# joejep/FOCNeRF

Measured on AMD Instinct MI355X. Metric: train_samples_per_sec, higher is better.
Workload: dtype f16

## Files before the change

### focnerf_amd/backend.py

```python
import math

import torch

from . import _lib
from ._lib import lib, ptr, stream_of, check, require_cuda, dtype_code, raw_stream


def _f32(*ts):
    for t in ts:
        if t is not None and t.dtype != torch.float32:
            raise RuntimeError(f"focnerf_amd: expected float32 tensor, got {t.dtype}")


def _contig(*ts):
    for t in ts:
        if t is not None and not t.is_contiguous():
            raise RuntimeError("focnerf_amd: tensor must be contiguous")


class _Scratch:

    def __init__(self):
        self._bufs = {}
        self._pinned = []
# ... 278 lines not shown
    def ffmlp_inference(inputs, weights, B, input_dim, output_dim, hidden_dim, num_layers, activation, output_activation, inference_buffer, outputs):
        require_cuda(inputs, weights, outputs); _half(inputs, weights, outputs); _contig(inputs, weights, outputs)
        check(lib.foc_ffmlp_inference(ptr(inputs), ptr(weights), B, input_dim, output_dim, hidden_dim, num_layers, activation, output_activation,
                                      ptr(inference_buffer), ptr(outputs), stream_of(inputs)), "ffmlp_inference")

    @staticmethod
    def ffmlp_backward(grad, inputs, weights, forward_buffer, B, input_dim, output_dim, hidden_dim, num_layers, activation, output_activation,
                       calc_grad_inputs, backward_buffer, grad_inputs, grad_weights):
        ts = (grad, inputs, weights, forward_buffer, backward_buffer, grad_inputs, grad_weights)
        require_cuda(*ts); _half(*ts); _contig(*ts)
        ws_bytes = lib.foc_ffmlp_backward_workspace_bytes(input_dim, hidden_dim, num_layers)
        ws = _scratch.get("ffmlp_ws", ws_bytes, grad.device)
        check(lib.foc_ffmlp_backward(ptr(grad), ptr(inputs), ptr(weights), ptr(forward_buffer), B, input_dim, output_dim, hidden_dim, num_layers,
                                     activation, output_activation, int(bool(calc_grad_inputs)), ptr(backward_buffer), ptr(grad_inputs),
                                     ptr(grad_weights), ptr(ws), ws.numel(), stream_of(grad)), "ffmlp_backward")

    @staticmethod
    def ffmlp_forward_planar(inputs_planar, weights, B, input_dim, output_dim, hidden_dim, num_layers, activation, output_activation, outputs):
        require_cuda(inputs_planar, weights, outputs); _half(inputs_planar, weights, outputs); _contig(inputs_planar, weights, outputs)
        check(lib.foc_ffmlp_forward_planar(ptr(inputs_planar), ptr(weights), B, input_dim, output_dim, hidden_dim, num_layers, activation,
                                           output_activation, ptr(outputs), stream_of(inputs_planar)), "ffmlp_forward_planar")

    @staticmethod
    def ffmlp_backward_planar(grad, inputs_planar, weights, B, input_dim, output_dim, hidden_dim, num_layers, activation, output_activation,
                              calc_grad_inputs, grad_inputs_planar, grad_weights):
        ts = (grad, inputs_planar, weights, grad_inputs_planar, grad_weights)
        require_cuda(*ts); _half(*ts); _contig(*ts)
        ws = _scratch.get("ffmlp_ws", lib.foc_ffmlp_backward_workspace_bytes(input_dim, hidden_dim, num_layers), grad.device)
        check(lib.foc_ffmlp_backward_planar(ptr(grad), ptr(inputs_planar), ptr(weights), B, input_dim, output_dim, hidden_dim, num_layers,
                                            activation, output_activation, int(bool(calc_grad_inputs)), ptr(grad_inputs_planar),
                                            ptr(grad_weights), ptr(ws), ws.numel(), stream_of(grad)), "ffmlp_backward_planar")

    @staticmethod
    def allocate_splitk(size):
        check(lib.foc_allocate_splitk(int(size)), "allocate_splitk")

    @staticmethod
    def free_splitk():
        check(lib.foc_free_splitk(), "free_splitk")
```

### focnerf_amd/csrc/combine.hip

```cpp
#include "common.h"
#include "fs_common.h"
#include <string.h>
#include <cmath>

static thread_local char g_err[512] = "";

void foc_set_error(const char *fmt, ...) {
    va_list ap;
    va_start(ap, fmt);
    vsnprintf(g_err, sizeof(g_err), fmt, ap);
    va_end(ap);
}

__global__ void __launch_bounds__(256) k_combine_select(const float *__restrict__ dens, const float *__restrict__ rgb,
                                                        float *__restrict__ max_dens, float *__restrict__ best_rgb, uint64_t n) {
    for (uint64_t i = (uint64_t)blockIdx.x * 256 + threadIdx.x; i < n; i += (uint64_t)gridDim.x * 256) {
        const float d = dens[i], m = max_dens[i];
        if (d > m) { best_rgb[i * 3] = rgb[i * 3]; best_rgb[i * 3 + 1] = rgb[i * 3 + 1]; best_rgb[i * 3 + 2] = rgb[i * 3 + 2]; }
        max_dens[i] = (d != d || m != m) ? __builtin_nanf("") : (d > m ? d : m);
    }
}

__global__ void __launch_bounds__(256) k_combine_pack(const float *__restrict__ dens, uint32_t rank, uint64_t *__restrict__ keys, uint64_t n) {
    for (uint64_t i = (uint64_t)blockIdx.x * 256 + threadIdx.x; i < n; i += (uint64_t)gridDim.x * 256) {
// ... 328 lines not shown
        acc4[i] = best;
    }
}

template <typename T>
__global__ void __launch_bounds__(256) k_mo_select(const T *__restrict__ sig_new, const T *__restrict__ feat_new, T *__restrict__ sig_best,
                                                   T *__restrict__ feat_best, uint64_t n, uint32_t width) {
    const uint64_t s0 = ((uint64_t)blockIdx.x * 4u + (threadIdx.x >> 6)) * 64u;
    if (s0 >= n) return;
    const uint32_t lane = threadIdx.x & 63u;
    bool take = false;
    if (s0 + lane < n) {
        const T a_raw = sig_new[s0 + lane];
        const float a = (float)a_raw, b = (float)sig_best[s0 + lane];
        take = (a != a) || (b == b && a >= b);
        if (take) sig_best[s0 + lane] = a_raw;
    }
    const uint64_t rows = __ballot(take);
    const uint32_t live = (uint32_t)(n - s0 < 64u ? n - s0 : 64u);
    const uint64_t base = s0 * width;
    for (uint32_t e = lane; e < live * width; e += 64u)
        if ((rows >> (e / width)) & 1ull) feat_best[base + e] = feat_new[base + e];
}

#include <stdlib.h>
#include <string.h>
#include <atomic>
#include <mutex>
struct FocOptionRow { const char *name; std::atomic<int> value; };
static FocOptionRow foc_option_table[FOC_OPT_COUNT] = {
    {"FOC_MLP_BWD_FUSED", 1}, {"FOC_FIELD_FWD_FUSED", 1}, {"FOC_GB_MERGE_MAX_RES", 480}, {"FOC_GB_FACTORED", 1}, {"FOC_GB_TAIL_SPLIT", 16}, {"FOC_GRID_FUSE_SMALL", 1},
    {"FOC_GRID_PAIRS", 1}, {"FOC_GRID_FAST", 1}, {"FOC_MARCH_SERIAL", -1}, {"FOC_MARCH_RAYS_ROW_MAX", 131072}, {"FOC_OCC_MARCH_FORM", -1},
    {"FOC_OCC_SAMPLE_MAJOR", 1}, {"FOC_OCC_FIELD_PIECE", 1 << 23}, {"FOC_DETERMINISTIC", 0},
};
static int foc_option_parse(int which, const char *text) {
    if (which == FOC_OPT_OCC_MARCH_FORM) {
        if (text[0] == 't') return 0;
        if (text[0] == 'r') return 1;
        if (text[0] == 'l') return 2;
        if (text[0] == 's') return 3;
    }
    return atoi(text);
}
static void foc_options_init() {
    static std::once_flag once;
    std::call_once(once, [] {
        for (int i = 0; i < FOC_OPT_COUNT; i++) {
            const char *e = getenv(foc_option_table[i].name);
            if (e && e[0]) foc_option_table[i].value.store(foc_option_parse(i, e), std::memory_order_relaxed);
        }
    });
}
int foc_opt(FocOpt which) { foc_options_init(); return foc_option_table[which].value.load(std::memory_order_relaxed); }

extern "C" {

int foc_set_option(const char *name, int value) {
    foc_options_init();
    for (int i = 0; i < FOC_OPT_COUNT; i++)
        if (name && strcmp(name, foc_option_table[i].name) == 0) { foc_option_table[i].value.store(value, std::memory_order_relaxed); return FOC_OK; }
    foc_set_error("set_option: unknown option '%s'", name ? name : "(null)");
    return FOC_E_INVALID;
}

int foc_get_option(const char *name, int *value) {
    foc_options_init();
// ... 213 lines not shown
```

### focnerf_amd/csrc/common.h

```cpp
#pragma once
#include <hip/hip_runtime.h>
#include <hip/hip_fp16.h>
#include <stdint.h>
#include <stdio.h>
#include <stdarg.h>
#include <map>
#include <mutex>
#include <tuple>
#include "../../include/focnerf.h"

#define FOC_WAVE 64

void foc_set_error(const char *fmt, ...);

enum FocOpt {
    FOC_OPT_MLP_BWD_FUSED,
    FOC_OPT_FIELD_FWD_FUSED,
    FOC_OPT_GB_MERGE_MAX_RES,
    FOC_OPT_GB_FACTORED,
    FOC_OPT_GB_TAIL_SPLIT,
    FOC_OPT_GRID_FUSE_SMALL,
    FOC_OPT_GRID_PAIRS,
    FOC_OPT_GRID_FAST,
    FOC_OPT_MARCH_SERIAL,
    FOC_OPT_MARCH_RAYS_ROW_MAX,
    FOC_OPT_OCC_MARCH_FORM,
    FOC_OPT_OCC_SAMPLE_MAJOR,
    FOC_OPT_OCC_FIELD_PIECE,
    FOC_OPT_DETERMINISTIC,
    FOC_OPT_COUNT
};
int foc_opt(FocOpt which);

#define FOC_REQUIRE(cond, code, ...)                    \
    do {                                                \
        if (!(cond)) {                                  \
            foc_set_error(__VA_ARGS__);                 \
            return (code);                              \
        }                                               \
    } while (0)

#define FOC_CHECK_LAUNCH(name)                                                     \
    do {                                                                           \
        hipError_t e_ = hipGetLastError();                                         \
        if (e_ != hipSuccess) {                                                    \
            foc_set_error("%s: launch failed: %s", name, hipGetErrorString(e_));   \
            return FOC_E_LAUNCH;                                                   \
        }                                                                          \
    } while (0)

static inline int foc_guard_pick(bool stream_is_null, int stream_device, int pointer_device, int current_device) {
    if (!stream_is_null && stream_device >= 0) return stream_device;
    if (pointer_device >= 0) return pointer_device;
    return current_device;
}
struct FocDeviceGuard {
    int prev = -1;
    explicit FocDeviceGuard(void *stream, const void *first_pointer = nullptr) {
        static int n_devices = -1;
        if (n_devices < 0 && hipGetDeviceCount(&n_devices) != hipSuccess) { (void)hipGetLastError(); n_devices = 0; }
        if (n_devices == 1) return;
        int cur = 0;
// ... 132 lines not shown
```

### focnerf_amd/csrc/ffmlp.hip

```cpp
#include "common.h"
#include "activations.h"
#include <stdlib.h>

#include <type_traits>
#include "mlp_common.h"

template <int HIDDEN, int NB, bool TRAIN, int IMODE, bool GEN = false>
__global__ void __launch_bounds__(MLP_BLOCK, 2) k_mlp_fwd(const _Float16 *__restrict__ inputs, const _Float16 *__restrict__ weights,
                                                       _Float16 *__restrict__ fwd_buf, _Float16 *__restrict__ outputs,
                                                       uint32_t B, uint32_t in_dim, uint32_t num_layers, int act, MlpHead hd) {
    const int relu = act == FOC_ACT_RELU;
    constexpr int MT = (HIDDEN + 31) / 32, KC = HIDDEN / 16;
    constexpr bool planar = IMODE == 1;
    extern __shared__ __attribute__((aligned(16))) _Float16 lds[];
    const uint32_t KS0 = IMODE == 2 ? 2u : in_dim / 16;
    const uint32_t f_hidden = MT * KS0, f_out = f_hidden + (num_layers - 1) * MT * KC;
    const float *obj_bias = reinterpret_cast<const float *>(lds + (size_t)(f_out + KC) * 512);
    if constexpr (IMODE == 2) {
        stage_weights_fwd<HIDDEN>(weights, lds, in_dim, num_layers, true, head_ld0(hd));
        if (head_bias(hd)) stage_head_bias(weights, hd, const_cast<float *>(obj_bias), HIDDEN);
    } else stage_weights_fwd<HIDDEN>(weights, lds, in_dim, num_layers);
    __syncthreads();

    const uint32_t lane = threadIdx.x & 63, wave = threadIdx.x >> 6;
// ... 301 lines not shown
                    if (!(o < OUT)) av = u32x4{0u, 0u, 0u, 0u};
                    if (!(i < IN)) bv = u32x4{0u, 0u, 0u, 0u};
                    acc[t] = mfma16(__builtin_bit_cast(h8, av), __builtin_bit_cast(h8, bv), acc[t]);
                }
            }
        }
    }
#pragma unroll
    for (int t = 0; t < 4; t++) {
        const uint32_t tile = wave + t * MLP_WAVES + 16 * blockIdx.z;
        if (tile < n_out_tiles) {
            const uint32_t mt = tile / NTi, nt = tile % NTi;
            const uint32_t i = 32 * nt + r;
#pragma unroll
            for (int reg = 0; reg < 16; reg++) {
                const uint32_t o = 32 * mt + acc_row(reg, h);
                if (o < OUT && i < IN) (void)__hip_atomic_fetch_add(ws + ws_off + (uint64_t)o * IN + i, acc[t][reg], __ATOMIC_RELAXED, __HIP_MEMORY_SCOPE_AGENT);
            }
        }
    }
}

__global__ void __launch_bounds__(256) k_mlp_dw_finalize(const float *__restrict__ ws, _Float16 *__restrict__ gw, uint32_t n) {
    for (uint32_t i = blockIdx.x * 256 + threadIdx.x; i < n; i += gridDim.x * 256) gw[i] = (_Float16)ws[i];
}
__global__ void __launch_bounds__(256) k_mlp_dw_finalize_slots(const float *__restrict__ ws, uint32_t slots, uint64_t stride, _Float16 *__restrict__ gw, uint32_t n) {
    for (uint32_t i = blockIdx.x * 256 + threadIdx.x; i < n; i += gridDim.x * 256) {
        float v = 0.0f;
        for (uint32_t k = 0; k < slots; k++) v += ws[k * stride + i];
        gw[i] = (_Float16)v;
    }
}

template <int HIDDEN, int NL, int NB, bool RECOMP, int IMODE, bool RELU_CT, bool IN32 = false, bool LEAN = false>
__global__ void __launch_bounds__(MLP_BLOCK, 2) k_mlp_bwd_fused(const _Float16 *__restrict__ grad, const _Float16 *__restrict__ inputs,
                                                             const _Float16 *__restrict__ weights, const _Float16 *__restrict__ fwd_buf,
                                                             _Float16 *__restrict__ bwd_buf_arg, _Float16 *__restrict__ grad_inputs, float *__restrict__ ws,
                                                             uint32_t B, uint32_t in_dim, int relu_rt, uint32_t lds_w_halfs, MlpHead hd) {
    const int relu = RELU_CT ? 1 : relu_rt;
    f16v FZ;
#pragma unroll
    for (int e = 0; e < 16; e++) FZ[e] = 0.0f;
    constexpr int MT = (HIDDEN + 31) / 32, KC = HIDDEN / 16, RW = 32 * NB;
    constexpr bool planar = IMODE == 1, HEAD = IMODE >= 2, NARROW = IMODE == 3;
    static_assert(!HEAD || RECOMP, "the head input modes have no stored-activation form");
    constexpr int WD = (HIDDEN < 32 ? 32 : HIDDEN) + 8;
    extern __shared__ __attribute__((aligned(16))) _Float16 lds[];
    const bool with_dx = LEAN ? true : grad_inputs != nullptr;
    _Float16 *const bwd_buf = LEAN ? nullptr : bwd_buf_arg;
    uint32_t ld0 = in_dim;
    bool has_obj = false;
    if constexpr (HEAD) { ld0 = head_ld0(hd); has_obj = hd.obj != nullptr; }
    bool col31_set = false;
    _Float16 col31 = (_Float16)0.0f;
    if constexpr (HEAD) { col31_set = head_bias(hd); col31 = has_obj ? (_Float16)1.0f : (_Float16)hd.pad; }
    stage_weights_bwd<HIDDEN>(weights, lds, in_dim, NL, with_dx, HEAD, ld0);
    const uint32_t WA = (in_dim > (uint32_t)HIDDEN ? in_dim : (uint32_t)(HIDDEN < 32 ? 32 : HIDDEN)) + 8;
    _Float16 *sD = lds + lds_w_halfs;
    _Float16 *sA = sD + 4 * RW * WD;
    _Float16 *ldsF = sA + 4 * RW * WA;
    const float *obj_bias = reinterpret_cast<const float *>(ldsF + (size_t)(((HIDDEN + 31) / 32) * (in_dim / 16) + (NL - 1) * ((HIDDEN + 31) / 32) * (HIDDEN / 16)) * 512);
    if constexpr (RECOMP) {
        stage_weights_fwd<HIDDEN>(weights, ldsF, in_dim, NL, false, ld0);
        if constexpr (HEAD) { if (head_bias(hd)) stage_head_bias(weights, hd, const_cast<float *>(obj_bias), HIDDEN); }
    }
    __syncthreads();

    const uint32_t lane = threadIdx.x & 63, wave = threadIdx.x >> 6;
    const int c = lane & 31, h = lane >> 5;
// ... 364 lines not shown
            __builtin_amdgcn_s_setprio(0);
#ifndef FOC_TIMING_NO_BARRIER
            foc_lds_barrier();
#endif
        }
    }
    float *slot = ws + (uint64_t)blockIdx.x * ((NL + 1) * MLP_DW_SLOT_STAGE);
    float *meet = reinterpret_cast<float *>(sD);
#pragma unroll
    for (int s = 0; s <= NL; s++) {
        const uint32_t OUT = s == 0 ? 16u : (uint32_t)HIDDEN;
        const uint32_t IN = s < NL ? (uint32_t)HIDDEN : in_dim;
        const uint32_t ntile = ((OUT + 31) / 32) * ((IN + 31) / 32), ksplit = (ntile * 2 <= 4) ? 2u : 1u;
        if (ksplit == 2u) {
            __syncthreads();
            if (wave >= ntile && wave < 2u * ntile) {
#pragma unroll
                for (int reg = 0; reg < 16; reg++) meet[((wave - ntile) * 16 + reg) * 64 + lane] = dwacc[s][reg];
            }
            __syncthreads();
            if (wave < ntile) {
#pragma unroll
                for (int reg = 0; reg < 16; reg++) slot[(s * 4 + wave) * 1024 + reg * 64 + lane] = dwacc[s][reg] + meet[(wave * 16 + reg) * 64 + lane];
            }
        } else if (wave < ntile) {
#pragma unroll
            for (int reg = 0; reg < 16; reg++) slot[(s * 4 + wave) * 1024 + reg * 64 + lane] = dwacc[s][reg];
        }
    }
}

template <int HIDDEN>
__global__ void __launch_bounds__(1024) k_mlp_dw_reduce(const float *__restrict__ slots, uint32_t n_slots, uint32_t NL, uint32_t in_dim, uint32_t ld0,
                                                        _Float16 *__restrict__ gw, float *__restrict__ wsb) {
    __shared__ float part[16][64];
    const uint32_t lane = threadIdx.x & 63, slice = threadIdx.x >> 6;
    const uint32_t s = blockIdx.x / 64, w = (blockIdx.x / 16) % 4, reg = blockIdx.x % 16;
    const uint32_t OUT = s == 0 ? 16u : (uint32_t)HIDDEN, IN = s < NL ? (uint32_t)HIDDEN : in_dim;
    const uint32_t NTi = (IN + 31) / 32, MTo = (OUT + 31) / 32, ntile = MTo * NTi, ksplit = 1u;
    if (w >= ntile) return;
    const uint32_t mt = w / NTi, nt = w % NTi, h = lane >> 5;
    const uint32_t o = 32 * mt + (uint32_t)acc_row((int)reg, (int)h), i = 32 * nt + (lane & 31);
    if (!(o < OUT) && !(32 * mt + (uint32_t)acc_row((int)reg, 1 - (int)h) < OUT)) return;
    const uint64_t stride = (uint64_t)(NL + 1) * MLP_DW_SLOT_STAGE;
    const float *p = slots + (uint64_t)(s * 4 + w) * 1024 + reg * 64 + lane;
    float a0 = 0.f, a1 = 0.f, a2 = 0.f, a3 = 0.f;
    for (uint32_t k = 0; k < ksplit; k++) {
        const float *q = p + (uint64_t)k * ntile * 1024;
        uint32_t g = slice;
        for (; g + 48 < n_slots; g += 64) {
            a0 += q[(uint64_t)g * stride]; a1 += q[(uint64_t)(g + 16) * stride]; a2 += q[(uint64_t)(g + 32) * stride]; a3 += q[(uint64_t)(g + 48) * stride];
        }
        for (; g < n_slots; g += 16) a0 += q[(uint64_t)g * stride];
    }
    part[slice][lane] = (a0 + a1) + (a2 + a3);
    __syncthreads();
    if (slice == 0 && o < OUT && i < IN) {
        float v = 0.f;
#pragma unroll
        for (int k = 0; k < 16; k++) v += part[k][lane];
        const uint64_t first = (uint64_t)HIDDEN * ld0, lsz = (uint64_t)HIDDEN * HIDDEN;
        const uint32_t fl = NL - s;
        const uint64_t off = (s == 0 ? first + (uint64_t)(NL - 1) * lsz : (fl == 0 ? 0 : first + (uint64_t)(fl - 1) * lsz)) + (uint64_t)o * (s == NL ? ld0 : IN) + i;
        if (wsb) wsb[off] = v; else gw[off] = (_Float16)v;
    }
}

__global__ void __launch_bounds__(256) k_mlp_dw_finalize_obj(const float *__restrict__ ws, _Float16 *__restrict__ gw, uint32_t n, uint32_t hidden,
                                                             const _Float16 *__restrict__ W, const _Float16 *__restrict__ obj, float *__restrict__ grad_obj,
                                                             float pad) {
    const uint32_t n0 = hidden * HEAD_OBJ_LD;
    for (uint32_t i = blockIdx.x * 256 + threadIdx.x; i < n; i += gridDim.x * 256) {
        float v = ws[i];
        if (i < n0) {
            const uint32_t o = i / HEAD_OBJ_LD, col = i % HEAD_OBJ_LD;
            if (col >= 31) v = col < 47 ? ws[o * HEAD_OBJ_LD + 31] * (float)obj[col - 31] : (pad != 0.0f ? ws[o * HEAD_OBJ_LD + 31] * pad : 0.0f);
        }
        gw[i] = (_Float16)v;
    }
    if (blockIdx.x == 0 && threadIdx.x < 16 && grad_obj) {
        float a = 0.0f;
        for (uint32_t o = 0; o < hidden; o++) a = fmaf((float)W[o * HEAD_OBJ_LD + 31 + threadIdx.x], ws[o * HEAD_OBJ_LD + 31], a);
        grad_obj[threadIdx.x] = a;
    }
}

__device__ __forceinline__ void nf_sh16_half(float x, float y, float z, int h, h8 &out) {
    const float xy = x * y, xz = x * z, yz = y * z, x2 = x * x, y2 = y * y, z2 = z * z;
    float o[8];
    if (h == 0) {
        o[0] = 0.28209479177387814f; o[1] = -0.48860251190291987f * y; o[2] = 0.48860251190291987f * z; o[3] = -0.48860251190291987f * x;
        o[4] = 1.0925484305920792f * xy; o[5] = -1.0925484305920792f * yz; o[6] = 0.94617469575755997f * z2 - 0.31539156525251999f;
        o[7] = -1.0925484305920792f * xz;
    } else {
        o[0] = 0.54627421529603959f * x2 - 0.54627421529603959f * y2; o[1] = 0.59004358992664352f * y * (-3.0f * x2 + y2);
        o[2] = 2.8906114426405538f * xy * z; o[3] = 0.45704579946446572f * y * (1.0f - 5.0f * z2);
        o[4] = 0.3731763325901154f * z * (5.0f * z2 - 3.0f); o[5] = 0.45704579946446572f * x * (1.0f - 5.0f * z2);
        o[6] = 1.4453057213202769f * z * (x2 - y2); o[7] = 0.59004358992664352f * x * (-x2 + 3.0f * y2);
    }
#pragma unroll
    for (int j = 0; j < 8; j++) out[j] = (_Float16)o[j];
}

template <int NLS, int NLC, bool PLANAR, bool RELU_CT, bool BLK, bool OBJ, bool P31 = false>
__global__ void __launch_bounds__(MLP_BLOCK, 2) k_nerf_infer(const _Float16 *__restrict__ enc, const float *__restrict__ dirs, uint32_t dir_div,
                                                          uint32_t dir_block, uint32_t n_dirs, const _Float16 *__restrict__ w_sigma, const _Float16 *__restrict__ w_color, uint32_t B,
                                                          int relu_rt, float *__restrict__ sigma_out, float *__restrict__ rgb_out, const _Float16 *__restrict__ obj,
                                                          float pad) {
    const int relu = RELU_CT ? 1 : relu_rt;
    f16v FZ;
#pragma unroll
    for (int e = 0; e < 16; e++) FZ[e] = 0.0f;
    constexpr int HIDDEN = 64, MT = 2, KC = 4, NB = 2, IN = 32, KS0 = 2;
    extern __shared__ __attribute__((aligned(16))) _Float16 lds[];
    constexpr uint32_t n_sigma = MT * KS0 + (NLS - 1) * MT * KC + KC;
// ... 227 lines not shown
    if (gen) kern = k_mlp_fwd<HIDDEN, NB, TRAIN, 0, true>;
    if constexpr (HIDDEN == 64 && !TRAIN) { if (head) kern = k_mlp_fwd<HIDDEN, NB, false, 2>; }
    else FOC_REQUIRE(!head, FOC_E_INVALID, "color_head_forward: hidden_dim must be 64");
    const uint32_t grid = foc_persistent_grid(kern, MLP_BLOCK, lds, foc_div_up(foc_div_up(B, 32 * NB), MLP_WAVES));
    hipLaunchKernelGGL(kern, dim3(grid), dim3(MLP_BLOCK), lds, st, (const _Float16 *)inputs, (const _Float16 *)weights, (_Float16 *)fwd_buf,
                       (_Float16 *)outputs, B, in_dim, num_layers, act, head ? *head : MlpHead{nullptr, nullptr, 1u, 16u, nullptr, 0.0f});
    FOC_CHECK_LAUNCH(TRAIN ? "ffmlp_forward" : "ffmlp_inference");
    return FOC_OK;
}

template <bool TRAIN>
static int mlp_fwd(const void *inputs, const void *weights, uint32_t B, uint32_t input_dim, uint32_t output_dim, uint32_t hidden_dim,
                   uint32_t num_layers, uint32_t activation, uint32_t output_activation, void *buffer, void *outputs, void *stream, int planar = 0) {
    const char *who = TRAIN ? "ffmlp_forward" : "ffmlp_inference";
    int rc = mlp_check(who, B, input_dim, output_dim, hidden_dim, num_layers, activation, output_activation);
    if (rc) return rc;
    if (B == 0) return FOC_OK;
    FOC_REQUIRE(inputs && weights && outputs && (!TRAIN || buffer), FOC_E_INVALID, "%s: null pointer", who);
    const int act = (int)activation;
    hipStream_t st = (hipStream_t)stream;
    switch (hidden_dim) {
        case 16: return mlp_fwd_launch<16, TRAIN>(inputs, weights, B, input_dim, num_layers, act, buffer, outputs, planar, st);
        case 32: return mlp_fwd_launch<32, TRAIN>(inputs, weights, B, input_dim, num_layers, act, buffer, outputs, planar, st);
        case 64: return mlp_fwd_launch<64, TRAIN>(inputs, weights, B, input_dim, num_layers, act, buffer, outputs, planar, st);
        case 128: return mlp_fwd_launch<128, TRAIN>(inputs, weights, B, input_dim, num_layers, act, buffer, outputs, planar, st);
        case 256:
            FOC_REQUIRE(!planar, FOC_E_INVALID, "%s: planar inputs are served up to hidden_dim 128", who);
            return mlp_wide_forward(TRAIN, inputs, weights, B, input_dim, 256, num_layers, act, buffer, outputs, st);
    }
    return FOC_E_INVALID;
}

template <int HIDDEN, int NL>
static int mlp_bwd_fused_launch(const void *grad, const void *inputs, const void *weights, const void *fwd_buf, uint32_t B, uint32_t in_dim, int relu,
                                void *bwd_buf, void *grad_inputs, void *grad_weights, float *ws, int planar, hipStream_t st, const MlpHead *head = nullptr,
                                float *grad_obj = nullptr) {
    FOC_REQUIRE(!planar || fwd_buf == nullptr, FOC_E_INVALID, "ffmlp_backward: planar inputs need the re-evaluating form (forward_buffer NULL)");
    constexpr int NB = 1, RW = 32 * NB, WD = (HIDDEN < 32 ? 32 : HIDDEN) + 8;
    const bool dx = grad_inputs != nullptr;
    const size_t lds_w = mlp_bwd_lds<HIDDEN>(in_dim, NL, dx);
    const uint32_t WA = (in_dim > (uint32_t)HIDDEN ? in_dim : (uint32_t)(HIDDEN < 32 ? 32 : HIDDEN)) + 8;
    const bool recomp = fwd_buf == nullptr;
    constexpr int MT = (HIDDEN + 31) / 32, KC = HIDDEN / 16;
    const bool has_obj = head && head->obj;
    const size_t lds = lds_w + (size_t)4 * RW * (WD + WA) * sizeof(_Float16) + (recomp ? (size_t)(MT * (in_dim / 16) + (NL - 1) * MT * KC) * 1024 : 0) +
                       (head && head_bias(*head) ? 256 : 0);
    FOC_REQUIRE(lds <= 160 * 1024, FOC_E_INVALID, "ffmlp_backward: fused kernel needs %zu B of LDS", lds);
#ifdef FOC_TIMING_ONE_WG
    const size_t lds_launch = lds < 84 * 1024 ? 84 * 1024 : lds;
#else
    const size_t lds_launch = lds;
#endif
    auto kern = recomp ? (planar ? (relu ? k_mlp_bwd_fused<HIDDEN, NL, NB, true, 1, true> : k_mlp_bwd_fused<HIDDEN, NL, NB, true, 1, false>)
                                 : (relu ? k_mlp_bwd_fused<HIDDEN, NL, NB, true, 0, true> : k_mlp_bwd_fused<HIDDEN, NL, NB, true, 0, false>))
                       : k_mlp_bwd_fused<HIDDEN, NL, NB, false, 0, false>;
    const bool lean = !bwd_buf && dx;
    if constexpr (HIDDEN == 64) {
        if (recomp && relu && in_dim <= 32 && !head) {
            if (lean) kern = planar ? k_mlp_bwd_fused<HIDDEN, NL, NB, true, 1, true, true, true> : k_mlp_bwd_fused<HIDDEN, NL, NB, true, 0, true, true, true>;
            else kern = planar ? k_mlp_bwd_fused<HIDDEN, NL, NB, true, 1, true, true> : k_mlp_bwd_fused<HIDDEN, NL, NB, true, 0, true, true>;
        }
    }
    if constexpr (HIDDEN == 64 && NL >= 2 && NL <= 3) {
        if (head) kern = head->out_width == 4u ? (relu ? (lean ? k_mlp_bwd_fused<HIDDEN, NL, NB, true, 3, true, false, true> : k_mlp_bwd_fused<HIDDEN, NL, NB, true, 3, true>)
                                                       : k_mlp_bwd_fused<HIDDEN, NL, NB, true, 3, false>)
                                               : (relu ? (lean ? k_mlp_bwd_fused<HIDDEN, NL, NB, true, 2, true, false, true> : k_mlp_bwd_fused<HIDDEN, NL, NB, true, 2, true>)
                                                       : k_mlp_bwd_fused<HIDDEN, NL, NB, true, 2, false>);
    }
    else FOC_REQUIRE(!head, FOC_E_INVALID, "color_head_backward: hidden_dim must be 64 and num_layers 2 or 3");
    const uint32_t n_w = HIDDEN * ((has_obj ? HEAD_OBJ_LD : in_dim) + HIDDEN * (NL - 1) + 16);
    const uint32_t grid = min(foc_persistent_grid(kern, MLP_BLOCK, lds_launch, foc_div_up(B, 4 * RW), 2u), MLP_DW_MAX_SLOTS);
    float *slots = ws + mlp_dw_blob_floats(has_obj ? HEAD_OBJ_LD : in_dim, HIDDEN, NL);
    hipLaunchKernelGGL(kern, dim3(grid), dim3(MLP_BLOCK), lds_launch, st, (const _Float16 *)grad, (const _Float16 *)inputs, (const _Float16 *)weights,
                       (const _Float16 *)fwd_buf, (_Float16 *)bwd_buf, (_Float16 *)grad_inputs, slots, B, in_dim, relu, (uint32_t)(lds_w / sizeof(_Float16)),
                       head ? *head : MlpHead{nullptr, nullptr, 1u, 16u, nullptr, 0.0f});
    FOC_CHECK_LAUNCH("ffmlp_backward(fused)");
    hipLaunchKernelGGL((k_mlp_dw_reduce<HIDDEN>), dim3((NL + 1) * 64), dim3(1024), 0, st, (const float *)slots, grid, (uint32_t)NL, in_dim,
                       has_obj ? (uint32_t)HEAD_OBJ_LD : in_dim, (_Float16 *)grad_weights, has_obj ? ws : (float *)nullptr);
    FOC_CHECK_LAUNCH("ffmlp_backward(reduce)");
    if (has_obj) {
        hipLaunchKernelGGL(k_mlp_dw_finalize_obj, dim3(foc_grid_1d(n_w, 256)), dim3(256), 0, st, ws, (_Float16 *)grad_weights, n_w, (uint32_t)HIDDEN,
                           (const _Float16 *)weights, head->obj, grad_obj, head->pad);
        FOC_CHECK_LAUNCH("ffmlp_backward(finalize)");
    }
    return FOC_OK;
}

template <int HIDDEN>
static int mlp_dw_launch(const void *grad, const void *inputs, const void *fwd_buf, const void *bwd_buf, uint32_t B, uint32_t in_dim, uint32_t num_layers,
                         void *grad_weights, float *ws, bool det, hipStream_t st) {
    const uint32_t n_w = HIDDEN * (in_dim + HIDDEN * (num_layers - 1) + 16);
    const uint64_t det_stride = det ? mlp_dw_blob_floats(in_dim, HIDDEN, num_layers) : 0;
    uint32_t gx = foc_div_up(B, DW_CHUNK);
    if (det && gx > MLP_DW_DET_SLOTS) gx = MLP_DW_DET_SLOTS;
    if (foc_zero_async(ws, det ? (size_t)gx * det_stride * sizeof(float) : (size_t)n_w * sizeof(float), st) != hipSuccess) { foc_set_error("ffmlp_backward: memset of workspace failed"); return FOC_E_LAUNCH; }
    const int wgs_per_cu = 8;
    const uint32_t tiles = ((HIDDEN + 31) / 32) * ((max((uint32_t)HIDDEN, in_dim) + 31) / 32), GZ = (tiles + 15) / 16;
    const uint32_t capx = foc_div_up(foc_num_cus() * (uint32_t)wgs_per_cu, (num_layers + 1) * GZ);
    if (gx > capx) gx = capx;
    if (gx < 1) gx = 1;
    auto kern = k_mlp_dw<HIDDEN>;
    if constexpr (HIDDEN <= 128) { if (in_dim > 128) kern = k_mlp_dw<HIDDEN, 256>; }
    hipLaunchKernelGGL(kern, dim3(gx, num_layers + 1, GZ), dim3(MLP_BLOCK), 0, st, (const _Float16 *)grad, (const _Float16 *)inputs,
                       (const _Float16 *)fwd_buf, (const _Float16 *)bwd_buf, ws, B, in_dim, num_layers, det_stride);
    FOC_CHECK_LAUNCH("ffmlp_backward(weights)");
    if (det) hipLaunchKernelGGL(k_mlp_dw_finalize_slots, dim3(foc_grid_1d(n_w, 256)), dim3(256), 0, st, ws, gx, det_stride, (_Float16 *)grad_weights, n_w);
    else hipLaunchKernelGGL(k_mlp_dw_finalize, dim3(foc_grid_1d(n_w, 256)), dim3(256), 0, st, ws, (_Float16 *)grad_weights, n_w);
    FOC_CHECK_LAUNCH("ffmlp_backward(finalize)");
    return FOC_OK;
}

template <int HIDDEN>
static int mlp_bwd_launch(const void *grad, const void *inputs, const void *weights, const void *fwd_buf, uint32_t B, uint32_t in_dim,
                          uint32_t num_layers, int act, void *bwd_buf, void *grad_inputs, void *grad_weights, float *ws, int planar, bool det, hipStream_t st) {
    const bool gen = act != FOC_ACT_RELU && act != FOC_ACT_NONE;
    const int relu = act == FOC_ACT_RELU;
    const int use_fused = foc_opt(FOC_OPT_MLP_BWD_FUSED);
    if constexpr (HIDDEN <= 64) {
// ... 101 lines not shown
        case 128: return mlp_bwd_launch<128>(grad, inputs, weights, forward_buffer, B, input_dim, num_layers, relu, backward_buffer, gi, grad_weights, (float *)workspace, planar, det, st);
        case 256: {
            FOC_REQUIRE(backward_buffer && forward_buffer, FOC_E_INVALID, "ffmlp_backward: hidden_dim 256 runs layer by layer and needs forward_buffer and backward_buffer");
            FOC_REQUIRE(!planar, FOC_E_INVALID, "ffmlp_backward: planar inputs are served up to hidden_dim 64");
            rc = mlp_wide_backward_activations(grad, weights, forward_buffer, B, input_dim, 256, num_layers, relu, backward_buffer, gi, st);
            if (rc) return rc;
            return mlp_dw_launch<256>(grad, inputs, forward_buffer, backward_buffer, B, input_dim, num_layers, grad_weights, (float *)workspace, det, st);
        }
    }
    return FOC_E_INVALID;
}

int foc_ffmlp_backward(const void *grad, const void *inputs, const void *weights, const void *forward_buffer, uint32_t B, uint32_t input_dim,
                       uint32_t output_dim, uint32_t hidden_dim, uint32_t num_layers, uint32_t activation, uint32_t output_activation,
                       int calc_grad_inputs, void *backward_buffer, void *grad_inputs, void *grad_weights, void *workspace, uint64_t workspace_bytes,
                       void *stream) {
    FocDeviceGuard foc_guard_(stream, grad);
    return mlp_bwd_entry(grad, inputs, weights, forward_buffer, B, input_dim, output_dim, hidden_dim, num_layers, activation, output_activation,
                         calc_grad_inputs, backward_buffer, grad_inputs, grad_weights, workspace, workspace_bytes, 0, stream);
}

int foc_ffmlp_forward_planar(const void *inputs_planar, const void *weights, uint32_t B, uint32_t input_dim, uint32_t output_dim, uint32_t hidden_dim,
                             uint32_t num_layers, uint32_t activation, uint32_t output_activation, void *outputs, void *stream) {
    FocDeviceGuard foc_guard_(stream, inputs_planar);
    return mlp_fwd<false>(inputs_planar, weights, B, input_dim, output_dim, hidden_dim, num_layers, activation, output_activation, nullptr, outputs, stream, 1);
}

int foc_ffmlp_backward_planar(const void *grad, const void *inputs_planar, const void *weights, uint32_t B, uint32_t input_dim, uint32_t output_dim,
                              uint32_t hidden_dim, uint32_t num_layers, uint32_t activation, uint32_t output_activation, int calc_grad_inputs,
                              void *grad_inputs_planar, void *grad_weights, void *workspace, uint64_t workspace_bytes, void *stream) {
    FocDeviceGuard foc_guard_(stream, grad);
    return mlp_bwd_entry(grad, inputs_planar, weights, nullptr, B, input_dim, output_dim, hidden_dim, num_layers, activation, output_activation,
                         calc_grad_inputs, nullptr, grad_inputs_planar, grad_weights, workspace, workspace_bytes, 1, stream);
}

int nerf_field_inference(const void *enc, int enc_planar, const float *dirs, uint32_t dir_div, uint32_t dir_block, uint32_t n_dirs,
                         const void *sigma_weights, uint32_t sigma_layers, const void *color_weights, uint32_t color_layers, uint32_t hidden_dim,
                         uint32_t activation, uint32_t B, float *sigma, float *rgb, const void *obj_feat, float input_pad, bool pad31,
                         void *stream) {
    FocDeviceGuard foc_guard_(stream, enc);
    if (B == 0) return FOC_OK;
    FOC_REQUIRE(enc && dirs && sigma_weights && color_weights && rgb, FOC_E_INVALID, "nerf_field_inference: null pointer");
    FOC_REQUIRE(hidden_dim == 64 && dir_div >= 1, FOC_E_INVALID, "nerf_field_inference: hidden_dim must be 64 (got %u)", hidden_dim);
    FOC_REQUIRE(dir_block == 0 || n_dirs >= 1, FOC_E_INVALID, "nerf_field_inference: the block-interleaved row order needs the number of directions");
    FOC_REQUIRE((uint64_t)dir_block * dir_div < (1ull << 32), FOC_E_INVALID, "nerf_field_inference: dir_block * dir_div must fit 32 bits");
    FOC_REQUIRE(activation == 0 || activation == 6, FOC_E_INVALID, "nerf_field_inference: hidden activation must be relu(0) or none(6)");
    int rc = head_pad_check("nerf_field_inference", pad31, obj_feat, input_pad);
    if (rc) return rc;
    const int relu = activation == 0;
    hipStream_t st = (hipStream_t)stream;
    const uint32_t key = sigma_layers * 10 + color_layers;
    const float pad = input_pad;
    switch (key) {
        case 12: return nerf_infer_launch<1, 2>(enc, dirs, dir_div, dir_block, n_dirs, sigma_weights, color_weights, B, relu, enc_planar, sigma, rgb, obj_feat, pad, st);
        case 13: return nerf_infer_launch<1, 3>(enc, dirs, dir_div, dir_block, n_dirs, sigma_weights, color_weights, B, relu, enc_planar, sigma, rgb, obj_feat, pad, st);
        case 22: return nerf_infer_launch<2, 2>(enc, dirs, dir_div, dir_block, n_dirs, sigma_weights, color_weights, B, relu, enc_planar, sigma, rgb, obj_feat, pad, st);
        case 23: return nerf_infer_launch<2, 3>(enc, dirs, dir_div, dir_block, n_dirs, sigma_weights, color_weights, B, relu, enc_planar, sigma, rgb, obj_feat, pad, st);
        case 33: return nerf_infer_launch<3, 3>(enc, dirs, dir_div, dir_block, n_dirs, sigma_weights, color_weights, B, relu, enc_planar, sigma, rgb, obj_feat, pad, st);
        default: foc_set_error("nerf_field_inference: layer counts (%u, %u) are not built (1/2, 1/3, 2/2, 2/3, 3/3)", sigma_layers, color_layers); return FOC_E_INVALID;
    }
}

int foc_nerf_field_inference(const void *enc, int enc_planar, const float *dirs, uint32_t dir_div, uint32_t dir_block, uint32_t n_dirs,
                             const void *sigma_weights, uint32_t sigma_layers,
                             const void *color_weights, uint32_t color_layers, uint32_t hidden_dim, uint32_t activation, uint32_t B, float *sigma,
                             float *rgb, const void *obj_feat, void *stream) {
// ... 75 lines not shown
                "color_head_backward: workspace of %llu bytes, foc_ffmlp_backward_workspace_bytes(%u, 64, %u) asks for %llu", (unsigned long long)workspace_bytes,
                obj_feat ? HEAD_OBJ_LD : 32u, num_layers, (unsigned long long)foc_ffmlp_backward_workspace_bytes(obj_feat ? HEAD_OBJ_LD : 32u, 64, num_layers));
    FOC_REQUIRE(out_width == 16 || out_width == 4, FOC_E_INVALID, "color_head_backward: out_width must be 16 or 4 (got %u)", out_width);
    FOC_REQUIRE(activation == FOC_ACT_RELU || activation == FOC_ACT_NONE, FOC_E_INVALID, "color_head_backward: hidden activation must be relu(0) or none(6)");
    rc = head_pad_check("color_head_backward", pad31, obj_feat, input_pad);
    if (rc) return rc;
    const MlpHead hd{(const _Float16 *)ray_sh, (const _Float16 *)grad_h0, samples_per_ray, out_width, (const _Float16 *)obj_feat, input_pad};
    const int relu = activation == 0;
    if (num_layers == 2) return mlp_bwd_fused_launch<64, 2>(grad, h, weights, nullptr, B, 32, relu, nullptr, grad_h, grad_weights, (float *)workspace, 0, (hipStream_t)stream, &hd, grad_obj);
    return mlp_bwd_fused_launch<64, 3>(grad, h, weights, nullptr, B, 32, relu, nullptr, grad_h, grad_weights, (float *)workspace, 0, (hipStream_t)stream, &hd, grad_obj);
}

int foc_color_head_backward(const void *grad, const void *h, const void *ray_sh, uint32_t samples_per_ray, const void *grad_h0, const void *weights,
                            uint32_t B, uint32_t hidden_dim, uint32_t num_layers, uint32_t activation, void *grad_h, void *grad_weights, void *workspace,
                            uint64_t workspace_bytes, uint32_t out_width, const void *obj_feat, float *grad_obj, void *stream) {
    return color_head_backward(grad, h, ray_sh, samples_per_ray, grad_h0, weights, B, hidden_dim, num_layers, activation, grad_h, grad_weights, workspace,
                               workspace_bytes, out_width, obj_feat, grad_obj, 0.0f, false, stream);
}

int foc_color_head_backward_pad(const void *grad, const void *h, const void *ray_sh, uint32_t samples_per_ray, const void *grad_h0, const void *weights,
                                uint32_t B, uint32_t hidden_dim, uint32_t num_layers, uint32_t activation, void *grad_h, void *grad_weights, void *workspace,
                                uint64_t workspace_bytes, uint32_t out_width, const void *obj_feat, float *grad_obj, float input_pad, void *stream) {
    return color_head_backward(grad, h, ray_sh, samples_per_ray, grad_h0, weights, B, hidden_dim, num_layers, activation, grad_h, grad_weights, workspace,
                               workspace_bytes, out_width, obj_feat, grad_obj, input_pad, false, stream);
}

int foc_color_head_backward_pad31(const void *grad, const void *h, const void *ray_sh, uint32_t samples_per_ray, const void *grad_h0, const void *weights,
                                  uint32_t B, uint32_t hidden_dim, uint32_t num_layers, uint32_t activation, void *grad_h, void *grad_weights, void *workspace,
                                  uint64_t workspace_bytes, uint32_t out_width, const void *obj_feat, float *grad_obj, float input_pad, void *stream) {
    return color_head_backward(grad, h, ray_sh, samples_per_ray, grad_h0, weights, B, hidden_dim, num_layers, activation, grad_h, grad_weights, workspace,
                               workspace_bytes, out_width, obj_feat, grad_obj, input_pad, true, stream);
}

int foc_allocate_splitk(uint64_t size) { (void)size; return FOC_OK; }
int foc_free_splitk(void) { return FOC_OK; }

}
```

### focnerf_amd/csrc/field_fwd.hip

```cpp
#include "mlp_common.h"

typedef uint32_t ff_u2 __attribute__((ext_vector_type(2)));

__device__ __forceinline__ uint32_t ff_pack(float a, float b) {
    typedef _Float16 h2 __attribute__((ext_vector_type(2)));
    const h2 p = {(_Float16)a, (_Float16)b};
    return __builtin_bit_cast(uint32_t, p);
}

#ifndef FF_MIN_WAVES
#define FF_MIN_WAVES 2
#endif
template <int NLS, int NLC, bool RELU>
__global__ void __launch_bounds__(MLP_BLOCK, FF_MIN_WAVES) k_field_fwd_train(const _Float16 *__restrict__ planes, const _Float16 *__restrict__ w_sigma,
                                                               const _Float16 *__restrict__ w_color, _Float16 *__restrict__ h_out,
                                                               _Float16 *__restrict__ c_out, uint32_t B, MlpHead hd) {
    constexpr int HIDDEN = 64, MT = 2, KC = 4, KS0 = 2;
    constexpr int FS = MT * KS0 + (NLS - 1) * MT * KC + KC;
    constexpr int FC = MT * KS0 + (NLC - 1) * MT * KC + KC;
    extern __shared__ __attribute__((aligned(16))) _Float16 lds[];
    _Float16 *ldsS = lds, *ldsC = lds + FS * 512;
    const float *obj_bias = reinterpret_cast<const float *>(ldsC + FC * 512);
    stage_weights_fwd<HIDDEN>(w_sigma, ldsS, 32, NLS);
    stage_weights_fwd<HIDDEN>(w_color, ldsC, 32, NLC, true, head_ld0(hd));
    if (head_bias(hd)) stage_head_bias(w_color, hd, const_cast<float *>(obj_bias), HIDDEN);
    __syncthreads();

    const uint32_t lane = threadIdx.x & 63, wave = threadIdx.x >> 6;
    const int c = lane & 31, h = lane >> 5;
    const uint32_t n_tiles = (B + 31) / 32;
    const uint32_t tstride = gridDim.x * MLP_WAVES;
    uint32_t tile = blockIdx.x * MLP_WAVES + wave;
    h8 x_nxt[KS0], sh_nxt;
    auto fetch = [&](uint32_t t) {
#ifdef FF_TIMING_NO_LOAD
        const uint64_t r = (uint64_t)c + 0 * t;
#else
        const uint64_t r = min((uint64_t)min(t, n_tiles - 1u) * 32 + c, (uint64_t)B - 1);
#endif
#pragma unroll
        for (int kc = 0; kc < KS0; kc++) x_nxt[kc] = ld_planar8(planes, B, r, kc, h);
        sh_nxt = ld_head8(planes, hd, r, 0, h);
    };
    fetch(tile);
    for (; tile < n_tiles; tile += tstride) {
#ifndef FF_TIMING_HOIST
        asm volatile("" ::: "memory");
#endif
// ... 60 lines not shown
#pragma unroll
            for (int mt = 0; mt < MT; mt++) acc[mt] = mfma16(ld_frag(ldsC, mt * KS0 + kc, lane), kc == 0 ? sh : hk, acc[mt]);
        for (uint32_t l = 1; l <= (uint32_t)NLC; l++) {
            h8 bf[KC];
#pragma unroll
            for (int kc = 0; kc < KC; kc++) bf[kc] = acc_to_frag<RELU>(acc[kc >> 1], kc & 1);
            if (l < (uint32_t)NLC) {
                const uint32_t fbase = MT * KS0 + (l - 1) * MT * KC;
#pragma unroll
                for (int mt = 0; mt < MT; mt++)
#pragma unroll
                    for (int e = 0; e < 16; e++) acc[mt][e] = 0.0f;
#pragma unroll
                for (int kc = 0; kc < KC; kc++)
#pragma unroll
                    for (int mt = 0; mt < MT; mt++) acc[mt] = mfma16(ld_frag(ldsC, fbase + mt * KC + kc, lane), bf[kc], acc[mt]);
            } else {
#pragma unroll
                for (int e = 0; e < 16; e++) o[e] = 0.0f;
#pragma unroll
                for (int kc = 0; kc < KC; kc++) o = mfma16(ld_frag(ldsC, FC - KC + kc, lane), bf[kc], o);
                if (hd.out_width == 4u) {
#ifdef FF_TIMING_NO_STORE
                    if (h == 0 && row_raw == 0xFFFFFFFFFFull) *reinterpret_cast<ff_u2 *>(c_out + row_raw * 4) = ff_u2{ff_pack(o[0], o[1]), ff_pack(o[2], o[3])};
#else
                    if (h == 0 && row_raw < B) *reinterpret_cast<ff_u2 *>(c_out + row_raw * 4) = ff_u2{ff_pack(o[0], o[1]), ff_pack(o[2], o[3])};
#endif
                } else store_tile<false>(c_out, 16, row_raw, B, 0, 16, o, h);
            }
        }
    }
}

template <int NLS, int NLC, bool RELU>
static int ff_launch(const void *planes, const void *w_sigma, const void *w_color, void *h, void *c, uint32_t B, const MlpHead &hd, hipStream_t st) {
    auto kern = k_field_fwd_train<NLS, NLC, RELU>;
    const size_t lds = (size_t)((4 + (NLS - 1) * 8 + 4) + (4 + (NLC - 1) * 8 + 4)) * 1024 + 256;
    const uint32_t grid = foc_persistent_grid(kern, MLP_BLOCK, lds, foc_div_up(foc_div_up(B, 32), MLP_WAVES));
    hipLaunchKernelGGL(kern, dim3(grid), dim3(MLP_BLOCK), lds, st, (const _Float16 *)planes, (const _Float16 *)w_sigma, (const _Float16 *)w_color,
                       (_Float16 *)h, (_Float16 *)c, B, hd);
    FOC_CHECK_LAUNCH("field_forward_train");
    return FOC_OK;
}

template <int NLS, int NLC>
static int ff_launch_act(const void *planes, const void *w_sigma, const void *w_color, void *h, void *c, uint32_t B, int relu, const MlpHead &hd, hipStream_t st) {
    return relu ? ff_launch<NLS, NLC, true>(planes, w_sigma, w_color, h, c, B, hd, st) : ff_launch<NLS, NLC, false>(planes, w_sigma, w_color, h, c, B, hd, st);
}

int field_forward_train(const void *planes, const void *sigma_weights, uint32_t sigma_layers, const void *ray_sh, uint32_t samples_per_ray,
                        const void *color_weights, uint32_t color_layers, uint32_t hidden_dim, uint32_t activation, uint32_t B, void *h, void *c,
                        uint32_t out_width, const void *obj_feat, float input_pad, bool pad31, void *stream) {
    FocDeviceGuard foc_guard_(stream, planes);
    if (B == 0) return FOC_OK;
    FOC_REQUIRE(planes && sigma_weights && ray_sh && color_weights && h && c, FOC_E_INVALID, "field_forward_train: null pointer");
    FOC_REQUIRE(hidden_dim == 64 && samples_per_ray >= 1, FOC_E_INVALID, "field_forward_train: hidden_dim must be 64 (got %u), samples_per_ray >= 1", hidden_dim);
    FOC_REQUIRE(activation == FOC_ACT_RELU || activation == FOC_ACT_NONE, FOC_E_INVALID, "field_forward_train: hidden activation must be relu(0) or none(6)");
    FOC_REQUIRE(out_width == 16 || out_width == 4, FOC_E_INVALID, "field_forward_train: out_width must be 16 or 4 (got %u)", out_width);
    const int prc = head_pad_check("field_forward_train", pad31, obj_feat, input_pad);
    if (prc) return prc;
    const MlpHead hd{(const _Float16 *)ray_sh, nullptr, samples_per_ray, out_width, (const _Float16 *)obj_feat, input_pad};
    const int relu = activation == FOC_ACT_RELU;
    hipStream_t st = (hipStream_t)stream;
    switch (sigma_layers * 10 + color_layers) {
        case 12: return ff_launch_act<1, 2>(planes, sigma_weights, color_weights, h, c, B, relu, hd, st);
        case 13: return ff_launch_act<1, 3>(planes, sigma_weights, color_weights, h, c, B, relu, hd, st);
        case 22: return ff_launch_act<2, 2>(planes, sigma_weights, color_weights, h, c, B, relu, hd, st);
        case 23: return ff_launch_act<2, 3>(planes, sigma_weights, color_weights, h, c, B, relu, hd, st);
        case 33: return ff_launch_act<3, 3>(planes, sigma_weights, color_weights, h, c, B, relu, hd, st);
        default: foc_set_error("field_forward_train: layer counts (%u, %u) are not built (1/2, 1/3, 2/2, 2/3, 3/3)", sigma_layers, color_layers); return FOC_E_INVALID;
    }
}

extern "C" {

int foc_field_forward_train(const void *planes, const void *sigma_weights, uint32_t sigma_layers, const void *ray_sh, uint32_t samples_per_ray,
                            const void *color_weights, uint32_t color_layers, uint32_t hidden_dim, uint32_t activation, uint32_t B, void *h, void *c,
                            uint32_t out_width, const void *obj_feat, void *stream) {
    return field_forward_train(planes, sigma_weights, sigma_layers, ray_sh, samples_per_ray, color_weights, color_layers, hidden_dim, activation, B, h, c,
                               out_width, obj_feat, 0.0f, false, stream);
}

int foc_field_forward_train_pad(const void *planes, const void *sigma_weights, uint32_t sigma_layers, const void *ray_sh, uint32_t samples_per_ray,
                                const void *color_weights, uint32_t color_layers, uint32_t hidden_dim, uint32_t activation, uint32_t B, void *h, void *c,
                                uint32_t out_width, const void *obj_feat, float input_pad, void *stream) {
    return field_forward_train(planes, sigma_weights, sigma_layers, ray_sh, samples_per_ray, color_weights, color_layers, hidden_dim, activation, B, h, c,
                               out_width, obj_feat, input_pad, false, stream);
}

int foc_field_forward_train_pad31(const void *planes, const void *sigma_weights, uint32_t sigma_layers, const void *ray_sh, uint32_t samples_per_ray,
                                  const void *color_weights, uint32_t color_layers, uint32_t hidden_dim, uint32_t activation, uint32_t B, void *h, void *c,
                                  uint32_t out_width, const void *obj_feat, float input_pad, void *stream) {
    return field_forward_train(planes, sigma_weights, sigma_layers, ray_sh, samples_per_ray, color_weights, color_layers, hidden_dim, activation, B, h, c,
                               out_width, obj_feat, input_pad, true, stream);
}

}
```

### focnerf_amd/csrc/fixedstep.hip

```cpp
#include "common.h"
#include "fs_common.h"
#include <float.h>

__global__ void __launch_bounds__(256) k_fs_sample(const float *__restrict__ rays_o, const float *__restrict__ rays_d, const float *__restrict__ nears,
                                                   const float *__restrict__ fars, const float *__restrict__ aabb, const float *__restrict__ noise,
                                                   uint32_t N, uint32_t T, float bound, float *__restrict__ xyzs, float *__restrict__ enc_in,
                                                   _Float16 *__restrict__ ray_sh, uint32_t ray_block) {
    const uint64_t total = ray_block ? (uint64_t)((N + FS_RAY_BLOCK - 1) / FS_RAY_BLOCK) * FS_RAY_BLOCK * T : (uint64_t)N * T;
    const FsBox box = fs_box(aabb);
    const float two_b = 2 * bound;
    for (uint64_t s = (uint64_t)blockIdx.x * 256 + threadIdx.x; s < total; s += (uint64_t)gridDim.x * 256) {
        uint32_t n, i;
        bool own = true;
        if (ray_block) {
            const uint32_t blk = (uint32_t)(s / ((uint64_t)FS_RAY_BLOCK * T)), in = (uint32_t)(s - (uint64_t)blk * FS_RAY_BLOCK * T);
            i = in / FS_RAY_BLOCK;
            n = blk * FS_RAY_BLOCK + in % FS_RAY_BLOCK;
            own = n < N;
            n = own ? n : N - 1;
        } else {
            n = (uint32_t)(s / T); i = (uint32_t)(s - (uint64_t)n * T);
        }
        const FsGeom g = fs_geom(nears, fars, n, T);
        const float z = fs_z(g, i, T, noise, (uint64_t)n * T + i);
        float x, y, w;
        fs_point(rays_o[n * 3], rays_o[n * 3 + 1], rays_o[n * 3 + 2], rays_d[n * 3], rays_d[n * 3 + 1], rays_d[n * 3 + 2], z, box, x, y, w);
        if (xyzs) { xyzs[s * 3] = x; xyzs[s * 3 + 1] = y; xyzs[s * 3 + 2] = w; }
        if (enc_in) { enc_in[s * 3] = fs_norm(x, bound, two_b); enc_in[s * 3 + 1] = fs_norm(y, bound, two_b); enc_in[s * 3 + 2] = fs_norm(w, bound, two_b); }
        if (ray_sh && i == 0 && own) {
            h8 lo, hi;
            foc_sh16_h(rays_d[n * 3], rays_d[n * 3 + 1], rays_d[n * 3 + 2], lo, hi);
            h8 *dst = reinterpret_cast<h8 *>(ray_sh + (uint64_t)n * 16);
            dst[0] = lo; dst[1] = hi;
        }
    }
}

__global__ void __launch_bounds__(256) k_fs_head_fwd(const _Float16 *__restrict__ h, const float *__restrict__ rays_d, const float *__restrict__ nears,
                                                     const float *__restrict__ fars, const float *__restrict__ noise, uint32_t N, uint32_t T,
                                                     float density_scale, float *__restrict__ sigma_out, float *__restrict__ trans_out,
                                                     float *__restrict__ weights_out, float *__restrict__ weights_sum, float *__restrict__ depth,
                                                     _Float16 *__restrict__ cin, const _Float16 *__restrict__ obj, uint32_t cin_ld) {
    const uint32_t lane = threadIdx.x & 63;
    const uint32_t n = blockIdx.x * 4 + (threadIdx.x >> 6);
    if (n >= N) return;
    const FsGeom g = fs_geom(nears, fars, n, T);
    h8 shlo, shhi;
    h8 ob1 = {0, 0, 0, 0, 0, 0, 0, 0}, ob2 = {0, 0, 0, 0, 0, 0, 0, 0};
    _Float16 ob0 = (_Float16)0;
    if (cin) {
        foc_sh16_h(rays_d[n * 3], rays_d[n * 3 + 1], rays_d[n * 3 + 2], shlo, shhi);
        if (obj) {
            ob0 = obj[0];
#pragma unroll
            for (int k = 0; k < 8; k++) ob1[k] = obj[1 + k];
#pragma unroll
            for (int k = 0; k < 7; k++) ob2[k] = obj[9 + k];
        }
    }
    float Tc = 1.0f, ws = 0, dp = 0;
    for (uint32_t base = 0; base < T; base += 64) {
        const uint32_t i = base + lane;
        const bool valid = i < T;
        const uint64_t s = (uint64_t)n * T + (valid ? i : T - 1);
        h8 r0, r1;
        if (cin) { r0 = *reinterpret_cast<const h8 *>(h + s * 16); r1 = *reinterpret_cast<const h8 *>(h + s * 16 + 8); }
        else r0[0] = h[s * 16];
        const float sigma = expf((float)r0[0]);
// ... 305 lines not shown
    const uint32_t fe = st->first_enc, W = fe ? N - fe + 2u : 0u;
    const uint32_t H = W ? N / W : 0u;
    const bool grid = W >= 16u && N % W == 0u && H >= 8u && st->count == 2u * (H - 1u) && st->bad == 0u;
    for (uint32_t p = blockIdx.x * 256 + threadIdx.x; p < N; p += gridDim.x * 256) {
        uint32_t src = p;
        if (grid) {
            const uint64_t wt = (uint64_t)W * th;
            const uint32_t ty = (uint32_t)(p / wt), rem = (uint32_t)(p - ty * wt);
            const uint32_t rows_here = min(th, H - ty * th);
            const uint32_t tx = min(rem / (rows_here * tw), (W - 1u) / tw), r2 = rem - tx * rows_here * tw;
            const uint32_t cols_here = min(tw, W - tx * tw);
            src = (ty * th + r2 / cols_here) * W + tx * tw + r2 % cols_here;
        }
        perm[p] = (int64_t)src;
    }
}

extern "C" {

int foc_fixed_sample(const float *rays_o, const float *rays_d, const float *nears, const float *fars, const float *aabb, const float *noise,
                     uint32_t N, uint32_t T, float bound, float *xyzs, float *enc_in, void *ray_sh, uint32_t ray_block, void *stream) {
    FocDeviceGuard foc_guard_(stream, rays_o);
    if (N == 0) return FOC_OK;
    FOC_REQUIRE(rays_o && rays_d && nears && fars && aabb && (xyzs || enc_in), FOC_E_INVALID, "fixed_sample: null pointer");
    FOC_REQUIRE(T >= 2, FOC_E_INVALID, "fixed_sample: T must be >= 2");
    FOC_REQUIRE(ray_block == 0 || ray_block == FS_RAY_BLOCK, FOC_E_INVALID, "fixed_sample: ray_block must be 0 (ray-major) or %u (got %u)", FS_RAY_BLOCK, ray_block);
    const uint64_t rows = ray_block ? (uint64_t)foc_div_up(N, FS_RAY_BLOCK) * FS_RAY_BLOCK * T : (uint64_t)N * T;
    hipLaunchKernelGGL(k_fs_sample, dim3(foc_grid_1d(rows, 256, 256 * 16)), dim3(256), 0, (hipStream_t)stream, rays_o, rays_d, nears, fars, aabb,
                       noise, N, T, bound, xyzs, enc_in, (_Float16 *)ray_sh, ray_block);
    FOC_CHECK_LAUNCH("fixed_sample");
    return FOC_OK;
}

int foc_fixed_head_forward(const void *h, const float *rays_d, const float *nears, const float *fars, const float *noise, uint32_t N, uint32_t T,
                           float density_scale, float *sigma, float *trans, float *weights, float *weights_sum, float *depth, void *cin,
                           const void *obj_feat, uint32_t cin_width, void *stream) {
    FocDeviceGuard foc_guard_(stream, h);
    if (N == 0) return FOC_OK;
    FOC_REQUIRE(h && rays_d && nears && fars && sigma && trans && weights && weights_sum && depth, FOC_E_INVALID, "fixed_head_forward: null pointer");
    FOC_REQUIRE(T >= 2, FOC_E_INVALID, "fixed_head_forward: T must be >= 2");
    FOC_REQUIRE(cin_width == 32 || cin_width == 48, FOC_E_INVALID, "fixed_head_forward: cin_width must be 32 or 48 (got %u)", cin_width);
    FOC_REQUIRE(!obj_feat || cin_width == 48, FOC_E_INVALID, "fixed_head_forward: an object feature needs the 48-wide colour input");
    hipLaunchKernelGGL(k_fs_head_fwd, dim3(foc_div_up(N, 4)), dim3(256), 0, (hipStream_t)stream, (const _Float16 *)h, rays_d, nears, fars, noise, N, T,
                       density_scale, sigma, trans, weights, weights_sum, depth, (_Float16 *)cin, (const _Float16 *)obj_feat, cin_width);
    FOC_CHECK_LAUNCH("fixed_head_forward");
    return FOC_OK;
}

int foc_fixed_head_backward(const void *h, const float *sigma, const float *trans, const float *nears, const float *fars, const float *noise,
                            const float *grad_w, const float *grad_ws, const float *grad_depth, const void *grad_cin, uint32_t N, uint32_t T,
                            float density_scale, void *grad_h, uint32_t cin_width, void *stream) {
    FocDeviceGuard foc_guard_(stream, h);
    if (N == 0) return FOC_OK;
    FOC_REQUIRE(h && sigma && trans && nears && fars && grad_h, FOC_E_INVALID, "fixed_head_backward: null pointer");
    FOC_REQUIRE(T >= 2, FOC_E_INVALID, "fixed_head_backward: T must be >= 2");
    FOC_REQUIRE(cin_width == 32 || cin_width == 48, FOC_E_INVALID, "fixed_head_backward: cin_width must be 32 or 48 (got %u)", cin_width);
    hipLaunchKernelGGL(k_fs_head_bwd, dim3(foc_div_up(N, 4)), dim3(256), 0, (hipStream_t)stream, (const _Float16 *)h, sigma, trans, nears, fars, noise,
                       grad_w, grad_ws, grad_depth, (const _Float16 *)grad_cin, N, T, density_scale, (_Float16 *)grad_h, cin_width);
    FOC_CHECK_LAUNCH("fixed_head_backward");
    return FOC_OK;
}

int foc_fixed_composite_forward(const void *c, const float *weights, const float *bg_ray, float bg_scalar, uint32_t N, uint32_t T, float thresh,
                                float *image, void *stream) {
    FocDeviceGuard foc_guard_(stream, c);
    if (N == 0) return FOC_OK;
// ... 149 lines not shown
```

### focnerf_amd/csrc/fs_common.h

```cpp
#pragma once
#include "common.h"
#include "sample_math.h"

struct FsGeom { float near, far, span, sample_dist, step; };

#define FS_RAY_BLOCK 64u
__host__ __device__ __forceinline__ uint64_t fs_block_row(uint32_t n, uint32_t i, uint32_t T) {
    return (uint64_t)(n / FS_RAY_BLOCK) * FS_RAY_BLOCK * T + (uint64_t)i * FS_RAY_BLOCK + n % FS_RAY_BLOCK;
}

__device__ __forceinline__ FsGeom fs_geom(const float *__restrict__ nears, const float *__restrict__ fars, uint32_t n, uint32_t T) {
    FsGeom g;
    g.near = nears[n]; g.far = fars[n];
    g.span = g.far - g.near;
    g.sample_dist = g.span / (float)T;
    g.step = 1.0f / (float)(T - 1);
    return g;
}
__device__ __forceinline__ float fs_z0(const FsGeom &g, uint32_t i, uint32_t T) {
    const float lin = (i < T / 2) ? (g.step * (float)i) : fmaf(-g.step, (float)(T - 1 - i), 1.0f);
    return g.near + g.span * lin;
}
__device__ __forceinline__ float fs_jitter(const FsGeom &g, float z, float u) { return z + (u - 0.5f) * g.sample_dist; }
__device__ __forceinline__ float fs_z(const FsGeom &g, uint32_t i, uint32_t T, const float *__restrict__ noise, uint64_t s) {
    float z = fs_z0(g, i, T);
    if (noise) z = fs_jitter(g, z, noise[s]);
    return z;
}
__device__ __forceinline__ float fs_zu(const FsGeom &g, uint32_t i, uint32_t T, bool jitter, float u) {
    float z = fs_z0(g, i, T);
    if (jitter) z = fs_jitter(g, z, u);
    return z;
}

struct FsSample { float z, delta, oz; };
__device__ __forceinline__ FsSample fs_sample(const FsGeom &g, uint32_t i, uint32_t ic, uint32_t T, bool jitter, float u0, float u1) {
    FsSample p;
    p.z = fs_zu(g, ic, T, jitter, u0);
    p.delta = g.sample_dist;
    if (i + 1 < T) p.delta = fs_zu(g, i + 1, T, jitter, u1) - p.z;
    p.oz = (p.z - g.near) / g.span;
    p.oz = p.oz < 0.0f ? 0.0f : (p.oz > 1.0f ? 1.0f : p.oz);
    return p;
}
__device__ __forceinline__ FsSample fs_sample_ld(const FsGeom &g, uint32_t i, uint32_t ic, uint32_t T, const float *__restrict__ noise, uint64_t s) {
    const bool jitter = noise != nullptr;
    return fs_sample(g, i, ic, T, jitter, jitter ? noise[s] : 0.0f, jitter && i + 1 < T ? noise[s + 1] : 0.0f);
}

__device__ __forceinline__ float fs_trans_scan(float om, uint32_t lane, float &Tc) {
// ... 102 lines not shown
```

### focnerf_amd/csrc/mlp_common.h

```cpp
#pragma once
#include "common.h"
#include "activations.h"

typedef _Float16 h8 __attribute__((ext_vector_type(8)));
typedef _Float16 h4 __attribute__((ext_vector_type(4)));
typedef float f16v __attribute__((ext_vector_type(16)));
typedef short s4 __attribute__((__vector_size__(4 * sizeof(short))));
typedef __attribute__((address_space(3))) s4 lds_s4;
typedef uint32_t u32x2 __attribute__((ext_vector_type(2)));
typedef uint32_t u32x4 __attribute__((ext_vector_type(4)));

#define MLP_BLOCK 256
#define MLP_WAVES 4
#define MLP_DW_SLOT_STAGE 4096u
#define MLP_DW_MAX_SLOTS 1024u
#ifndef FOC_MLP_SETPRIO
#define FOC_MLP_SETPRIO 1
#endif

__device__ __forceinline__ int acc_row(int reg, int h) { return (reg & 3) + 8 * (reg >> 2) + 4 * h; }
__device__ __forceinline__ int chain_k(int kc, int h, int j) { return 16 * kc + 8 * (j >> 2) + 4 * h + (j & 3); }

__device__ __forceinline__ f16v mfma16(const h8 a, const h8 b, const f16v c) {
    return __builtin_amdgcn_mfma_f32_32x32x16_f16(a, b, c, 0, 0, 0);
}

__device__ __forceinline__ h8 ld_frag(const _Float16 *lds, uint32_t frag, uint32_t lane) {
    return *reinterpret_cast<const h8 *>(lds + (size_t)frag * 512 + lane * 8);
}

template <bool RELU>
__device__ __forceinline__ h8 acc_to_frag(const f16v &acc, int s) {
    typedef _Float16 h2 __attribute__((ext_vector_type(2)));
    h8 r;
#pragma unroll
    for (int j = 0; j < 8; j += 2) {
        h2 p = {(_Float16)acc[8 * s + j], (_Float16)acc[8 * s + j + 1]};
        if (RELU) p = __builtin_elementwise_max(p, h2{(_Float16)0, (_Float16)0});
        r[j] = p[0]; r[j + 1] = p[1];
    }
    return r;
}

__device__ __forceinline__ h8 acc_to_frag_act(const f16v &acc, int s, int act) {
    h8 r;
#pragma unroll
    for (int j = 0; j < 8; j++) r[j] = foc_act_forward((_Float16)acc[8 * s + j], act);
    return r;
}

__device__ __forceinline__ h8 relu_gate(const h8 d, const h8 a) {
    const u32x4 db = __builtin_bit_cast(u32x4, d), ab = __builtin_bit_cast(u32x4, a);
    u32x4 r;
#pragma unroll
    for (int i = 0; i < 4; i++) {
        uint32_t m, o;
        asm("v_pk_min_u16 %0, %1, %2" : "=v"(m) : "v"(ab[i]), "v"(0x00010001u));
        asm("v_pk_mul_lo_u16 %0, %1, %2" : "=v"(o) : "v"(db[i]), "v"(m));
        r[i] = o;
    }
    return __builtin_bit_cast(h8, r);
}

__device__ __forceinline__ h8 ld_planar8(const _Float16 *__restrict__ base, uint64_t B, uint64_t row, uint32_t kc, int h) {
    const uint32_t *p = reinterpret_cast<const uint32_t *>(base) + (uint64_t)(8 * kc + 4 * h) * B + row;
    const u32x4 v = {p[0], p[B], p[2 * B], p[3 * B]};
    return __builtin_bit_cast(h8, v);
}

struct MlpHead {
    const _Float16 *ray_sh;
    const _Float16 *grad_h0;
    uint32_t samples_per_ray;
    uint32_t out_width;
    const _Float16 *obj;
    float pad;
};
#define HEAD_OBJ_LD 48u
__device__ __forceinline__ uint32_t head_ld0(const MlpHead &hd) { return hd.obj ? HEAD_OBJ_LD : 32u; }
__host__ __device__ __forceinline__ bool head_bias(const MlpHead &hd) { return hd.obj != nullptr || hd.pad != 0.0f; }

__device__ __forceinline__ void stage_obj_bias(const _Float16 *__restrict__ W0, const _Float16 *__restrict__ obj, float *bias, uint32_t hidden, float pad) {
    if (threadIdx.x < hidden) {
        const uint32_t n = threadIdx.x, r = n & 31u, mt = n >> 5;
        const uint32_t h = (r >> 2) & 1u, reg = (r & 3u) + 4u * (r >> 3);
        float a = 0.0f;
#pragma unroll
        for (int j = 0; j < 16; j++) a = fmaf((float)W0[(size_t)n * HEAD_OBJ_LD + 31 + j], (float)obj[j], a);
        if (pad != 0.0f) a = fmaf((float)W0[(size_t)n * HEAD_OBJ_LD + 47], pad, a);
        bias[(mt * 2 + h) * 16 + reg] = a;
    }
}
static inline int head_pad_check(const char *who, bool pad31, const void *obj_feat, float input_pad) {
    if (pad31) FOC_REQUIRE(!obj_feat, FOC_E_INVALID, "%s_pad31: input_pad is column 31 of the 32-wide colour input, obj_feat must be NULL "
                                                     "(a 48-wide row takes its pad through foc_%s_pad)", who, who);
    else FOC_REQUIRE(input_pad == 0.0f || obj_feat, FOC_E_INVALID, "%s: input_pad is column 47 of the 48-wide colour input and needs obj_feat", who);
    return FOC_OK;
}
static inline bool head_layer_pair(uint32_t sigma_layers, uint32_t color_layers) {
    const uint32_t lk = sigma_layers * 10 + color_layers;
    return lk == 12 || lk == 13 || lk == 22 || lk == 23 || lk == 33;
}
extern "C" {
FOC_INTERNAL int field_forward_train(const void *planes, const void *sigma_weights, uint32_t sigma_layers, const void *ray_sh, uint32_t samples_per_ray,
                                     const void *color_weights, uint32_t color_layers, uint32_t hidden_dim, uint32_t activation, uint32_t B, void *h, void *c,
                                     uint32_t out_width, const void *obj_feat, float input_pad, bool pad31, void *stream);
FOC_INTERNAL int nerf_field_inference(const void *enc, int enc_planar, const float *dirs, uint32_t dir_div, uint32_t dir_block, uint32_t n_dirs,
                                      const void *sigma_weights, uint32_t sigma_layers, const void *color_weights, uint32_t color_layers, uint32_t hidden_dim,
                                      uint32_t activation, uint32_t B, float *sigma, float *rgb, const void *obj_feat, float input_pad, bool pad31, void *stream);
FOC_INTERNAL int color_head_forward(const void *h, const void *ray_sh, uint32_t samples_per_ray, const void *weights, uint32_t B, uint32_t hidden_dim,
                                    uint32_t num_layers, uint32_t activation, void *outputs, uint32_t out_width, const void *obj_feat, float input_pad, bool pad31,
                                    void *stream);
FOC_INTERNAL int color_head_backward(const void *grad, const void *h, const void *ray_sh, uint32_t samples_per_ray, const void *grad_h0, const void *weights,
                                     uint32_t B, uint32_t hidden_dim, uint32_t num_layers, uint32_t activation, void *grad_h, void *grad_weights, void *workspace,
                                     uint64_t workspace_bytes, uint32_t out_width, const void *obj_feat, float *grad_obj, float input_pad, bool pad31,
                                     void *stream);
}
__device__ __forceinline__ void stage_pad31_bias(const _Float16 *__restrict__ W0, float pad, float *bias, uint32_t hidden) {
    if (threadIdx.x < hidden) {
        const uint32_t n = threadIdx.x, r = n & 31u, mt = n >> 5;
        const uint32_t h = (r >> 2) & 1u, reg = (r & 3u) + 4u * (r >> 3);
        bias[(mt * 2 + h) * 16 + reg] = (float)W0[(size_t)n * 32 + 31] * pad;
    }
}
__device__ __forceinline__ void stage_head_bias(const _Float16 *__restrict__ W0, const MlpHead &hd, float *bias, uint32_t hidden) {
    if (hd.obj) stage_obj_bias(W0, hd.obj, bias, hidden, hd.pad);
    else stage_pad31_bias(W0, hd.pad, bias, hidden);
}
__device__ __forceinline__ f16v ld_obj_bias(const float *bias, int mt, int h) {
    typedef float f4 __attribute__((ext_vector_type(4)));
    const f4 *p = reinterpret_cast<const f4 *>(bias + (mt * 2 + h) * 16);
    const f4 a = p[0], b = p[1], c = p[2], d = p[3];
    return f16v{a.x, a.y, a.z, a.w, b.x, b.y, b.z, b.w, c.x, c.y, c.z, c.w, d.x, d.y, d.z, d.w};
}
__device__ __forceinline__ void ld_head_raw(const _Float16 *__restrict__ hrows, uint64_t row, int h, u32x4 &v, uint32_t &nxt) {
    const uint32_t *p = reinterpret_cast<const uint32_t *>(hrows + row * 16) + 4 * h;
    v = *reinterpret_cast<const u32x4 *>(p);
    nxt = h == 0 ? p[4] : 0u;
}
__device__ __forceinline__ void ld_head_raw_all(const _Float16 *__restrict__ hrows, uint64_t row, int h, u32x4 &v, uint32_t &nxt) {
    const uint32_t *p = reinterpret_cast<const uint32_t *>(hrows + row * 16) + 4 * h;
    v = *reinterpret_cast<const u32x4 *>(p);
    nxt = p[h == 0 ? 4 : 3];
}
__device__ __forceinline__ h8 head_shift(const u32x4 v, uint32_t nxt) {
    const u32x4 r = {__builtin_amdgcn_alignbit(v.y, v.x, 16), __builtin_amdgcn_alignbit(v.z, v.y, 16), __builtin_amdgcn_alignbit(v.w, v.z, 16),
                     __builtin_amdgcn_alignbit(nxt, v.w, 16)};
    return __builtin_bit_cast(h8, r);
}
__device__ __forceinline__ h8 ld_head8(const _Float16 *__restrict__ hrows, const MlpHead &hd, uint64_t row, uint32_t kc, int h) {
    if (kc == 0) return *reinterpret_cast<const h8 *>(hd.ray_sh + (uint64_t)((uint32_t)row / hd.samples_per_ray) * 16 + 8 * h);
    u32x4 v; uint32_t nxt;
    ld_head_raw_all(hrows, row, h, v, nxt);
    return head_shift(v, h == 0 ? nxt : 0u);
}

template <int HIDDEN>
__device__ void stage_weights_fwd(const _Float16 *__restrict__ W, _Float16 *lds, uint32_t in_dim, uint32_t num_layers, bool with_out = true, uint32_t ld0 = 0) {
    constexpr int MT = (HIDDEN + 31) / 32, KC = HIDDEN / 16;
    const uint32_t KS0 = in_dim / 16;
    if (!ld0) ld0 = in_dim;
    const uint32_t n0 = MT * KS0, nh = (num_layers - 1) * MT * KC, total = n0 + nh + (with_out ? KC : 0);
    const _Float16 *Wh = W + (size_t)HIDDEN * ld0;
    const _Float16 *Wo = Wh + (size_t)(num_layers - 1) * HIDDEN * HIDDEN;
    for (uint32_t idx = threadIdx.x; idx < total * 64; idx += MLP_BLOCK) {
        const uint32_t f = idx >> 6, lane = idx & 63, r = lane & 31, h = lane >> 5;
        h8 v;
#pragma unroll
        for (int j = 0; j < 8; j++) v[j] = (_Float16)0;
        if (f < n0) {
            const uint32_t mt = f / KS0, kc = f % KS0, row = 32 * mt + r;
            if (row < HIDDEN) v = *reinterpret_cast<const h8 *>(W + (size_t)row * ld0 + 16 * kc + 8 * h);
        } else if (f < n0 + nh) {
            const uint32_t g = f - n0, l = g / (MT * KC), mt = (g / KC) % MT, kc = g % KC, row = 32 * mt + r;
            if (row < HIDDEN) {
                const _Float16 *p = Wh + (size_t)l * HIDDEN * HIDDEN + (size_t)row * HIDDEN + 16 * kc + 4 * h;
                const h4 lo = *reinterpret_cast<const h4 *>(p), hi = *reinterpret_cast<const h4 *>(p + 8);
#pragma unroll
                for (int j = 0; j < 4; j++) { v[j] = lo[j]; v[4 + j] = hi[j]; }
            }
        } else {
            const uint32_t kc = f - n0 - nh;
            if (r < 16) {
                const _Float16 *p = Wo + (size_t)r * HIDDEN + 16 * kc + 4 * h;
                const h4 lo = *reinterpret_cast<const h4 *>(p), hi = *reinterpret_cast<const h4 *>(p + 8);
#pragma unroll
                for (int j = 0; j < 4; j++) { v[j] = lo[j]; v[4 + j] = hi[j]; }
            }
        }
        *reinterpret_cast<h8 *>(lds + (size_t)f * 512 + lane * 8) = v;
    }
}

template <int HIDDEN>
__device__ void stage_weights_bwd(const _Float16 *__restrict__ W, _Float16 *lds, uint32_t in_dim, uint32_t num_layers, bool with_dx, bool head = false,
                                  uint32_t ld0 = 0) {
    constexpr int MT = (HIDDEN + 31) / 32, KC = HIDDEN / 16;
    const uint32_t MT0 = (in_dim + 31) / 32;
    if (!ld0) ld0 = in_dim;
    const uint32_t no = MT, nh = (num_layers - 1) * MT * KC, nx = with_dx ? MT0 * KC : 0, total = no + nh + nx;
    const _Float16 *Wh = W + (size_t)HIDDEN * ld0;
    const _Float16 *Wo = Wh + (size_t)(num_layers - 1) * HIDDEN * HIDDEN;
    for (uint32_t idx = threadIdx.x; idx < total * 64; idx += MLP_BLOCK) {
        const uint32_t f = idx >> 6, lane = idx & 63, r = lane & 31, h = lane >> 5;
        h8 v;
#pragma unroll
        for (int j = 0; j < 8; j++) v[j] = (_Float16)0;
        if (f < no) {
            const uint32_t i = 32 * f + r;
            if (i < HIDDEN) {
#pragma unroll
                for (int j = 0; j < 8; j++) v[j] = Wo[(size_t)(8 * h + j) * HIDDEN + i];
            }
        } else if (f < no + nh) {
            const uint32_t g = f - no, l = g / (MT * KC), mt = (g / KC) % MT, kc = g % KC, i = 32 * mt + r;
            if (i < HIDDEN) {
#pragma unroll
                for (int j = 0; j < 8; j++) v[j] = Wh[(size_t)l * HIDDEN * HIDDEN + (size_t)chain_k(kc, h, j) * HIDDEN + i];
            }
        } else {
            const uint32_t g = f - no - nh, mt0 = g / KC, kc = g % KC, i = 32 * mt0 + r;
            if (head) {
                if (i >= 17 && i < 32) {
#pragma unroll
                    for (int j = 0; j < 8; j++) v[j] = W[(size_t)chain_k(kc, h, j) * ld0 + (i - 1)];
                }
            } else if (i < in_dim) {
#pragma unroll
                for (int j = 0; j < 8; j++) v[j] = W[(size_t)chain_k(kc, h, j) * ld0 + i];
            }
        }
        *reinterpret_cast<h8 *>(lds + (size_t)f * 512 + lane * 8) = v;
    }
}

template <bool RELU>
__device__ __forceinline__ void store_tile(_Float16 *__restrict__ dst, uint32_t ld, uint64_t row, uint64_t nrows, uint32_t col0, uint32_t ncols,
                                           const f16v &acc, int h) {
    if (row >= nrows) return;
#pragma unroll
    for (int q = 0; q < 4; q++) {
        const uint32_t col = col0 + 8 * q + 4 * h;
        if (col < ncols) {
            h4 v;
#pragma unroll
            for (int e = 0; e < 4; e++) {
                _Float16 x = (_Float16)acc[4 * q + e];
                if (RELU) x = x > (_Float16)0 ? x : (_Float16)0;
                v[e] = x;
            }
            *reinterpret_cast<h4 *>(dst + row * ld + col) = v;
        }
    }
}

__device__ __forceinline__ void store_tile_act(_Float16 *__restrict__ dst, uint32_t ld, uint64_t row, uint64_t nrows, uint32_t col0, uint32_t ncols,
                                               const f16v &acc, int h, int act) {
    if (row >= nrows) return;
#pragma unroll
    for (int q = 0; q < 4; q++) {
        const uint32_t col = col0 + 8 * q + 4 * h;
        if (col < ncols) {
// ... 8 lines not shown
```

### focnerf_amd/csrc/raymarching.hip

```cpp
#include "common.h"
#include "occ_cell.h"
#include "sample_math.h"
#include "ragged.h"
#include <float.h>

#define RM_SQRT3 1.7320508075688772f
#define RM_RPI   0.3183098861837907f

__device__ __forceinline__ float rm_sign(float x) { return copysignf(1.0f, x); }

__device__ __forceinline__ void rm_near_far(float ox, float oy, float oz, float dx, float dy, float dz, float a0, float a1, float a2, float a3, float a4, float a5,
                                            float min_near, float &near_out, float &far_out) {
    const float rdx = 1 / dx, rdy = 1 / dy, rdz = 1 / dz;
    float near = (a0 - ox) * rdx, far = (a3 - ox) * rdx, t;
    if (near > far) { t = near; near = far; far = t; }
    float near_y = (a1 - oy) * rdy, far_y = (a4 - oy) * rdy;
    if (near_y > far_y) { t = near_y; near_y = far_y; far_y = t; }
    bool miss = (near > far_y || near_y > far);
    if (!miss) {
        if (near_y > near) near = near_y;
        if (far_y < far) far = far_y;
        float near_z = (a2 - oz) * rdz, far_z = (a5 - oz) * rdz;
        if (near_z > far_z) { t = near_z; near_z = far_z; far_z = t; }
        miss = (near > far_z || near_z > far);
        if (!miss) {
            if (near_z > near) near = near_z;
            if (far_z < far) far = far_z;
            if (near < min_near) near = min_near;
        }
    }
    near_out = miss ? FLT_MAX : near;
    far_out = miss ? FLT_MAX : far;
}

__global__ void __launch_bounds__(256) k_near_far_from_aabb(const float *__restrict__ rays_o, const float *__restrict__ rays_d,
                                     const float *__restrict__ aabb, uint32_t N, float min_near,
                                     float *__restrict__ nears, float *__restrict__ fars) {
    const float a0 = aabb[0], a1 = aabb[1], a2 = aabb[2], a3 = aabb[3], a4 = aabb[4], a5 = aabb[5];
    for (uint32_t n = blockIdx.x * blockDim.x + threadIdx.x; n < N; n += gridDim.x * blockDim.x) {
        float near, far;
        rm_near_far(rays_o[n * 3], rays_o[n * 3 + 1], rays_o[n * 3 + 2], rays_d[n * 3], rays_d[n * 3 + 1], rays_d[n * 3 + 2], a0, a1, a2, a3, a4, a5, min_near, near, far);
        nears[n] = near;
        fars[n] = far;
    }
}

__global__ void __launch_bounds__(256) k_sph_from_ray(const float *__restrict__ rays_o, const float *__restrict__ rays_d, float radius,
                               uint32_t N, float *__restrict__ coords) {
    for (uint32_t n = blockIdx.x * blockDim.x + threadIdx.x; n < N; n += gridDim.x * blockDim.x) {
        const float ox = rays_o[n * 3], oy = rays_o[n * 3 + 1], oz = rays_o[n * 3 + 2];
        const float dx = rays_d[n * 3], dy = rays_d[n * 3 + 1], dz = rays_d[n * 3 + 2];
        const float A = fmaf(dz, dz, fmaf(dy, dy, dx * dx));
        const float B = fmaf(oz, dz, fmaf(oy, dy, ox * dx));
        const float C = fmaf(-radius, radius, fmaf(oz, oz, fmaf(oy, oy, ox * ox)));
        const float t = (-B + sqrtf(fmaf(B, B, -(A * C)))) / A;
        const float x = fmaf(t, dx, ox), y = fmaf(t, dy, oy), z = fmaf(t, dz, oz);
        const float theta = atan2f(sqrtf(fmaf(z, z, x * x)), y);
        const float phi = atan2f(z, x);
        coords[n * 2] = fmaf(2 * theta, RM_RPI, -1.0f);
        coords[n * 2 + 1] = phi * RM_RPI;
    }
}

__global__ void __launch_bounds__(256) k_morton3D(const int32_t *__restrict__ coords, uint32_t N, int32_t *__restrict__ indices) {
    for (uint32_t n = blockIdx.x * blockDim.x + threadIdx.x; n < N; n += gridDim.x * blockDim.x)
        indices[n] = (int32_t)rm_morton3D((uint32_t)coords[n * 3], (uint32_t)coords[n * 3 + 1], (uint32_t)coords[n * 3 + 2]);
// ... 1202 lines not shown
```

### focnerf_amd/csrc/sample_math.h

```cpp
#pragma once
#include "common.h"

typedef _Float16 h8 __attribute__((ext_vector_type(8)));

__device__ __forceinline__ void foc_sh16(float x, float y, float z, float (&o)[16]) {
    const float xy = x * y, xz = x * z, yz = y * z, x2 = x * x, y2 = y * y, z2 = z * z;
    o[0] = 0.28209479177387814f;
    o[1] = -0.48860251190291987f * y;
    o[2] = 0.48860251190291987f * z;
    o[3] = -0.48860251190291987f * x;
    o[4] = 1.0925484305920792f * xy;
    o[5] = -1.0925484305920792f * yz;
    o[6] = 0.94617469575755997f * z2 - 0.31539156525251999f;
    o[7] = -1.0925484305920792f * xz;
    o[8] = 0.54627421529603959f * x2 - 0.54627421529603959f * y2;
    o[9] = 0.59004358992664352f * y * (-3.0f * x2 + y2);
    o[10] = 2.8906114426405538f * xy * z;
    o[11] = 0.45704579946446572f * y * (1.0f - 5.0f * z2);
    o[12] = 0.3731763325901154f * z * (5.0f * z2 - 3.0f);
    o[13] = 0.45704579946446572f * x * (1.0f - 5.0f * z2);
    o[14] = 1.4453057213202769f * z * (x2 - y2);
    o[15] = 0.59004358992664352f * x * (-x2 + 3.0f * y2);
}
__device__ __forceinline__ void foc_sh16_h(float x, float y, float z, h8 &lo, h8 &hi) {
    float sh[16];
    foc_sh16(x, y, z, sh);
#pragma unroll
    for (int k = 0; k < 8; k++) { lo[k] = foc_f2h(sh[k]); hi[k] = foc_f2h(sh[8 + k]); }
}

__device__ __forceinline__ float foc_sigmoid_h(float x) { return (float)(_Float16)(1.0f / (1.0f + expf(-x))); }

__device__ __forceinline__ float foc_clamp15(float x) { return x < -15.0f ? -15.0f : (x > 15.0f ? 15.0f : x); }
__device__ __forceinline__ float foc_trunc_exp_bwd(float x) { return expf(foc_clamp15(x)); }
__device__ __forceinline__ float foc_trunc_exp_bwd(float x, float e) {
    const float xc = foc_clamp15(x);
    return xc != x ? expf(xc) : e;
}
struct FocExp15 { float lo, hi; };
__device__ __forceinline__ FocExp15 foc_exp15() {
    float a = -15.0f, b = 15.0f;
    asm volatile("" : "+v"(a));
    asm volatile("" : "+v"(b));
    return FocExp15{expf(a), expf(b)};
}
__device__ __forceinline__ float foc_trunc_exp_bwd_of_sigma(float sigma, const FocExp15 &e) { return fminf(fmaxf(sigma, e.lo), e.hi); }

struct FocBg { float b0, b1, b2; };
__device__ __forceinline__ FocBg foc_bg(const float *__restrict__ bg_ray, float bg_scalar, uint32_t k) {
    return FocBg{bg_ray ? bg_ray[k * 3] : bg_scalar, bg_ray ? bg_ray[k * 3 + 1] : bg_scalar, bg_ray ? bg_ray[k * 3 + 2] : bg_scalar};
}
```

### focnerf_amd/field.py

```python
import os
from dataclasses import dataclass
from typing import Optional

import torch
from torch.autograd import Function
from torch.amp import custom_bwd, custom_fwd

from .backend import _gridencoder, _ffmlp
from .ffmlp import FFMLP, PackedMLP, single_pass_backward
from .gridencoder import GridEncoder, GridSpec


def fused_mlp(model, name):
    get = getattr(model, "fused_mlp", None)
    return get(name) if get is not None else getattr(model, name, None)


@dataclass(frozen=True)
class MlpShape:
    input_dim: int
    hidden_dim: int
    num_layers: int
    activation: int
    output_activation: int
# ... 114 lines not shown
    def __enter__(self):
        global _half_scope
        self._outer = _half_scope
        if _half_scope is None:
            _half_scope = {}
        return self

    def __exit__(self, *exc):
        global _half_scope
        _half_scope = self._outer
        return False


def _half_of(param):
    if param.dtype == torch.half:
        return param.contiguous()
    if _half_scope is None:
        return param.detach().to(torch.half).contiguous()
    hit = _half_scope.get(id(param))
    if hit is not None and hit[0] is param and hit[1].device == param.device:
        if hit[2] is not None and _raw_stream_of(param.device) != hit[3]:
            torch.cuda.current_stream(param.device).wait_event(hit[2])
        return hit[1]
    h = param.detach().to(torch.half).contiguous()
    ev = st = None
    if h.is_cuda:
        st = _raw_stream_of(h.device)
        ev = torch.cuda.Event()
        ev.record(torch.cuda.current_stream(h.device))
    _half_scope[id(param)] = (param, h, ev, st)
    return h


def scope_cached(key, owner, make):
    if _half_scope is None:
        return make()
    hit = _half_scope.get(key)
    if hit is not None and hit[0] is owner:
        if hit[2] is not None and _raw_stream_of(hit[1].device) != hit[3]:
            torch.cuda.current_stream(hit[1].device).wait_event(hit[2])
        return hit[1]
    v = make()
    ev = st = None
    if v.is_cuda:
        st = _raw_stream_of(v.device)
        ev = torch.cuda.Event()
        ev.record(torch.cuda.current_stream(v.device))
    _half_scope[key] = (owner, v, ev, st)
    return v


def _check_colour_branch(colour, B):
    cweights, shape, ray_sh, T, c_width, obj_feat = colour[:6]
    T = int(T)
    if not (ray_sh.dtype == torch.half and ray_sh.dim() == 2 and ray_sh.shape[1] == 16 and ray_sh.is_contiguous() and T > 0
            and B == ray_sh.shape[0] * T):
        raise RuntimeError(f"hashgrid_mlp colour branch: ray_sh must be a contiguous half [B / T, 16] tensor with B = {B}, T = {T}; got "
                           f"{tuple(ray_sh.shape)} {ray_sh.dtype}{'' if ray_sh.is_contiguous() else ' (strided)'}")
    if c_width not in (4, 16):
        raise RuntimeError(f"hashgrid_mlp colour branch: c_width must be 4 or 16, got {c_width}")
    if shape.input_dim not in (32, 48) or (obj_feat is not None) != (shape.input_dim == 48) or (obj_feat is not None and obj_feat.numel() != 16):
        raise RuntimeError(f"hashgrid_mlp colour branch: a {shape.input_dim}-wide colour input takes "
                           f"{'a 16-element object feature' if shape.input_dim == 48 else 'no object feature'}, got "
                           f"{'none' if obj_feat is None else f'{obj_feat.numel()} elements'}")
    if cweights.numel() != 64 * (shape.input_dim + 64 * (shape.num_layers - 1) + 16):
        raise RuntimeError(f"hashgrid_mlp colour branch: the colour weights hold {cweights.numel()} elements, a {shape.input_dim}-wide "
                           f"{shape.num_layers}-layer network has {64 * (shape.input_dim + 64 * (shape.num_layers - 1) + 16)}")


class _hashgrid_mlp(Function):
    @staticmethod
    @custom_fwd(device_type="cuda")
    def forward(ctx, x, embeddings, weights, offsets, grid, sigma, training, colour=None):
        x = x.contiguous().float()
        B = x.shape[0]
        if colour is not None:
            _check_colour_branch(colour, B)
        S, H, (gridtype, align_corners, interp) = grid.log2_scale, grid.base_resolution, grid.tail()
        L = offsets.shape[0] - 1
        emb = _half_of(embeddings)
        w = _half_of(weights)
        enc = torch.empty(L, B, 2, device=x.device, dtype=torch.half)
        ticket = _gridencoder.grid_encode_forward_counted(x, emb, offsets, enc, B, 3, 2, L, S, H, gridtype, align_corners, interp,
                                                          standalone=_gridencoder.precount_standalone()) if training else None
        if ticket is None:
            _gridencoder.grid_encode_forward(x, emb, offsets, enc, B, 3, 2, L, S, H, None, gridtype, align_corners, interp)
        h = torch.empty(B, 16, device=x.device, dtype=torch.half)
        c = None
        if colour is not None:
            from ._lib import ptr, stream_of, check
            cweights, cshape, ray_sh, T, c_width, obj_feat = colour[:6]
            pad = float(colour[6]) if len(colour) > 6 else 0.0
            wc = _half_of(cweights)
            obj16 = object_feature_half(obj_feat, "hashgrid_mlp colour branch")
            c = torch.empty(B, c_width, device=x.device, dtype=torch.half)
            args = (ptr(enc), ptr(w), sigma.num_layers, ptr(ray_sh), int(T), ptr(wc), int(cshape.num_layers), 64, int(sigma.activation), B, ptr(h),
                    ptr(c), int(c_width), ptr(obj16))
            fn, extra = pad_twin("foc_field_forward_train", pad, obj16 is not None)
            check(fn(*args, *extra, stream_of(enc)), "field_forward_train")
        else:
            _ffmlp.ffmlp_forward_planar(enc, w, B, sigma.input_dim, 16, sigma.hidden_dim, sigma.num_layers, sigma.activation, sigma.output_activation, h)
        if training:
            ctx.save_for_backward(x, emb, w, offsets, enc)
            ctx.cfg = (grid, sigma, B, L)
            ctx.ticket = ticket
        if c is None:
            return h
        ctx.mark_non_differentiable(c)
        ctx.set_materialize_grads(False)
        return h, c

    @staticmethod
    @custom_bwd(device_type="cuda")
    def backward(ctx, grad_h, _grad_c=None):
        x, emb, w, offsets, enc = ctx.saved_tensors
        grid, sigma, B, L = ctx.cfg
        if grad_h is None:
            return (None,) * 8
        grad_h = grad_h.contiguous().half()
        g_enc = torch.empty_like(enc)
        g_w = torch.empty_like(w)
        _ffmlp.ffmlp_backward_planar(grad_h, enc, w, B, sigma.input_dim, 16, sigma.hidden_dim, sigma.num_layers, sigma.activation,
                                     sigma.output_activation, True, g_enc, g_w)
        g_emb = torch.zeros_like(emb)
        _gridencoder.grid_encode_backward(g_enc, x, emb, offsets, g_emb, B, 3, 2, L, grid.log2_scale, grid.base_resolution, None, None, *grid.tail(),
                                          grad_bl=False, precount=ctx.ticket)
        return None, g_emb, g_w, None, None, None, None, None


@torch.no_grad()
def field_infer(model, xn, dirs, dir_div=1, dir_block=0, obj_feat=None):
    from ._lib import ptr, stream_of, check
    enc, sn, cn = model.encoder, fused_mlp(model, "sigma_net"), fused_mlp(model, "color_net")
    grid = enc.spec()
    xn = xn.contiguous().float()
    dirs = dirs.contiguous().float()
    M = xn.shape[0]
    L = enc.offsets.shape[0] - 1
    emb, ws, wc = _half_of(enc.embeddings), _half_of(sn.weights), _half_of(cn.weights)
    planes = torch.empty(L, M, 2, device=xn.device, dtype=torch.half)
    _gridencoder.grid_encode_forward(xn, emb, enc.offsets, planes, M, 3, 2, L, grid.log2_scale, grid.base_resolution, None, *grid.tail())
    sigma = torch.empty(M, dtype=torch.float32, device=xn.device)
    rgb = torch.empty(M, 3, dtype=torch.float32, device=xn.device)
    obj16 = None
    if getattr(model, "uses_object_feature", False):
        if obj_feat is None:
            raise RuntimeError("field_infer: an object-conditioned network needs its encoded object feature")
        obj16 = object_feature_half(obj_feat, "field_infer")
    args = (ptr(planes), 1, ptr(dirs), int(dir_div), int(dir_block), dirs.shape[0], ptr(ws), sn.num_layers, ptr(wc), cn.num_layers, 64, sn.activation, M,
            ptr(sigma), ptr(rgb), ptr(obj16))
    fn, extra = pad_twin("foc_nerf_field_inference", float(getattr(model, "colour_input_pad", 0.0)), obj16 is not None)
    check(fn(*args, *extra, stream_of(xn)), "nerf_field_inference")
    return sigma, rgb


def hashgrid_mlp(encoder, mlp, x, bound=1, colour=None):
# ... 9 lines not shown
```

### focnerf_amd/fixedstep.py

```python
import torch
from torch.autograd import Function

from . import raymarching
from ._lib import lib, ptr, stream_of, check
from .gridencoder import grid_encode


RAY_BLOCK = 64


def ray_block_default():
    import os
    return RAY_BLOCK if os.environ.get("FOC_RAY_BLOCK", str(RAY_BLOCK)) != "0" else 0


def blocked_rows(N, T, ray_block):
    return N * T if not ray_block else -(-N // ray_block) * ray_block * T


def fixed_sample(rays_o, rays_d, nears, fars, aabb, noise, T, bound, want_xyzs=False, want_ray_sh=False, ray_block=0):
    N = rays_o.shape[0]
    dev = rays_o.device
    rows = blocked_rows(N, T, ray_block)
    enc_in = torch.empty(rows, 3, dtype=torch.float32, device=dev)
    xyzs = torch.empty(rows, 3, dtype=torch.float32, device=dev) if want_xyzs else None
    ray_sh = torch.empty(N, 16, dtype=torch.float16, device=dev) if want_ray_sh else None
    check(lib.foc_fixed_sample(ptr(rays_o), ptr(rays_d), ptr(nears), ptr(fars), ptr(aabb), ptr(noise), N, T, float(bound), ptr(xyzs), ptr(enc_in),
                               ptr(ray_sh), int(ray_block), stream_of(rays_o)), "fixed_sample")
    if want_ray_sh:
        return enc_in, xyzs, ray_sh
    return enc_in, xyzs


def ray_sh_rows(rays_d):
    rays_d = rays_d.contiguous().float()
    N, dev = rays_d.shape[0], rays_d.device
    zeros, ones = torch.zeros(N, device=dev), torch.ones(N, device=dev)
    aabb = torch.tensor([-1., -1., -1., 1., 1., 1.], device=dev)
    return fixed_sample(torch.zeros_like(rays_d), rays_d, zeros, ones, aabb, None, 2, 1.0, want_ray_sh=True)[2]


class _density_head(Function):

    @staticmethod
    def forward(ctx, h, rays_d, nears, fars, noise, N, T, density_scale, obj_feat=None):
        from .field import object_feature_half
        h = h.contiguous()
        assert h.dtype == torch.float16 and h.shape == (N * T, 16)
        dev = h.device
        M = N * T
        sigma = torch.empty(M, dtype=torch.float32, device=dev)
        trans = torch.empty(M, dtype=torch.float32, device=dev)
        weights = torch.empty(M, dtype=torch.float32, device=dev)
        ws = torch.empty(N, dtype=torch.float32, device=dev)
        depth = torch.empty(N, dtype=torch.float32, device=dev)
        width = 32 if obj_feat is None else 48
        obj_feat = object_feature_half(obj_feat, "_density_head")
        cin = torch.empty(M, width, dtype=torch.float16, device=dev)
        check(lib.foc_fixed_head_forward(ptr(h), ptr(rays_d), ptr(nears), ptr(fars), ptr(noise), N, T, float(density_scale), ptr(sigma), ptr(trans),
                                         ptr(weights), ptr(ws), ptr(depth), ptr(cin), ptr(obj_feat), width, stream_of(h)), "fixed_head_forward")
        ctx.save_for_backward(h, sigma, trans, nears, fars, noise if noise is not None else torch.empty(0, device=dev))
        ctx.has_noise = noise is not None
        ctx.dims = (N, T, float(density_scale))
        ctx.width = width
# ... 30 lines not shown
        check(lib.foc_fixed_composite_forward(ptr(c), ptr(weights), ptr(bg_ray), float(bg_scalar), N, T, float(thresh), ptr(image), stream_of(c)),
              "fixed_composite_forward")
        ctx.bg_grad = bg_ray is not None and ctx.needs_input_grad[2]
        if ctx.bg_grad and weights_sum is None:
            raise RuntimeError("_fixed_composite: a background that needs a gradient needs weights_sum")
        empty = torch.empty(0, device=c.device)
        ctx.save_for_backward(c, weights, bg_ray if bg_ray is not None else empty, weights_sum.detach() if ctx.bg_grad else empty)
        ctx.has_bg = bg_ray is not None
        ctx.dims = (N, T, float(thresh), float(bg_scalar))
        return image

    @staticmethod
    def backward(ctx, g_image):
        c, weights, bg_ray, weights_sum = ctx.saved_tensors
        N, T, thresh, bg_scalar = ctx.dims
        bg_ray = bg_ray if ctx.has_bg else None
        g_image = g_image.contiguous().float()
        grad_c = torch.empty_like(c)
        grad_w = torch.empty_like(weights)
        check(lib.foc_fixed_composite_backward(ptr(g_image), ptr(c), ptr(weights), ptr(bg_ray), bg_scalar, N, T, thresh, ptr(grad_c), ptr(grad_w),
                                               stream_of(c)), "fixed_composite_backward")
        g_bg = g_image * (1 - weights_sum).unsqueeze(-1) if ctx.bg_grad else None
        return grad_c, grad_w, g_bg, None, None, None, None, None


_C_WIDTH = 4


class _render_tail(Function):

    @staticmethod
    def forward(ctx, h, cweights, ray_sh, nears, fars, noise, bg_ray, bg_scalar, N, T, density_scale, thresh, num_layers, activation, obj_feat=None,
                want_sumsq=False, c_pre=None, w16_pre=None, input_pad=0.0, want_dist=False):
        from .field import _half_of, pad_twin, object_feature_half
        h = h.contiguous()
        assert h.dtype == torch.float16 and h.shape == (N * T, 16)
        assert ray_sh.dtype == torch.float16 and ray_sh.shape == (N, 16) and ray_sh.is_contiguous()
        dev, M = h.device, N * T
        st = stream_of(h)
        w16 = w16_pre if w16_pre is not None else _half_of(cweights)
        obj16 = object_feature_half(obj_feat, "_render_tail")
        assert obj16 is None or w16.numel() == 64 * (48 + 64 * (int(num_layers) - 1) + 16)
        if c_pre is not None:
            assert c_pre.dtype == torch.float16 and c_pre.shape == (M, _C_WIDTH) and c_pre.is_contiguous()
            c = c_pre
        else:
            c = torch.empty(M, _C_WIDTH, dtype=torch.float16, device=dev)
            args = (ptr(h), ptr(ray_sh), T, ptr(w16), M, 64, int(num_layers), int(activation), ptr(c), _C_WIDTH, ptr(obj16))
            fn, extra = pad_twin("foc_color_head_forward", input_pad, obj16 is not None)
            check(fn(*args, *extra, st), "color_head_forward")
        sigma = torch.empty(M, dtype=torch.float32, device=dev)
        trans = torch.empty(M, dtype=torch.float32, device=dev)
        weights = torch.empty(M, dtype=torch.float32, device=dev)
        ws = torch.empty(N, dtype=torch.float32, device=dev)
        depth = torch.empty(N, dtype=torch.float32, device=dev)
        image = torch.empty(N, 3, dtype=torch.float32, device=dev)
        sumsq = torch.empty(N, dtype=torch.float32, device=dev) if want_sumsq else None
        tail = (ptr(h), ptr(c), ptr(nears), ptr(fars), ptr(noise), ptr(bg_ray), float(bg_scalar), N, T, float(density_scale), float(thresh), ptr(sigma),
                ptr(trans), ptr(weights), ptr(ws), ptr(depth), ptr(image), _C_WIDTH, ptr(sumsq))
        dist = wm = None
        if want_dist:
            dist, wm = torch.empty(N, dtype=torch.float32, device=dev), torch.empty(N, dtype=torch.float32, device=dev)
            check(lib.foc_fixed_tail_forward_dist(*tail, ptr(dist), ptr(wm), st), "fixed_tail_forward_dist")
        else:
            check(lib.foc_fixed_tail_forward(*tail, st), "fixed_tail_forward")
        empty = torch.empty(0, device=dev)
        ctx.bg_grad = bg_ray is not None and ctx.needs_input_grad[6]
        ctx.save_for_backward(h, w16, sigma, trans, weights, c, ray_sh, nears, fars, noise if noise is not None else empty,
                              bg_ray if bg_ray is not None else empty, obj16 if obj16 is not None else empty,
                              ws if ctx.bg_grad or want_dist else empty, wm if want_dist else empty)
        ctx.outputs = (bool(want_sumsq), bool(want_dist))
        ctx.flags = (noise is not None, bg_ray is not None, obj16 is not None, obj_feat.dtype if obj_feat is not None else None,
                     tuple(obj_feat.shape) if obj_feat is not None else None)
        ctx.dims = (N, T, float(density_scale), float(thresh), float(bg_scalar), int(num_layers), int(activation), float(input_pad))
        ctx.mark_non_differentiable(sigma, weights, c)
        ctx.set_materialize_grads(False)
        return (image, ws, depth, sigma, weights, c) + ((sumsq,) if want_sumsq else ()) + ((dist,) if want_dist else ())

    @staticmethod
    def backward(ctx, g_image, g_ws, g_depth, _g_sigma, _g_weights, _g_c, *g_extra):
        from .backend import _scratch
        from .field import pad_twin
        h, w16, sigma, trans, weights, c, ray_sh, nears, fars, noise, bg_ray, obj16, ws, wm = ctx.saved_tensors
        g_extra = list(g_extra)
        g_sumsq = g_extra.pop(0) if ctx.outputs[0] else None
        g_dist = g_extra.pop(0) if ctx.outputs[1] else None
        has_noise, has_bg, has_obj, obj_dtype, obj_shape = ctx.flags
        obj16 = obj16 if has_obj else None
        N, T, ds, thresh, bg_scalar, num_layers, activation, input_pad = ctx.dims
        noise = noise if has_noise else None
        bg_ray = bg_ray if has_bg else None
        dev, M = h.device, N * T
        st = stream_of(h)
        g_image = g_image.contiguous().float() if g_image is not None else torch.zeros(N, 3, dtype=torch.float32, device=dev)
        g_ws = g_ws.contiguous().float() if g_ws is not None else None
        g_depth = g_depth.contiguous().float() if g_depth is not None else None
        g_sumsq = g_sumsq.contiguous().float() if g_sumsq is not None else None
        grad_c = torch.empty_like(c)
        grad_h0 = torch.empty(M, dtype=torch.float16, device=dev)
        if g_dist is not None:
            g_dist = g_dist.contiguous().float()
            check(lib.foc_fixed_tail_backward_dist(ptr(g_image), ptr(g_ws), ptr(g_depth), ptr(c), ptr(sigma), ptr(trans), ptr(weights), ptr(ws), ptr(nears),
                                                   ptr(fars), ptr(noise), ptr(bg_ray), bg_scalar, N, T, ds, thresh, ptr(grad_c), ptr(grad_h0), _C_WIDTH,
                                                   ptr(g_sumsq), ptr(wm), None, ptr(g_dist), st), "fixed_tail_backward_dist")
        else:
            check(lib.foc_fixed_tail_backward(ptr(g_image), ptr(g_ws), ptr(g_depth), ptr(c), ptr(sigma), ptr(trans), ptr(weights), ptr(nears), ptr(fars),
                                              ptr(noise), ptr(bg_ray), bg_scalar, N, T, ds, thresh, ptr(grad_c), ptr(grad_h0), _C_WIDTH, ptr(g_sumsq), st),
                  "fixed_tail_backward")
        grad_h = torch.empty_like(h)
        g_w = torch.empty_like(w16)
        wsb = _scratch.get("ffmlp_ws", lib.foc_ffmlp_backward_workspace_bytes(48 if has_obj else 32, 64, num_layers), dev)
        g_obj32 = torch.empty(16, dtype=torch.float32, device=dev) if has_obj and ctx.needs_input_grad[14] else None
        args = (ptr(grad_c), ptr(h), ptr(ray_sh), T, ptr(grad_h0), ptr(w16), M, 64, num_layers, activation, ptr(grad_h), ptr(g_w), ptr(wsb),
                wsb.numel(), _C_WIDTH, ptr(obj16), ptr(g_obj32))
        fn, extra = pad_twin("foc_color_head_backward", input_pad, has_obj)
        check(fn(*args, *extra, st), "color_head_backward")
        g_obj = g_obj32.to(obj_dtype).view(obj_shape) if g_obj32 is not None else None
        g_bg = g_image * (1 - ws).unsqueeze(-1) if ctx.bg_grad else None
        return (grad_h, g_w, None, None, None, None, g_bg) + (None,) * 7 + (g_obj, None, None, None, None, None)


class _masked_norm(Function):

    @staticmethod
    def forward(ctx, sumsq, outside):
        crit = torch.sqrt((sumsq * outside).sum())
        ctx.save_for_backward(crit, outside)
        return crit

    @staticmethod
    def backward(ctx, g):
        crit, outside = ctx.saved_tensors
        coef = torch.where(crit > 0, g / (2 * crit), torch.zeros_like(crit))
        return outside * coef, None


def _unfused_distortion(weights, nears, fars, noise, N, T):
    from .loss import ray_distortion
    span = (fars - nears).unsqueeze(-1)
    z = span * torch.linspace(0.0, 1.0, T, device=weights.device).unsqueeze(0)
    if noise is not None:
        z = z + (noise.view(N, T) - 0.5) * (span / T)
    delta = torch.cat([z[:, 1:] - z[:, :-1], span / T], dim=-1)
    live = (fars > nears).unsqueeze(-1)
    zero = torch.zeros_like(z)
    return ray_distortion(torch.where(live, weights.view(N, T), zero), torch.where(live, z + 0.5 * delta, zero), torch.where(live, delta, zero))


def _background(bg_color, N, dev):
    if bg_color is None:
        return None, 1.0
    if torch.is_tensor(bg_color):
        if bg_color.numel() > 1:
            return bg_color.to(dev, torch.float32).reshape(-1, 3).expand(N, 3).contiguous(), 0.0
        return None, float(bg_color)
    return None, float(bg_color)


def render_fixed_steps(model, rays_o, rays_d, yolo_details=None, num_steps=512, bg_color=None, perturb=False, weight_thresh=1e-10,
                       return_fields=None, _out=None, distortion=False, **kwargs):
    import time
    if return_fields is None:
        return_fields = not model.training
    t_start = time.time()
    prefix = rays_o.shape[:-1]
    rays_o = rays_o.contiguous().view(-1, 3).float()
    rays_d = rays_d.contiguous().view(-1, 3).float()
    N, T = rays_o.shape[0], int(num_steps)
    dev = rays_o.device
    aabb = model.aabb_train if model.training else model.aabb_infer
    nears, fars = raymarching.near_far_from_aabb(rays_o, rays_d, aabb, model.min_near)
    noise = torch.rand(N * T, dtype=torch.float32, device=dev) if perturb else None
    from .field import field_plan, field_infer
    plan = field_plan(model)
    if getattr(model, "bg_radius", 0) > 0:
        bg_color = model._background_colour(rays_o, rays_d, bg_color)
    want_tail = plan.tail and model.training and torch.is_grad_enabled()
    fused_infer = not torch.is_grad_enabled() and plan.infer
    if distortion and not torch.is_grad_enabled():
        raise ValueError("render_fixed_steps: distortion=True needs the training route (gradients enabled): the inference paths form no "
                         "differentiable weights; call it under torch.enable_grad() with model.train()")
    rb = ray_block_default() if fused_infer else 0
    enc_in, _, ray_sh = fixed_sample(rays_o, rays_d, nears, fars, aabb, noise, T, model.bound, want_ray_sh=True) if want_tail else \
        fixed_sample(rays_o, rays_d, nears, fars, aabb, noise, T, model.bound, ray_block=rb) + (None,)

    if fused_infer:
        obj_feat = model.encode_object_feature(yolo_details, dev) if plan.uses_object_feature else None
        sigma, rgb = field_infer(model, enc_in, rays_d, dir_div=T, dir_block=rb, obj_feat=obj_feat)
        bg_ray, bg_scalar = _background(bg_color, N, dev)
        direct = (_out is not None and _out[0].dtype == torch.float32 and _out[1].dtype == torch.float32 and _out[0].is_contiguous()
                  and _out[1].is_contiguous() and _out[0].numel() == N and _out[1].numel() == 3 * N and _out[0].device == dev)
        depth, image = (_out[0].view(N), _out[1].view(N, 3)) if direct else (torch.empty(N, dtype=torch.float32, device=dev),
                                                                              torch.empty(N, 3, dtype=torch.float32, device=dev))
        weights_sum = torch.empty(N, dtype=torch.float32, device=dev)
        rgb_masked = densities = None
        if return_fields:
            if direct and len(_out) == 4 and all(t.dtype == torch.float32 and t.is_contiguous() and t.device == dev for t in _out[2:]) \
                    and _out[2].numel() == N * T and _out[3].numel() == 3 * N * T and rb:
                densities, rgb_masked = _out[2].view(N * T), _out[3].view(N * T, 3)
            else:
                rgb_masked = torch.empty(N * T, 3, dtype=torch.float32, device=dev)
                densities = torch.empty(N * T, dtype=torch.float32, device=dev) if rb else None
        check(lib.foc_fixed_render_inference(ptr(sigma), ptr(rgb), ptr(nears), ptr(fars), ptr(noise), ptr(bg_ray), float(bg_scalar), N, T,
                                             float(model.density_scale), float(weight_thresh), ptr(image), ptr(depth), ptr(weights_sum), ptr(rgb_masked),
                                             rb, ptr(densities), stream_of(sigma)), "fixed_render_inference")
        t_mid = time.time()
        results = {'depth': depth.view(*prefix), 'image': image.view(*prefix, 3), 'weights_sum': weights_sum, 'criterion_outside_mask': None,
                   'timing': [t_mid - t_start, time.time() - t_mid]}
        if return_fields:
            results['densities'] = (densities if rb else sigma).view(N, T, 1)
            results['rgbs'] = rgb_masked.view(N, T, 3)
        return results

    enc = model.encoder
    from .field import hashgrid_mlp, fused_mlp
    c_pre = obj_feat = None
    cweights = fused_mlp(model, "color_net").weights if want_tail else None
    with torch.autocast("cuda", dtype=torch.float16):
        if plan.uses_object_feature:
            obj_feat = model.encode_object_feature(yolo_details, dev)
        if plan.field:
            colour = wc16 = None
            if want_tail and plan.train_forward:
                from .field import _half_of
                wc16 = _half_of(cweights)
                colour = (wc16, plan.colour, ray_sh, T, _C_WIDTH, obj_feat, plan.colour_input_pad)
            h = hashgrid_mlp(enc, fused_mlp(model, "sigma_net"), enc_in, None, colour)
            if colour is not None:
                h, c_pre = h
        else:
            feats = grid_encode(enc_in, enc.embeddings, enc.offsets, enc.per_level_scale, enc.base_resolution, False, enc.gridtype_id,
                                enc.align_corners, enc.interp_id)
            h = fused_mlp(model, "sigma_net")(feats)
        if h.shape[1] != 16:
            raise RuntimeError("render_fixed_steps expects a 16-wide sigma head (1 + geo_feat_dim = 16)")
        fused_tail = want_tail
        want_crit = model.training and yolo_details is not None and yolo_details[0] is not None
        criterion_outside_mask = None
        if fused_tail:
            cn = fused_mlp(model, "color_net")
            bg_ray, bg_scalar = _background(bg_color, N, dev)
            outs = _render_tail.apply(h, cweights, ray_sh, nears, fars, noise, bg_ray, bg_scalar, N, T, model.density_scale, weight_thresh,
                                      cn.num_layers, cn.activation, obj_feat, want_crit and yolo_details[0].numel() == N, c_pre,
                                      wc16 if c_pre is not None else None, plan.colour_input_pad, *((True,) if distortion else ()))
            image, weights_sum, depth, sigma, weights, c = outs[:6]
            ray_dist = outs[-1] if distortion else None
            if len(outs) - bool(distortion) == 7:
                criterion_outside_mask = _masked_norm.apply(outs[6], (~yolo_details[0].reshape(N)).to(torch.float32))
        else:
            weights, weights_sum, depth, sigma, cin = _density_head.apply(h, rays_d, nears, fars, noise, N, T, model.density_scale, obj_feat)
            if plan.colour_input_pad != 0:
                cin = torch.cat([cin[:, :-1], cin.new_full((cin.shape[0], 1), plan.colour_input_pad)], dim=1)
            if distortion:
                ray_dist = _unfused_distortion(weights, nears, fars, noise, N, T)
        if want_crit and criterion_outside_mask is None:
            from .activation import trunc_exp
            criterion_outside_mask = torch.norm(trunc_exp(h[:, 0]).view(N, T)[~yolo_details[0].squeeze(0)] - 0)
        if not fused_tail:
            c = fused_mlp(model, "color_net").forward_padded(cin)
# ... 69 lines not shown
```

### include/focnerf.h

```cpp
#ifndef FOCNERF_H
#define FOCNERF_H

#include <stddef.h>
#include <stdint.h>

#ifdef __cplusplus
extern "C" {
#endif

#define FOC_OK            0
#define FOC_E_INVALID     1
#define FOC_E_DTYPE       2
#define FOC_E_LAUNCH      3

#define FOC_F32 0
#define FOC_F16 1

#define FOC_ABI_VERSION 2
int         foc_abi_version(void);
const char *foc_last_error(void);
int foc_set_option(const char *name, int value);
int foc_get_option(const char *name, int *value);
int foc_guard_pick_device(int stream_is_null, int stream_device, int pointer_device, int current_device);
const char *foc_arch(void);
// ... 206 lines not shown
                           uint32_t B, uint32_t hidden_dim, uint32_t num_layers, uint32_t activation,
                           void *outputs, uint32_t out_width, const void *obj_feat, void *stream);
int foc_color_head_backward(const void *grad, const void *h, const void *ray_sh, uint32_t samples_per_ray,
                            const void *grad_h0, const void *weights, uint32_t B, uint32_t hidden_dim,
                            uint32_t num_layers, uint32_t activation, void *grad_h, void *grad_weights,
                            void *workspace, uint64_t workspace_bytes, uint32_t out_width, const void *obj_feat, float *grad_obj, void *stream);
int foc_color_head_forward_pad(const void *h, const void *ray_sh, uint32_t samples_per_ray, const void *weights,
                               uint32_t B, uint32_t hidden_dim, uint32_t num_layers, uint32_t activation,
                               void *outputs, uint32_t out_width, const void *obj_feat, float input_pad, void *stream);
int foc_color_head_backward_pad(const void *grad, const void *h, const void *ray_sh, uint32_t samples_per_ray,
                                const void *grad_h0, const void *weights, uint32_t B, uint32_t hidden_dim,
                                uint32_t num_layers, uint32_t activation, void *grad_h, void *grad_weights,
                                void *workspace, uint64_t workspace_bytes, uint32_t out_width, const void *obj_feat, float *grad_obj,
                                float input_pad, void *stream);
int foc_color_head_forward_pad31(const void *h, const void *ray_sh, uint32_t samples_per_ray, const void *weights,
                                 uint32_t B, uint32_t hidden_dim, uint32_t num_layers, uint32_t activation,
                                 void *outputs, uint32_t out_width, const void *obj_feat, float input_pad, void *stream);
int foc_color_head_backward_pad31(const void *grad, const void *h, const void *ray_sh, uint32_t samples_per_ray,
                                  const void *grad_h0, const void *weights, uint32_t B, uint32_t hidden_dim,
                                  uint32_t num_layers, uint32_t activation, void *grad_h, void *grad_weights,
                                  void *workspace, uint64_t workspace_bytes, uint32_t out_width, const void *obj_feat, float *grad_obj,
                                  float input_pad, void *stream);

int foc_field_forward_train(const void *planes, const void *sigma_weights, uint32_t sigma_layers, const void *ray_sh, uint32_t samples_per_ray,
                            const void *color_weights, uint32_t color_layers, uint32_t hidden_dim, uint32_t activation, uint32_t B,
                            void *h, void *c, uint32_t out_width, const void *obj_feat, void *stream);
int foc_field_forward_train_pad(const void *planes, const void *sigma_weights, uint32_t sigma_layers, const void *ray_sh, uint32_t samples_per_ray,
                                const void *color_weights, uint32_t color_layers, uint32_t hidden_dim, uint32_t activation, uint32_t B,
                                void *h, void *c, uint32_t out_width, const void *obj_feat, float input_pad, void *stream);
int foc_field_forward_train_pad31(const void *planes, const void *sigma_weights, uint32_t sigma_layers, const void *ray_sh, uint32_t samples_per_ray,
                                  const void *color_weights, uint32_t color_layers, uint32_t hidden_dim, uint32_t activation, uint32_t B,
                                  void *h, void *c, uint32_t out_width, const void *obj_feat, float input_pad, void *stream);

int foc_allocate_splitk(uint64_t size);
int foc_free_splitk(void);


int foc_combine_select(const float *dens, const float *rgb, float *max_dens, float *best_rgb,
                       uint64_t n, void *stream);

int foc_combine_pack_keys(const float *dens, uint32_t rank, uint64_t *keys, uint64_t n, void *stream);
int foc_combine_unpack(const uint64_t *keys, uint32_t rank, const float *rgb,
                       float *max_dens, float *masked_rgb, uint64_t n, void *stream);

int foc_composite_fixed_steps(const float *sigmas, const float *rgbs, const float *nears,
                              const float *fars, uint32_t N, uint32_t T, float bg,
                              float *image4, float *depth, void *stream);

#define FOC_COMBINE_MAX_OBJECTS 16

int foc_combine_select_composite(const float *const *fields4, uint32_t K, const float *nears, const float *fars,
                                 uint32_t N, uint32_t T, const float *bgs, uint32_t n_bg, float *image4, float *depth,
                                 float *merged4, void *stream);

int foc_combine_select4(const float *field4, float *acc4, uint64_t n, void *stream);

int foc_combine_select_composite_attr(const float *const *fields4, uint32_t K, const uint8_t *const *id_planes,
                                      const uint32_t *ids, uint32_t n_obj, const float *nears, const float *fars,
                                      uint32_t N, uint32_t T, const float *bgs, uint32_t n_bg, float *image4, float *depth,
                                      float *merged4, float *obj_weights, float *obj_depth, int32_t *instance,
                                      uint8_t *winner, void *stream);

typedef struct FocCulledField {
    const uint64_t *mask;
    const uint32_t *offsets;
    const float *sigma_c;
    const float *rgb_c;
    uint32_t m_occ;
    float density_scale;
    float thresh;
    float sigma_gain;
} FocCulledField;
int foc_combine_select_composite_culled(const FocCulledField *objs, uint32_t K, uint32_t struct_bytes, const uint32_t *ids,
                                        uint32_t n_obj, const float *nears, const float *fars, uint32_t N, uint32_t T,
                                        const float *bgs, uint32_t n_bg, float *image4, float *depth, float *merged4,
                                        float *obj_weights, float *obj_depth, int32_t *instance, uint8_t *winner, void *stream);

int foc_combine_select4_ids(const float *field4, uint32_t id, float *acc4, uint8_t *acc_ids, uint64_t n, void *stream);

int foc_mo_select(const void *sigma_new, const void *feat_new, void *sigma_best, void *feat_best, uint64_t n,
                  uint32_t feat_width, uint32_t elem_bytes, void *stream);


int foc_fixed_sample(const float *rays_o, const float *rays_d, const float *nears, const float *fars,
                     const float *aabb, const float *noise, uint32_t N, uint32_t T, float bound,
                     float *xyzs, float *enc_in, void *ray_sh, uint32_t ray_block, void *stream);

int foc_fixed_head_forward(const void *h, const float *rays_d, const float *nears, const float *fars,
                           const float *noise, uint32_t N, uint32_t T, float density_scale,
                           float *sigma, float *trans, float *weights, float *weights_sum, float *depth,
                           void *cin, const void *obj_feat, uint32_t cin_width, void *stream);
int foc_fixed_head_backward(const void *h, const float *sigma, const float *trans, const float *nears,
                            const float *fars, const float *noise, const float *grad_w, const float *grad_ws,
                            const float *grad_depth, const void *grad_cin, uint32_t N, uint32_t T,
                            float density_scale, void *grad_h, uint32_t cin_width, void *stream);

int foc_fixed_tail_forward(const void *h, const void *c, const float *nears, const float *fars, const float *noise,
                           const float *bg_ray, float bg_scalar, uint32_t N, uint32_t T, float density_scale, float thresh,
                           float *sigma, float *trans, float *weights, float *weights_sum, float *depth, float *image,
                           uint32_t c_width, float *ray_sumsq, void *stream);
int foc_fixed_tail_backward(const float *grad_image, const float *grad_ws, const float *grad_depth, const void *c,
                            const float *sigma, const float *trans, const float *weights, const float *nears,
                            const float *fars, const float *noise, const float *bg_ray, float bg_scalar, uint32_t N,
                            uint32_t T, float density_scale, float thresh, void *grad_c, void *grad_h0, uint32_t c_width,
                            const float *grad_sumsq, void *stream);

int foc_occ_tail_forward(const void *h, const void *c, uint32_t c_width, const float *deltas, const int32_t *rays,
                         uint32_t M, uint32_t N, float T_thresh, float density_scale, const float *bg_ray, float bg_scalar,
                         const float *nears, const float *fars, float *weights_sum, float *image_raw, float *image,
                         float *depth, void *stream);
int foc_occ_tail_backward(const float *grad_image, const float *grad_ws, const void *h, const void *c, uint32_t c_width,
                          const float *deltas, const int32_t *rays, const int32_t *counter, const float *weights_sum,
                          const float *image_raw, uint32_t M, uint32_t N, float T_thresh, float density_scale,
                          const float *bg_ray, float bg_scalar, void *grad_c, void *grad_h0, void *stream);
int foc_occ_tail_forward_sumsq(const void *h, const void *c, uint32_t c_width, const float *deltas, const int32_t *rays,
                               uint32_t M, uint32_t N, float T_thresh, float density_scale, const float *bg_ray, float bg_scalar,
                               const float *nears, const float *fars, float *weights_sum, float *image_raw, float *image,
                               float *depth, float *ray_sumsq, void *stream);
int foc_occ_tail_backward_sumsq(const float *grad_image, const float *grad_ws, const void *h, const void *c, uint32_t c_width,
// ... 243 lines not shown
```

Before: 1.321 billion.

## Read fp32 MLP weights directly in kernels and fuse AABB near/far into sampling

Adds fp32-weight variants of the fused MLP forward and backward and of the color-head backward. These kernels read the master fp32 weight blob directly and write fp32 weight gradients, so the per-step fp16 weight casts and their copies can be skipped. It also adds a single-launch fixed sampler that computes the AABB near/far values inside the sampling kernel, replacing a separate near_far_from_aabb launch. The fp32 route is behind an option that defaults to 0 and a blob-route check, while the fused sampling is on by default for training. This adds many templated kernel variants and narrow shape requirements (input 32, hidden 64).

Result: faster. 1.342 billion (median of 6 runs) (+1.6%).

```diff
diff --git a/focnerf_amd/backend.py b/focnerf_amd/backend.py
--- a/focnerf_amd/backend.py
+++ b/focnerf_amd/backend.py
@@ -334,6 +334,16 @@
                                             ptr(grad_weights), ptr(ws), ws.numel(), stream_of(grad)), "ffmlp_backward_planar")
 
     @staticmethod
+    def ffmlp_backward_planar_w32(grad, inputs_planar, weights, B, input_dim, output_dim, hidden_dim, num_layers, activation, output_activation,
+                                  calc_grad_inputs, grad_inputs_planar, grad_weights):
+        ts = (grad, inputs_planar, grad_inputs_planar)
+        require_cuda(*ts, weights, grad_weights); _half(*ts); _f32(weights, grad_weights); _contig(*ts, weights, grad_weights)
+        ws = _scratch.get("ffmlp_ws", lib.foc_ffmlp_backward_workspace_bytes(input_dim, hidden_dim, num_layers), grad.device)
+        check(lib.foc_ffmlp_backward_planar_w32(ptr(grad), ptr(inputs_planar), ptr(weights), B, input_dim, output_dim, hidden_dim, num_layers,
+                                                activation, output_activation, int(bool(calc_grad_inputs)), ptr(grad_inputs_planar),
+                                                ptr(grad_weights), ptr(ws), ws.numel(), stream_of(grad)), "ffmlp_backward_planar_w32")
+
+    @staticmethod
     def allocate_splitk(size):
         check(lib.foc_allocate_splitk(int(size)), "allocate_splitk")
 
diff --git a/focnerf_amd/csrc/combine.hip b/focnerf_amd/csrc/combine.hip
--- a/focnerf_amd/csrc/combine.hip
+++ b/focnerf_amd/csrc/combine.hip
@@ -384,6 +384,7 @@
     {"FOC_MLP_BWD_FUSED", 1}, {"FOC_FIELD_FWD_FUSED", 1}, {"FOC_GB_MERGE_MAX_RES", 480}, {"FOC_GB_FACTORED", 1}, {"FOC_GB_TAIL_SPLIT", 16}, {"FOC_GRID_FUSE_SMALL", 1},
     {"FOC_GRID_PAIRS", 1}, {"FOC_GRID_FAST", 1}, {"FOC_MARCH_SERIAL", -1}, {"FOC_MARCH_RAYS_ROW_MAX", 131072}, {"FOC_OCC_MARCH_FORM", -1},
     {"FOC_OCC_SAMPLE_MAJOR", 1}, {"FOC_OCC_FIELD_PIECE", 1 << 23}, {"FOC_DETERMINISTIC", 0},
+    {"FOC_MLP_FP32_WEIGHTS", 0}, {"FOC_SAMPLE_AABB", 1},
 };
 static int foc_option_parse(int which, const char *text) {
     if (which == FOC_OPT_OCC_MARCH_FORM) {
diff --git a/focnerf_amd/csrc/common.h b/focnerf_amd/csrc/common.h
--- a/focnerf_amd/csrc/common.h
+++ b/focnerf_amd/csrc/common.h
@@ -28,6 +28,8 @@
     FOC_OPT_OCC_SAMPLE_MAJOR,
     FOC_OPT_OCC_FIELD_PIECE,
     FOC_OPT_DETERMINISTIC,
+    FOC_OPT_MLP_FP32_WEIGHTS,
+    FOC_OPT_SAMPLE_AABB,
     FOC_OPT_COUNT
 };
 int foc_opt(FocOpt which);
diff --git a/focnerf_amd/csrc/ffmlp.hip b/focnerf_amd/csrc/ffmlp.hip
--- a/focnerf_amd/csrc/ffmlp.hip
+++ b/focnerf_amd/csrc/ffmlp.hip
@@ -357,9 +357,9 @@
     }
 }
 
-template <int HIDDEN, int NL, int NB, bool RECOMP, int IMODE, bool RELU_CT, bool IN32 = false, bool LEAN = false>
+template <int HIDDEN, int NL, int NB, bool RECOMP, int IMODE, bool RELU_CT, bool IN32 = false, bool LEAN = false, typename WT = _Float16>
 __global__ void __launch_bounds__(MLP_BLOCK, 2) k_mlp_bwd_fused(const _Float16 *__restrict__ grad, const _Float16 *__restrict__ inputs,
-                                                             const _Float16 *__restrict__ weights, const _Float16 *__restrict__ fwd_buf,
+                                                             const WT *__restrict__ weights, const _Float16 *__restrict__ fwd_buf,
                                                              _Float16 *__restrict__ bwd_buf_arg, _Float16 *__restrict__ grad_inputs, float *__restrict__ ws,
                                                              uint32_t B, uint32_t in_dim, int relu_rt, uint32_t lds_w_halfs, MlpHead hd) {
     const int relu = RELU_CT ? 1 : relu_rt;
@@ -790,7 +790,7 @@
 
 template <int HIDDEN>
 __global__ void __launch_bounds__(1024) k_mlp_dw_reduce(const float *__restrict__ slots, uint32_t n_slots, uint32_t NL, uint32_t in_dim, uint32_t ld0,
-                                                        _Float16 *__restrict__ gw, float *__restrict__ wsb) {
+                                                        _Float16 *__restrict__ gw, float *__restrict__ wsb, float *__restrict__ gw32) {
     __shared__ float part[16][64];
     const uint32_t lane = threadIdx.x & 63, slice = threadIdx.x >> 6;
     const uint32_t s = blockIdx.x / 64, w = (blockIdx.x / 16) % 4, reg = blockIdx.x % 16;
@@ -820,12 +820,15 @@
         const uint64_t first = (uint64_t)HIDDEN * ld0, lsz = (uint64_t)HIDDEN * HIDDEN;
         const uint32_t fl = NL - s;
         const uint64_t off = (s == 0 ? first + (uint64_t)(NL - 1) * lsz : (fl == 0 ? 0 : first + (uint64_t)(fl - 1) * lsz)) + (uint64_t)o * (s == NL ? ld0 : IN) + i;
-        if (wsb) wsb[off] = v; else gw[off] = (_Float16)v;
-    }
-}
-
-__global__ void __launch_bounds__(256) k_mlp_dw_finalize_obj(const float *__restrict__ ws, _Float16 *__restrict__ gw, uint32_t n, uint32_t hidden,
-                                                             const _Float16 *__restrict__ W, const _Float16 *__restrict__ obj, float *__restrict__ grad_obj,
+        if (wsb) wsb[off] = v;
+        else if (gw32) gw32[off] = (float)(_Float16)v;
+        else gw[off] = (_Float16)v;
+    }
+}
+
+template <typename WT>
+__global__ void __launch_bounds__(256) k_mlp_dw_finalize_obj(const float *__restrict__ ws, WT *__restrict__ gw, uint32_t n, uint32_t hidden,
+                                                             const WT *__restrict__ W, const _Float16 *__restrict__ obj, float *__restrict__ grad_obj,
                                                              float pad) {
     const uint32_t n0 = hidden * HEAD_OBJ_LD;
     for (uint32_t i = blockIdx.x * 256 + threadIdx.x; i < n; i += gridDim.x * 256) {
@@ -834,11 +837,11 @@
             const uint32_t o = i / HEAD_OBJ_LD, col = i % HEAD_OBJ_LD;
             if (col >= 31) v = col < 47 ? ws[o * HEAD_OBJ_LD + 31] * (float)obj[col - 31] : (pad != 0.0f ? ws[o * HEAD_OBJ_LD + 31] * pad : 0.0f);
         }
-        gw[i] = (_Float16)v;
+        gw[i] = (WT)(_Float16)v;
     }
     if (blockIdx.x == 0 && threadIdx.x < 16 && grad_obj) {
         float a = 0.0f;
-        for (uint32_t o = 0; o < hidden; o++) a = fmaf((float)W[o * HEAD_OBJ_LD + 31 + threadIdx.x], ws[o * HEAD_OBJ_LD + 31], a);
+        for (uint32_t o = 0; o < hidden; o++) a = fmaf((float)w_h(W[o * HEAD_OBJ_LD + 31 + threadIdx.x]), ws[o * HEAD_OBJ_LD + 31], a);
         grad_obj[threadIdx.x] = a;
     }
 }
@@ -1132,19 +1135,49 @@
 }
 
 template <int HIDDEN, int NL>
+static size_t mlp_bwd_fused_lds(size_t lds_w, uint32_t in_dim, bool recomp, const MlpHead *head) {
+    constexpr int RW = 32, WD = (HIDDEN < 32 ? 32 : HIDDEN) + 8, MT = (HIDDEN + 31) / 32, KC = HIDDEN / 16;
+    const uint32_t WA = (in_dim > (uint32_t)HIDDEN ? in_dim : (uint32_t)(HIDDEN < 32 ? 32 : HIDDEN)) + 8;
+    return lds_w + (size_t)4 * RW * (WD + WA) * sizeof(_Float16) + (recomp ? (size_t)(MT * (in_dim / 16) + (NL - 1) * MT * KC) * 1024 : 0) +
+           (head && head_bias(*head) ? 256 : 0);
+}
+
+template <int HIDDEN, int NL, typename WT, typename K>
+static int mlp_bwd_fused_run(K kern, size_t lds_launch, size_t lds_w, const void *grad, const void *inputs, const void *weights, const void *fwd_buf, uint32_t B,
+                             uint32_t in_dim, int relu, void *bwd_buf, void *grad_inputs, void *grad_weights, float *ws, hipStream_t st, const MlpHead *head,
+                             float *grad_obj) {
+    constexpr int NB = 1, RW = 32 * NB;
+    constexpr bool W32 = sizeof(WT) == 4;
+    const bool has_obj = head && head->obj;
+    const uint32_t n_w = HIDDEN * ((has_obj ? HEAD_OBJ_LD : in_dim) + HIDDEN * (NL - 1) + 16);
+    const uint32_t grid = min(foc_persistent_grid(kern, MLP_BLOCK, lds_launch, foc_div_up(B, 4 * RW), 2u), MLP_DW_MAX_SLOTS);
+    float *slots = ws + mlp_dw_blob_floats(has_obj ? HEAD_OBJ_LD : in_dim, HIDDEN, NL);
+    hipLaunchKernelGGL(kern, dim3(grid), dim3(MLP_BLOCK), lds_launch, st, (const _Float16 *)grad, (const _Float16 *)inputs, (const WT *)weights,
+                       (const _Float16 *)fwd_buf, (_Float16 *)bwd_buf, (_Float16 *)grad_inputs, slots, B, in_dim, relu, (uint32_t)(lds_w / sizeof(_Float16)),
+                       head ? *head : MlpHead{nullptr, nullptr, 1u, 16u, nullptr, 0.0f});
+    FOC_CHECK_LAUNCH("ffmlp_backward(fused)");
+    hipLaunchKernelGGL((k_mlp_dw_reduce<HIDDEN>), dim3((NL + 1) * 64), dim3(1024), 0, st, (const float *)slots, grid, (uint32_t)NL, in_dim,
+                       has_obj ? (uint32_t)HEAD_OBJ_LD : in_dim, W32 ? (_Float16 *)nullptr : (_Float16 *)grad_weights, has_obj ? ws : (float *)nullptr,
+                       W32 ? (float *)grad_weights : (float *)nullptr);
+    FOC_CHECK_LAUNCH("ffmlp_backward(reduce)");
+    if (has_obj) {
+        hipLaunchKernelGGL(k_mlp_dw_finalize_obj<WT>, dim3(foc_grid_1d(n_w, 256)), dim3(256), 0, st, ws, (WT *)grad_weights, n_w, (uint32_t)HIDDEN,
+                           (const WT *)weights, head->obj, grad_obj, head->pad);
+        FOC_CHECK_LAUNCH("ffmlp_backward(finalize)");
+    }
+    return FOC_OK;
+}
+
+template <int HIDDEN, int NL>
 static int mlp_bwd_fused_launch(const void *grad, const void *inputs, const void *weights, const void *fwd_buf, uint32_t B, uint32_t in_dim, int relu,
                                 void *bwd_buf, void *grad_inputs, void *grad_weights, float *ws, int planar, hipStream_t st, const MlpHead *head = nullptr,
                                 float *grad_obj = nullptr) {
     FOC_REQUIRE(!planar || fwd_buf == nullptr, FOC_E_INVALID, "ffmlp_backward: planar inputs need the re-evaluating form (forward_buffer NULL)");
-    constexpr int NB = 1, RW = 32 * NB, WD = (HIDDEN < 32 ? 32 : HIDDEN) + 8;
+    constexpr int NB = 1;
     const bool dx = grad_inputs != nullptr;
     const size_t lds_w = mlp_bwd_lds<HIDDEN>(in_dim, NL, dx);
-    const uint32_t WA = (in_dim > (uint32_t)HIDDEN ? in_dim : (uint32_t)(HIDDEN < 32 ? 32 : HIDDEN)) + 8;
     const bool recomp = fwd_buf == nullptr;
-    constexpr int MT = (HIDDEN + 31) / 32, KC = HIDDEN / 16;
-    const bool has_obj = head && head->obj;
-    const size_t lds = lds_w + (size_t)4 * RW * (WD + WA) * sizeof(_Float16) + (recomp ? (size_t)(MT * (in_dim / 16) + (NL - 1) * MT * KC) * 1024 : 0) +
-                       (head && head_bias(*head) ? 256 : 0);
+    const size_t lds = mlp_bwd_fused_lds<HIDDEN, NL>(lds_w, in_dim, recomp, head);
     FOC_REQUIRE(lds <= 160 * 1024, FOC_E_INVALID, "ffmlp_backward: fused kernel needs %zu B of LDS", lds);
 #ifdef FOC_TIMING_ONE_WG
     const size_t lds_launch = lds < 84 * 1024 ? 84 * 1024 : lds;
@@ -1168,22 +1201,29 @@
                                                        : k_mlp_bwd_fused<HIDDEN, NL, NB, true, 2, false>);
     }
     else FOC_REQUIRE(!head, FOC_E_INVALID, "color_head_backward: hidden_dim must be 64 and num_layers 2 or 3");
-    const uint32_t n_w = HIDDEN * ((has_obj ? HEAD_OBJ_LD : in_dim) + HIDDEN * (NL - 1) + 16);
-    const uint32_t grid = min(foc_persistent_grid(kern, MLP_BLOCK, lds_launch, foc_div_up(B, 4 * RW), 2u), MLP_DW_MAX_SLOTS);
-    float *slots = ws + mlp_dw_blob_floats(has_obj ? HEAD_OBJ_LD : in_dim, HIDDEN, NL);
-    hipLaunchKernelGGL(kern, dim3(grid), dim3(MLP_BLOCK), lds_launch, st, (const _Float16 *)grad, (const _Float16 *)inputs, (const _Float16 *)weights,
-                       (const _Float16 *)fwd_buf, (_Float16 *)bwd_buf, (_Float16 *)grad_inputs, slots, B, in_dim, relu, (uint32_t)(lds_w / sizeof(_Float16)),
-                       head ? *head : MlpHead{nullptr, nullptr, 1u, 16u, nullptr, 0.0f});
-    FOC_CHECK_LAUNCH("ffmlp_backward(fused)");
-    hipLaunchKernelGGL((k_mlp_dw_reduce<HIDDEN>), dim3((NL + 1) * 64), dim3(1024), 0, st, (const float *)slots, grid, (uint32_t)NL, in_dim,
-                       has_obj ? (uint32_t)HEAD_OBJ_LD : in_dim, (_Float16 *)grad_weights, has_obj ? ws : (float *)nullptr);
-    FOC_CHECK_LAUNCH("ffmlp_backward(reduce)");
-    if (has_obj) {
-        hipLaunchKernelGGL(k_mlp_dw_finalize_obj, dim3(foc_grid_1d(n_w, 256)), dim3(256), 0, st, ws, (_Float16 *)grad_weights, n_w, (uint32_t)HIDDEN,
-                           (const _Float16 *)weights, head->obj, grad_obj, head->pad);
-        FOC_CHECK_LAUNCH("ffmlp_backward(finalize)");
-    }
-    return FOC_OK;
+    return mlp_bwd_fused_run<HIDDEN, NL, _Float16>(kern, lds_launch, lds_w, grad, inputs, weights, fwd_buf, B, in_dim, relu, bwd_buf, grad_inputs, grad_weights, ws, st,
+                                                   head, grad_obj);
+}
+
+template <int NL>
+static int mlp_bwd_fused_launch_w32(const void *grad, const void *inputs, const void *weights, uint32_t B, int relu, void *grad_inputs, void *grad_weights,
+                                    float *ws, hipStream_t st, const MlpHead *head, float *grad_obj) {
+    constexpr int HIDDEN = 64, NB = 1;
+    const uint32_t in_dim = 32;
+    const size_t lds_w = mlp_bwd_lds<HIDDEN>(in_dim, NL, true);
+    const size_t lds = mlp_bwd_fused_lds<HIDDEN, NL>(lds_w, in_dim, true, head);
+    FOC_REQUIRE(lds <= 160 * 1024, FOC_E_INVALID, "ffmlp_backward: fused kernel needs %zu B of LDS", lds);
+    if (!head) {
+        auto kern = relu ? k_mlp_bwd_fused<HIDDEN, NL, NB, true, 1, true, true, true, float> : k_mlp_bwd_fused<HIDDEN, NL, NB, true, 1, false, false, false, float>;
+        return mlp_bwd_fused_run<HIDDEN, NL, float>(kern, lds, lds_w, grad, inputs, weights, nullptr, B, in_dim, relu, nullptr, grad_inputs, grad_weights, ws, st,
+                                                    nullptr, nullptr);
+    }
+    if constexpr (NL >= 2 && NL <= 3) {
+        auto kern = relu ? k_mlp_bwd_fused<HIDDEN, NL, NB, true, 3, true, false, true, float> : k_mlp_bwd_fused<HIDDEN, NL, NB, true, 3, false, false, false, float>;
+        return mlp_bwd_fused_run<HIDDEN, NL, float>(kern, lds, lds_w, grad, inputs, weights, nullptr, B, in_dim, relu, nullptr, grad_inputs, grad_weights, ws, st, head,
+                                                    grad_obj);
+    }
+    return FOC_E_INVALID;
 }
 
 template <int HIDDEN>
@@ -1351,6 +1391,39 @@
     FocDeviceGuard foc_guard_(stream, grad);
     return mlp_bwd_entry(grad, inputs_planar, weights, nullptr, B, input_dim, output_dim, hidden_dim, num_layers, activation, output_activation,
                          calc_grad_inputs, nullptr, grad_inputs_planar, grad_weights, workspace, workspace_bytes, 1, stream);
+}
+
+int foc_ffmlp_backward_planar_w32(const void *grad, const void *inputs_planar, const float *weights, uint32_t B, uint32_t input_dim, uint32_t output_dim,
+                                  uint32_t hidden_dim, uint32_t num_layers, uint32_t activation, uint32_t output_activation, int calc_grad_inputs,
+                                  void *grad_inputs_planar, float *grad_weights, void *workspace, uint64_t workspace_bytes, void *stream) {
+    FocDeviceGuard foc_guard_(stream, grad);
+    const char *who = "ffmlp_backward_planar_w32";
+    int rc = mlp_check(who, B, input_dim, output_dim, hidden_dim, num_layers, activation, output_activation);
+    if (rc) return rc;
+    FOC_REQUIRE(hidden_dim == 64 && input_dim == 32 && num_layers <= 4, FOC_E_INVALID,
+                "%s: serves input_dim 32, hidden_dim 64 and 1..4 layers (got %u, %u, %u)", who, input_dim, hidden_dim, num_layers);
+    FOC_REQUIRE(activation == FOC_ACT_RELU || activation == FOC_ACT_NONE, FOC_E_INVALID, "%s: hidden activation must be relu(0) or none(6)", who);
+    FOC_REQUIRE(calc_grad_inputs && foc_opt(FOC_OPT_MLP_BWD_FUSED), FOC_E_INVALID,
+                "%s: runs the single-pass backward with input gradients only (calc_grad_inputs set, FOC_MLP_BWD_FUSED on)", who);
+    FOC_REQUIRE(grad_weights, FOC_E_INVALID, "%s: null pointer", who);
+    if (B == 0) {
+        const size_t n_w = (size_t)64 * (32 + (size_t)64 * (num_layers - 1) + 16);
+        if (foc_zero_async(grad_weights, n_w * sizeof(float), (hipStream_t)stream) != hipSuccess) { foc_set_error("%s: memset failed", who); return FOC_E_LAUNCH; }
+        return FOC_OK;
+    }
+    FOC_REQUIRE(grad && inputs_planar && weights && grad_inputs_planar && workspace, FOC_E_INVALID, "%s: null pointer", who);
+    FOC_REQUIRE(((uintptr_t)weights & 15u) == 0, FOC_E_INVALID, "%s: the fp32 weight blob must be 16-byte aligned", who);
+    FOC_REQUIRE(workspace_bytes >= foc_ffmlp_backward_workspace_bytes(32, 64, num_layers), FOC_E_INVALID,
+                "%s: workspace of %llu bytes, foc_ffmlp_backward_workspace_bytes(32, 64, %u) asks for %llu", who, (unsigned long long)workspace_bytes, num_layers,
+                (unsigned long long)foc_ffmlp_backward_workspace_bytes(32, 64, num_layers));
+    const int relu = activation == FOC_ACT_RELU;
+    hipStream_t st = (hipStream_t)stream;
+    switch (num_layers) {
+        case 1: return mlp_bwd_fused_launch_w32<1>(grad, inputs_planar, weights, B, relu, grad_inputs_planar, grad_weights, (float *)workspace, st, nullptr, nullptr);
+        case 2: return mlp_bwd_fused_launch_w32<2>(grad, inputs_planar, weights, B, relu, grad_inputs_planar, grad_weights, (float *)workspace, st, nullptr, nullptr);
+        case 3: return mlp_bwd_fused_launch_w32<3>(grad, inputs_planar, weights, B, relu, grad_inputs_planar, grad_weights, (float *)workspace, st, nullptr, nullptr);
+        default: return mlp_bwd_fused_launch_w32<4>(grad, inputs_planar, weights, B, relu, grad_inputs_planar, grad_weights, (float *)workspace, st, nullptr, nullptr);
+    }
 }
 
 int nerf_field_inference(const void *enc, int enc_planar, const float *dirs, uint32_t dir_div, uint32_t dir_block, uint32_t n_dirs,
@@ -1492,6 +1565,36 @@
                                workspace_bytes, out_width, obj_feat, grad_obj, input_pad, true, stream);
 }
 
+int foc_color_head_backward_w32(const void *grad, const void *h, const void *ray_sh, uint32_t samples_per_ray, const void *grad_h0, const float *weights,
+                                uint32_t B, uint32_t hidden_dim, uint32_t num_layers, uint32_t activation, void *grad_h, float *grad_weights, void *workspace,
+                                uint64_t workspace_bytes, uint32_t out_width, const void *obj_feat, float *grad_obj, void *stream) {
+    FocDeviceGuard foc_guard_(stream, grad);
+    const char *who = "color_head_backward_w32";
+    int rc = mlp_check(who, B, 32, 16, hidden_dim, num_layers, activation, 6);
+    if (rc) return rc;
+    FOC_REQUIRE(hidden_dim == 64 && (num_layers == 2 || num_layers == 3) && samples_per_ray >= 1, FOC_E_INVALID,
+                "%s: hidden_dim must be 64 and num_layers 2 or 3 (got %u, %u)", who, hidden_dim, num_layers);
+    FOC_REQUIRE(out_width == 4, FOC_E_INVALID, "%s: out_width must be 4, the [B,4] logit gradients of the training tail (got %u)", who, out_width);
+    FOC_REQUIRE(activation == FOC_ACT_RELU || activation == FOC_ACT_NONE, FOC_E_INVALID, "%s: hidden activation must be relu(0) or none(6)", who);
+    FOC_REQUIRE(grad_weights, FOC_E_INVALID, "%s: null pointer", who);
+    const uint32_t ld0 = obj_feat ? HEAD_OBJ_LD : 32u;
+    if (B == 0) {
+        const size_t n_w = (size_t)64 * (ld0 + (size_t)64 * (num_layers - 1) + 16);
+        if (foc_zero_async(grad_weights, n_w * sizeof(float), (hipStream_t)stream) != hipSuccess) { foc_set_error("%s: memset failed", who); return FOC_E_LAUNCH; }
+        if (grad_obj && foc_zero_async(grad_obj, 16 * sizeof(float), (hipStream_t)stream) != hipSuccess) { foc_set_error("%s: memset failed", who); return FOC_E_LAUNCH; }
+        return FOC_OK;
+    }
+    FOC_REQUIRE(grad && h && ray_sh && weights && grad_h && workspace, FOC_E_INVALID, "%s: null pointer", who);
+    FOC_REQUIRE(((uintptr_t)weights & 15u) == 0, FOC_E_INVALID, "%s: the fp32 weight blob must be 16-byte aligned", who);
+    FOC_REQUIRE(workspace_bytes >= foc_ffmlp_backward_workspace_bytes(ld0, 64, num_layers), FOC_E_INVALID,
+                "%s: workspace of %llu bytes, foc_ffmlp_backward_workspace_bytes(%u, 64, %u) asks for %llu", who, (unsigned long long)workspace_bytes, ld0, num_layers,
+                (unsigned long long)foc_ffmlp_backward_workspace_bytes(ld0, 64, num_layers));
+    const MlpHead hd{(const _Float16 *)ray_sh, (const _Float16 *)grad_h0, samples_per_ray, out_width, (const _Float16 *)obj_feat, 0.0f};
+    const int relu = activation == FOC_ACT_RELU;
+    if (num_layers == 2) return mlp_bwd_fused_launch_w32<2>(grad, h, weights, B, relu, grad_h, grad_weights, (float *)workspace, (hipStream_t)stream, &hd, grad_obj);
+    return mlp_bwd_fused_launch_w32<3>(grad, h, weights, B, relu, grad_h, grad_weights, (float *)workspace, (hipStream_t)stream, &hd, grad_obj);
+}
+
 int foc_allocate_splitk(uint64_t size) { (void)size; return FOC_OK; }
 int foc_free_splitk(void) { return FOC_OK; }
 
diff --git a/focnerf_amd/csrc/field_fwd.hip b/focnerf_amd/csrc/field_fwd.hip
--- a/focnerf_amd/csrc/field_fwd.hip
+++ b/focnerf_amd/csrc/field_fwd.hip
@@ -11,9 +11,9 @@
 #ifndef FF_MIN_WAVES
 #define FF_MIN_WAVES 2
 #endif
-template <int NLS, int NLC, bool RELU>
-__global__ void __launch_bounds__(MLP_BLOCK, FF_MIN_WAVES) k_field_fwd_train(const _Float16 *__restrict__ planes, const _Float16 *__restrict__ w_sigma,
-                                                               const _Float16 *__restrict__ w_color, _Float16 *__restrict__ h_out,
+template <int NLS, int NLC, bool RELU, typename WT>
+__global__ void __launch_bounds__(MLP_BLOCK, FF_MIN_WAVES) k_field_fwd_train(const _Float16 *__restrict__ planes, const WT *__restrict__ w_sigma,
+                                                               const WT *__restrict__ w_color, _Float16 *__restrict__ h_out,
                                                                _Float16 *__restrict__ c_out, uint32_t B, MlpHead hd) {
     constexpr int HIDDEN = 64, MT = 2, KC = 4, KS0 = 2;
     constexpr int FS = MT * KS0 + (NLS - 1) * MT * KC + KC;
@@ -140,28 +140,31 @@
     }
 }
 
-template <int NLS, int NLC, bool RELU>
+template <int NLS, int NLC, bool RELU, typename WT>
 static int ff_launch(const void *planes, const void *w_sigma, const void *w_color, void *h, void *c, uint32_t B, const MlpHead &hd, hipStream_t st) {
-    auto kern = k_field_fwd_train<NLS, NLC, RELU>;
+    auto kern = k_field_fwd_train<NLS, NLC, RELU, WT>;
     const size_t lds = (size_t)((4 + (NLS - 1) * 8 + 4) + (4 + (NLC - 1) * 8 + 4)) * 1024 + 256;
     const uint32_t grid = foc_persistent_grid(kern, MLP_BLOCK, lds, foc_div_up(foc_div_up(B, 32), MLP_WAVES));
-    hipLaunchKernelGGL(kern, dim3(grid), dim3(MLP_BLOCK), lds, st, (const _Float16 *)planes, (const _Float16 *)w_sigma, (const _Float16 *)w_color,
+    hipLaunchKernelGGL(kern, dim3(grid), dim3(MLP_BLOCK), lds, st, (const _Float16 *)planes, (const WT *)w_sigma, (const WT *)w_color,
                        (_Float16 *)h, (_Float16 *)c, B, hd);
     FOC_CHECK_LAUNCH("field_forward_train");
     return FOC_OK;
 }
 
 template <int NLS, int NLC>
-static int ff_launch_act(const void *planes, const void *w_sigma, const void *w_color, void *h, void *c, uint32_t B, int relu, const MlpHead &hd, hipStream_t st) {
-    return relu ? ff_launch<NLS, NLC, true>(planes, w_sigma, w_color, h, c, B, hd, st) : ff_launch<NLS, NLC, false>(planes, w_sigma, w_color, h, c, B, hd, st);
-}
-
-int field_forward_train(const void *planes, const void *sigma_weights, uint32_t sigma_layers, const void *ray_sh, uint32_t samples_per_ray,
-                        const void *color_weights, uint32_t color_layers, uint32_t hidden_dim, uint32_t activation, uint32_t B, void *h, void *c,
-                        uint32_t out_width, const void *obj_feat, float input_pad, bool pad31, void *stream) {
+static int ff_launch_act(const void *planes, const void *w_sigma, const void *w_color, void *h, void *c, uint32_t B, int relu, bool w32, const MlpHead &hd, hipStream_t st) {
+    if (w32) return relu ? ff_launch<NLS, NLC, true, float>(planes, w_sigma, w_color, h, c, B, hd, st) : ff_launch<NLS, NLC, false, float>(planes, w_sigma, w_color, h, c, B, hd, st);
+    return relu ? ff_launch<NLS, NLC, true, _Float16>(planes, w_sigma, w_color, h, c, B, hd, st) : ff_launch<NLS, NLC, false, _Float16>(planes, w_sigma, w_color, h, c, B, hd, st);
+}
+
+static int field_forward_train_any(const void *planes, const void *sigma_weights, uint32_t sigma_layers, const void *ray_sh, uint32_t samples_per_ray,
+                                   const void *color_weights, uint32_t color_layers, uint32_t hidden_dim, uint32_t activation, uint32_t B, void *h, void *c,
+                                   uint32_t out_width, const void *obj_feat, float input_pad, bool pad31, bool w32, void *stream) {
     FocDeviceGuard foc_guard_(stream, planes);
     if (B == 0) return FOC_OK;
     FOC_REQUIRE(planes && sigma_weights && ray_sh && color_weights && h && c, FOC_E_INVALID, "field_forward_train: null pointer");
+    FOC_REQUIRE(!w32 || ((((uintptr_t)sigma_weights | (uintptr_t)color_weights) & 15u) == 0), FOC_E_INVALID,
+                "field_forward_train_w32: the fp32 weight blobs must be 16-byte aligned");
     FOC_REQUIRE(hidden_dim == 64 && samples_per_ray >= 1, FOC_E_INVALID, "field_forward_train: hidden_dim must be 64 (got %u), samples_per_ray >= 1", hidden_dim);
     FOC_REQUIRE(activation == FOC_ACT_RELU || activation == FOC_ACT_NONE, FOC_E_INVALID, "field_forward_train: hidden activation must be relu(0) or none(6)");
     FOC_REQUIRE(out_width == 16 || out_width == 4, FOC_E_INVALID, "field_forward_train: out_width must be 16 or 4 (got %u)", out_width);
@@ -171,16 +174,30 @@
     const int relu = activation == FOC_ACT_RELU;
     hipStream_t st = (hipStream_t)stream;
     switch (sigma_layers * 10 + color_layers) {
-        case 12: return ff_launch_act<1, 2>(planes, sigma_weights, color_weights, h, c, B, relu, hd, st);
-        case 13: return ff_launch_act<1, 3>(planes, sigma_weights, color_weights, h, c, B, relu, hd, st);
-        case 22: return ff_launch_act<2, 2>(planes, sigma_weights, color_weights, h, c, B, relu, hd, st);
-        case 23: return ff_launch_act<2, 3>(planes, sigma_weights, color_weights, h, c, B, relu, hd, st);
-        case 33: return ff_launch_act<3, 3>(planes, sigma_weights, color_weights, h, c, B, relu, hd, st);
+        case 12: return ff_launch_act<1, 2>(planes, sigma_weights, color_weights, h, c, B, relu, w32, hd, st);
+        case 13: return ff_launch_act<1, 3>(planes, sigma_weights, color_weights, h, c, B, relu, w32, hd, st);
+        case 22: return ff_launch_act<2, 2>(planes, sigma_weights, color_weights, h, c, B, relu, w32, hd, st);
+        case 23: return ff_launch_act<2, 3>(planes, sigma_weights, color_weights, h, c, B, relu, w32, hd, st);
+        case 33: return ff_launch_act<3, 3>(planes, sigma_weights, color_weights, h, c, B, relu, w32, hd, st);
         default: foc_set_error("field_forward_train: layer counts (%u, %u) are not built (1/2, 1/3, 2/2, 2/3, 3/3)", sigma_layers, color_layers); return FOC_E_INVALID;
     }
 }
 
+int field_forward_train(const void *planes, const void *sigma_weights, uint32_t sigma_layers, const void *ray_sh, uint32_t samples_per_ray,
+                        const void *color_weights, uint32_t color_layers, uint32_t hidden_dim, uint32_t activation, uint32_t B, void *h, void *c,
+                        uint32_t out_width, const void *obj_feat, float input_pad, bool pad31, void *stream) {
+    return field_forward_train_any(planes, sigma_weights, sigma_layers, ray_sh, samples_per_ray, color_weights, color_layers, hidden_dim, activation, B, h, c,
+                                   out_width, obj_feat, input_pad, pad31, false, stream);
+}
+
 extern "C" {
+
+int foc_field_forward_train_w32(const void *planes, const float *sigma_weights, uint32_t sigma_layers, const void *ray_sh, uint32_t samples_per_ray,
+                                const float *color_weights, uint32_t color_layers, uint32_t hidden_dim, uint32_t activation, uint32_t B, void *h, void *c,
+                                uint32_t out_width, const void *obj_feat, void *stream) {
+    return field_forward_train_any(planes, sigma_weights, sigma_layers, ray_sh, samples_per_ray, color_weights, color_layers, hidden_dim, activation, B, h, c,
+                                   out_width, obj_feat, 0.0f, false, true, stream);
+}
 
 int foc_field_forward_train(const void *planes, const void *sigma_weights, uint32_t sigma_layers, const void *ray_sh, uint32_t samples_per_ray,
                             const void *color_weights, uint32_t color_layers, uint32_t hidden_dim, uint32_t activation, uint32_t B, void *h, void *c,
diff --git a/focnerf_amd/csrc/fixedstep.hip b/focnerf_amd/csrc/fixedstep.hip
--- a/focnerf_amd/csrc/fixedstep.hip
+++ b/focnerf_amd/csrc/fixedstep.hip
@@ -1,6 +1,7 @@
 #include "common.h"
 #include "fs_common.h"
 #include <float.h>
+#include <type_traits>
 
 __global__ void __launch_bounds__(256) k_fs_sample(const float *__restrict__ rays_o, const float *__restrict__ rays_d, const float *__restrict__ nears,
                                                    const float *__restrict__ fars, const float *__restrict__ aabb, const float *__restrict__ noise,
@@ -34,6 +35,56 @@
             dst[0] = lo; dst[1] = hi;
         }
     }
+}
+
+struct FsXyz { float x, y, z; };
+__global__ void __launch_bounds__(256) k_fs_sample_aabb(const float *__restrict__ rays_o, const float *__restrict__ rays_d, const float *__restrict__ aabb,
+                                                        const float *__restrict__ noise, uint32_t N, uint32_t T, float min_near, float bound,
+                                                        float *__restrict__ nears, float *__restrict__ fars, float *__restrict__ enc_in,
+                                                        _Float16 *__restrict__ ray_sh) {
+    const uint32_t lane = threadIdx.x & 63;
+    const uint32_t n = blockIdx.x * 4 + (threadIdx.x >> 6);
+    if (n >= N) return;
+    const FsBox box = fs_box(aabb);
+    const float two_b = 2 * bound;
+    const float ox = rays_o[n * 3], oy = rays_o[n * 3 + 1], oz = rays_o[n * 3 + 2];
+    const float dx = rays_d[n * 3], dy = rays_d[n * 3 + 1], dz = rays_d[n * 3 + 2];
+    float near, far;
+    rm_near_far(ox, oy, oz, dx, dy, dz, box.a0, box.a1, box.a2, box.a3, box.a4, box.a5, min_near, near, far);
+    if (lane == 0) {
+        nears[n] = near;
+        fars[n] = far;
+        if (ray_sh) {
+            h8 lo, hi;
+            foc_sh16_h(dx, dy, dz, lo, hi);
+            h8 *dst = reinterpret_cast<h8 *>(ray_sh + (uint64_t)n * 16);
+            dst[0] = lo; dst[1] = hi;
+        }
+    }
+    const FsGeom g = fs_geom_of(near, far, T);
+    const uint64_t row0 = (uint64_t)n * T;
+    auto walk = [&](auto jitter_c) {
+        constexpr bool JITTER = decltype(jitter_c)::value;
+        for (uint32_t i0 = 0; i0 < T; i0 += 256) {
+            float u[4] = {0.0f, 0.0f, 0.0f, 0.0f};
+            if constexpr (JITTER) {
+#pragma unroll
+                for (int k = 0; k < 4; k++) u[k] = noise[row0 + min(i0 + 64 * k + lane, T - 1)];
+            }
+#pragma unroll
+            for (int k = 0; k < 4; k++) {
+                const uint32_t i = i0 + 64 * k + lane;
+                if (i < T) {
+                    const float z = fs_zu(g, i, T, JITTER, u[k]);
+                    float x, y, w;
+                    fs_point(ox, oy, oz, dx, dy, dz, z, box, x, y, w);
+                    *reinterpret_cast<FsXyz *>(enc_in + (row0 + i) * 3) = FsXyz{fs_norm(x, bound, two_b), fs_norm(y, bound, two_b), fs_norm(w, bound, two_b)};
+                }
+            }
+        }
+    };
+    if (noise) walk(std::true_type{});
+    else walk(std::false_type{});
 }
 
 __global__ void __launch_bounds__(256) k_fs_head_fwd(const _Float16 *__restrict__ h, const float *__restrict__ rays_d, const float *__restrict__ nears,
@@ -405,6 +456,20 @@
     return FOC_OK;
 }
 
+int foc_fixed_sample_aabb(const float *rays_o, const float *rays_d, const float *aabb, const float *noise, uint32_t N, uint32_t T, float min_near,
+                          float bound, float *nears, float *fars, float *enc_in, void *ray_sh, void *stream) {
+    FocDeviceGuard foc_guard_(stream, rays_o);
+    if (N == 0) return FOC_OK;
+    FOC_REQUIRE(rays_o && rays_d && aabb && nears && fars && enc_in, FOC_E_INVALID, "fixed_sample_aabb: null pointer");
+    FOC_REQUIRE(T >= 2, FOC_E_INVALID, "fixed_sample_aabb: T must be >= 2");
+    FOC_REQUIRE(T <= (1u << 30), FOC_E_INVALID, "fixed_sample_aabb: T must be <= 2^30 (got %u)", T);
+    FOC_REQUIRE(N <= (1u << 30), FOC_E_INVALID, "fixed_sample_aabb: N must be <= 2^30 (got %u)", N);
+    hipLaunchKernelGGL(k_fs_sample_aabb, dim3(foc_div_up(N, 4)), dim3(256), 0, (hipStream_t)stream, rays_o, rays_d, aabb, noise, N, T, min_near, bound,
+                       nears, fars, enc_in, (_Float16 *)ray_sh);
+    FOC_CHECK_LAUNCH("fixed_sample_aabb");
+    return FOC_OK;
+}
+
 int foc_fixed_head_forward(const void *h, const float *rays_d, const float *nears, const float *fars, const float *noise, uint32_t N, uint32_t T,
                            float density_scale, float *sigma, float *trans, float *weights, float *weights_sum, float *depth, void *cin,
                            const void *obj_feat, uint32_t cin_width, void *stream) {
diff --git a/focnerf_amd/csrc/fs_common.h b/focnerf_amd/csrc/fs_common.h
--- a/focnerf_amd/csrc/fs_common.h
+++ b/focnerf_amd/csrc/fs_common.h
@@ -9,13 +9,16 @@
     return (uint64_t)(n / FS_RAY_BLOCK) * FS_RAY_BLOCK * T + (uint64_t)i * FS_RAY_BLOCK + n % FS_RAY_BLOCK;
 }
 
-__device__ __forceinline__ FsGeom fs_geom(const float *__restrict__ nears, const float *__restrict__ fars, uint32_t n, uint32_t T) {
+__device__ __forceinline__ FsGeom fs_geom_of(float near, float far, uint32_t T) {
     FsGeom g;
-    g.near = nears[n]; g.far = fars[n];
+    g.near = near; g.far = far;
     g.span = g.far - g.near;
     g.sample_dist = g.span / (float)T;
     g.step = 1.0f / (float)(T - 1);
     return g;
+}
+__device__ __forceinline__ FsGeom fs_geom(const float *__restrict__ nears, const float *__restrict__ fars, uint32_t n, uint32_t T) {
+    return fs_geom_of(nears[n], fars[n], T);
 }
 __device__ __forceinline__ float fs_z0(const FsGeom &g, uint32_t i, uint32_t T) {
     const float lin = (i < T / 2) ? (g.step * (float)i) : fmaf(-g.step, (float)(T - 1 - i), 1.0f);
diff --git a/focnerf_amd/csrc/mlp_common.h b/focnerf_amd/csrc/mlp_common.h
--- a/focnerf_amd/csrc/mlp_common.h
+++ b/focnerf_amd/csrc/mlp_common.h
@@ -20,6 +20,19 @@
 
 __device__ __forceinline__ int acc_row(int reg, int h) { return (reg & 3) + 8 * (reg >> 2) + 4 * h; }
 __device__ __forceinline__ int chain_k(int kc, int h, int j) { return 16 * kc + 8 * (j >> 2) + 4 * h + (j & 3); }
+
+__device__ __forceinline__ _Float16 w_h(_Float16 v) { return v; }
+__device__ __forceinline__ _Float16 w_h(float v) { return (_Float16)v; }
+__device__ __forceinline__ h4 ld_w4(const _Float16 *p) { return *reinterpret_cast<const h4 *>(p); }
+__device__ __forceinline__ h4 ld_w4(const float *p) {
+    const float4 a = *reinterpret_cast<const float4 *>(p);
+    return h4{(_Float16)a.x, (_Float16)a.y, (_Float16)a.z, (_Float16)a.w};
+}
+__device__ __forceinline__ h8 ld_w8(const _Float16 *p) { return *reinterpret_cast<const h8 *>(p); }
+__device__ __forceinline__ h8 ld_w8(const float *p) {
+    const float4 a = *reinterpret_cast<const float4 *>(p), b = *reinterpret_cast<const float4 *>(p + 4);
+    return h8{(_Float16)a.x, (_Float16)a.y, (_Float16)a.z, (_Float16)a.w, (_Float16)b.x, (_Float16)b.y, (_Float16)b.z, (_Float16)b.w};
+}
 
 __device__ __forceinline__ f16v mfma16(const h8 a, const h8 b, const f16v c) {
     return __builtin_amdgcn_mfma_f32_32x32x16_f16(a, b, c, 0, 0, 0);
@@ -80,14 +93,15 @@
 __device__ __forceinline__ uint32_t head_ld0(const MlpHead &hd) { return hd.obj ? HEAD_OBJ_LD : 32u; }
 __host__ __device__ __forceinline__ bool head_bias(const MlpHead &hd) { return hd.obj != nullptr || hd.pad != 0.0f; }
 
-__device__ __forceinline__ void stage_obj_bias(const _Float16 *__restrict__ W0, const _Float16 *__restrict__ obj, float *bias, uint32_t hidden, float pad) {
+template <typename WT>
+__device__ __forceinline__ void stage_obj_bias(const WT *__restrict__ W0, const _Float16 *__restrict__ obj, float *bias, uint32_t hidden, float pad) {
     if (threadIdx.x < hidden) {
         const uint32_t n = threadIdx.x, r = n & 31u, mt = n >> 5;
         const uint32_t h = (r >> 2) & 1u, reg = (r & 3u) + 4u * (r >> 3);
         float a = 0.0f;
 #pragma unroll
-        for (int j = 0; j < 16; j++) a = fmaf((float)W0[(size_t)n * HEAD_OBJ_LD + 31 + j], (float)obj[j], a);
-        if (pad != 0.0f) a = fmaf((float)W0[(size_t)n * HEAD_OBJ_LD + 47], pad, a);
+        for (int j = 0; j < 16; j++) a = fmaf((float)w_h(W0[(size_t)n * HEAD_OBJ_LD + 31 + j]), (float)obj[j], a);
+        if (pad != 0.0f) a = fmaf((float)w_h(W0[(size_t)n * HEAD_OBJ_LD + 47]), pad, a);
         bias[(mt * 2 + h) * 16 + reg] = a;
     }
 }
@@ -116,14 +130,16 @@
                                      uint64_t workspace_bytes, uint32_t out_width, const void *obj_feat, float *grad_obj, float input_pad, bool pad31,
                                      void *stream);
 }
-__device__ __forceinline__ void stage_pad31_bias(const _Float16 *__restrict__ W0, float pad, float *bias, uint32_t hidden) {
+template <typename WT>
+__device__ __forceinline__ void stage_pad31_bias(const WT *__restrict__ W0, float pad, float *bias, uint32_t hidden) {
     if (threadIdx.x < hidden) {
         const uint32_t n = threadIdx.x, r = n & 31u, mt = n >> 5;
         const uint32_t h = (r >> 2) & 1u, reg = (r & 3u) + 4u * (r >> 3);
-        bias[(mt * 2 + h) * 16 + reg] = (float)W0[(size_t)n * 32 + 31] * pad;
-    }
-}
-__device__ __forceinline__ void stage_head_bias(const _Float16 *__restrict__ W0, const MlpHead &hd, float *bias, uint32_t hidden) {
+        bias[(mt * 2 + h) * 16 + reg] = (float)w_h(W0[(size_t)n * 32 + 31]) * pad;
+    }
+}
+template <typename WT>
+__device__ __forceinline__ void stage_head_bias(const WT *__restrict__ W0, const MlpHead &hd, float *bias, uint32_t hidden) {
     if (hd.obj) stage_obj_bias(W0, hd.obj, bias, hidden, hd.pad);
     else stage_pad31_bias(W0, hd.pad, bias, hidden);
 }
@@ -155,14 +171,14 @@
     return head_shift(v, h == 0 ? nxt : 0u);
 }
 
-template <int HIDDEN>
-__device__ void stage_weights_fwd(const _Float16 *__restrict__ W, _Float16 *lds, uint32_t in_dim, uint32_t num_layers, bool with_out = true, uint32_t ld0 = 0) {
+template <int HIDDEN, typename WT = _Float16>
+__device__ void stage_weights_fwd(const WT *__restrict__ W, _Float16 *lds, uint32_t in_dim, uint32_t num_layers, bool with_out = true, uint32_t ld0 = 0) {
     constexpr int MT = (HIDDEN + 31) / 32, KC = HIDDEN / 16;
     const uint32_t KS0 = in_dim / 16;
     if (!ld0) ld0 = in_dim;
     const uint32_t n0 = MT * KS0, nh = (num_layers - 1) * MT * KC, total = n0 + nh + (with_out ? KC : 0);
-    const _Float16 *Wh = W + (size_t)HIDDEN * ld0;
-    const _Float16 *Wo = Wh + (size_t)(num_layers - 1) * HIDDEN * HIDDEN;
+    const WT *Wh = W + (size_t)HIDDEN * ld0;
+    const WT *Wo = Wh + (size_t)(num_layers - 1) * HIDDEN * HIDDEN;
     for (uint32_t idx = threadIdx.x; idx < total * 64; idx += MLP_BLOCK) {
         const uint32_t f = idx >> 6, lane = idx & 63, r = lane & 31, h = lane >> 5;
         h8 v;
@@ -170,20 +186,20 @@
         for (int j = 0; j < 8; j++) v[j] = (_Float16)0;
         if (f < n0) {
             const uint32_t mt = f / KS0, kc = f % KS0, row = 32 * mt + r;
-            if (row < HIDDEN) v = *reinterpret_cast<const h8 *>(W + (size_t)row * ld0 + 16 * kc + 8 * h);
+            if (row < HIDDEN) v = ld_w8(W + (size_t)row * ld0 + 16 * kc + 8 * h);
         } else if (f < n0 + nh) {
             const uint32_t g = f - n0, l = g / (MT * KC), mt = (g / KC) % MT, kc = g % KC, row = 32 * mt + r;
             if (row < HIDDEN) {
-                const _Float16 *p = Wh + (size_t)l * HIDDEN * HIDDEN + (size_t)row * HIDDEN + 16 * kc + 4 * h;
-                const h4 lo = *reinterpret_cast<const h4 *>(p), hi = *reinterpret_cast<const h4 *>(p + 8);
+                const WT *p = Wh + (size_t)l * HIDDEN * HIDDEN + (size_t)row * HIDDEN + 16 * kc + 4 * h;
+                const h4 lo = ld_w4(p), hi = ld_w4(p + 8);
 #pragma unroll
                 for (int j = 0; j < 4; j++) { v[j] = lo[j]; v[4 + j] = hi[j]; }
             }
         } else {
             const uint32_t kc = f - n0 - nh;
             if (r < 16) {
-                const _Float16 *p = Wo + (size_t)r * HIDDEN + 16 * kc + 4 * h;
-                const h4 lo = *reinterpret_cast<const h4 *>(p), hi = *reinterpret_cast<const h4 *>(p + 8);
+                const WT *p = Wo + (size_t)r * HIDDEN + 16 * kc + 4 * h;
+                const h4 lo = ld_w4(p), hi = ld_w4(p + 8);
 #pragma unroll
                 for (int j = 0; j < 4; j++) { v[j] = lo[j]; v[4 + j] = hi[j]; }
             }
@@ -192,15 +208,15 @@
     }
 }
 
-template <int HIDDEN>
-__device__ void stage_weights_bwd(const _Float16 *__restrict__ W, _Float16 *lds, uint32_t in_dim, uint32_t num_layers, bool with_dx, bool head = false,
+template <int HIDDEN, typename WT = _Float16>
+__device__ void stage_weights_bwd(const WT *__restrict__ W, _Float16 *lds, uint32_t in_dim, uint32_t num_layers, bool with_dx, bool head = false,
                                   uint32_t ld0 = 0) {
     constexpr int MT = (HIDDEN + 31) / 32, KC = HIDDEN / 16;
     const uint32_t MT0 = (in_dim + 31) / 32;
     if (!ld0) ld0 = in_dim;
     const uint32_t no = MT, nh = (num_layers - 1) * MT * KC, nx = with_dx ? MT0 * KC : 0, total = no + nh + nx;
-    const _Float16 *Wh = W + (size_t)HIDDEN * ld0;
-    const _Float16 *Wo = Wh + (size_t)(num_layers - 1) * HIDDEN * HIDDEN;
+    const WT *Wh = W + (size_t)HIDDEN * ld0;
+    const WT *Wo = Wh + (size_t)(num_layers - 1) * HIDDEN * HIDDEN;
     for (uint32_t idx = threadIdx.x; idx < total * 64; idx += MLP_BLOCK) {
         const uint32_t f = idx >> 6, lane = idx & 63, r = lane & 31, h = lane >> 5;
         h8 v;
@@ -210,24 +226,24 @@
             const uint32_t i = 32 * f + r;
             if (i < HIDDEN) {
 #pragma unroll
-                for (int j = 0; j < 8; j++) v[j] = Wo[(size_t)(8 * h + j) * HIDDEN + i];
+                for (int j = 0; j < 8; j++) v[j] = w_h(Wo[(size_t)(8 * h + j) * HIDDEN + i]);
             }
         } else if (f < no + nh) {
             const uint32_t g = f - no, l = g / (MT * KC), mt = (g / KC) % MT, kc = g % KC, i = 32 * mt + r;
             if (i < HIDDEN) {
 #pragma unroll
-                for (int j = 0; j < 8; j++) v[j] = Wh[(size_t)l * HIDDEN * HIDDEN + (size_t)chain_k(kc, h, j) * HIDDEN + i];
+                for (int j = 0; j < 8; j++) v[j] = w_h(Wh[(size_t)l * HIDDEN * HIDDEN + (size_t)chain_k(kc, h, j) * HIDDEN + i]);
             }
         } else {
             const uint32_t g = f - no - nh, mt0 = g / KC, kc = g % KC, i = 32 * mt0 + r;
             if (head) {
                 if (i >= 17 && i < 32) {
 #pragma unroll
-                    for (int j = 0; j < 8; j++) v[j] = W[(size_t)chain_k(kc, h, j) * ld0 + (i - 1)];
+                    for (int j = 0; j < 8; j++) v[j] = w_h(W[(size_t)chain_k(kc, h, j) * ld0 + (i - 1)]);
                 }
             } else if (i < in_dim) {
 #pragma unroll
-                for (int j = 0; j < 8; j++) v[j] = W[(size_t)chain_k(kc, h, j) * ld0 + i];
+                for (int j = 0; j < 8; j++) v[j] = w_h(W[(size_t)chain_k(kc, h, j) * ld0 + i]);
             }
         }
         *reinterpret_cast<h8 *>(lds + (size_t)f * 512 + lane * 8) = v;
diff --git a/focnerf_amd/csrc/raymarching.hip b/focnerf_amd/csrc/raymarching.hip
--- a/focnerf_amd/csrc/raymarching.hip
+++ b/focnerf_amd/csrc/raymarching.hip
@@ -8,30 +8,6 @@
 #define RM_RPI   0.3183098861837907f
 
 __device__ __forceinline__ float rm_sign(float x) { return copysignf(1.0f, x); }
-
-__device__ __forceinline__ void rm_near_far(float ox, float oy, float oz, float dx, float dy, float dz, float a0, float a1, float a2, float a3, float a4, float a5,
-                                            float min_near, float &near_out, float &far_out) {
-    const float rdx = 1 / dx, rdy = 1 / dy, rdz = 1 / dz;
-    float near = (a0 - ox) * rdx, far = (a3 - ox) * rdx, t;
-    if (near > far) { t = near; near = far; far = t; }
-    float near_y = (a1 - oy) * rdy, far_y = (a4 - oy) * rdy;
-    if (near_y > far_y) { t = near_y; near_y = far_y; far_y = t; }
-    bool miss = (near > far_y || near_y > far);
-    if (!miss) {
-        if (near_y > near) near = near_y;
-        if (far_y < far) far = far_y;
-        float near_z = (a2 - oz) * rdz, far_z = (a5 - oz) * rdz;
-        if (near_z > far_z) { t = near_z; near_z = far_z; far_z = t; }
-        miss = (near > far_z || near_z > far);
-        if (!miss) {
-            if (near_z > near) near = near_z;
-            if (far_z < far) far = far_z;
-            if (near < min_near) near = min_near;
-        }
-    }
-    near_out = miss ? FLT_MAX : near;
-    far_out = miss ? FLT_MAX : far;
-}
 
 __global__ void __launch_bounds__(256) k_near_far_from_aabb(const float *__restrict__ rays_o, const float *__restrict__ rays_d,
                                      const float *__restrict__ aabb, uint32_t N, float min_near,
diff --git a/focnerf_amd/csrc/sample_math.h b/focnerf_amd/csrc/sample_math.h
--- a/focnerf_amd/csrc/sample_math.h
+++ b/focnerf_amd/csrc/sample_math.h
@@ -1,5 +1,6 @@
 #pragma once
 #include "common.h"
+#include <float.h>
 
 typedef _Float16 h8 __attribute__((ext_vector_type(8)));
 
@@ -50,3 +51,27 @@
 __device__ __forceinline__ FocBg foc_bg(const float *__restrict__ bg_ray, float bg_scalar, uint32_t k) {
     return FocBg{bg_ray ? bg_ray[k * 3] : bg_scalar, bg_ray ? bg_ray[k * 3 + 1] : bg_scalar, bg_ray ? bg_ray[k * 3 + 2] : bg_scalar};
 }
+
+__device__ __forceinline__ void rm_near_far(float ox, float oy, float oz, float dx, float dy, float dz, float a0, float a1, float a2, float a3, float a4, float a5,
+                                            float min_near, float &near_out, float &far_out) {
+    const float rdx = 1 / dx, rdy = 1 / dy, rdz = 1 / dz;
+    float near = (a0 - ox) * rdx, far = (a3 - ox) * rdx, t;
+    if (near > far) { t = near; near = far; far = t; }
+    float near_y = (a1 - oy) * rdy, far_y = (a4 - oy) * rdy;
+    if (near_y > far_y) { t = near_y; near_y = far_y; far_y = t; }
+    bool miss = (near > far_y || near_y > far);
+    if (!miss) {
+        if (near_y > near) near = near_y;
+        if (far_y < far) far = far_y;
+        float near_z = (a2 - oz) * rdz, far_z = (a5 - oz) * rdz;
+        if (near_z > far_z) { t = near_z; near_z = far_z; far_z = t; }
+        miss = (near > far_z || near_z > far);
+        if (!miss) {
+            if (near_z > near) near = near_z;
+            if (far_z < far) far = far_z;
+            if (near < min_near) near = min_near;
+        }
+    }
+    near_out = miss ? FLT_MAX : near;
+    far_out = miss ? FLT_MAX : far;
+}
diff --git a/focnerf_amd/field.py b/focnerf_amd/field.py
--- a/focnerf_amd/field.py
+++ b/focnerf_amd/field.py
@@ -170,6 +170,12 @@
     return h
 
 
+def fp32_blob_route(*blobs):
+    from ._lib import get_option
+    return (all(isinstance(w, torch.nn.Parameter) and w.dtype == torch.float32 and w.is_cuda and w.is_contiguous() and w.data_ptr() % 16 == 0 for w in blobs)
+            and get_option("FOC_MLP_FP32_WEIGHTS") != 0 and get_option("FOC_MLP_BWD_FUSED") != 0)
+
+
 def scope_cached(key, owner, make):
     if _half_scope is None:
         return make()
@@ -217,7 +223,9 @@
         S, H, (gridtype, align_corners, interp) = grid.log2_scale, grid.base_resolution, grid.tail()
         L = offsets.shape[0] - 1
         emb = _half_of(embeddings)
-        w = _half_of(weights)
+        w32 = bool(training and colour is not None and (float(colour[6]) if len(colour) > 6 else 0.0) == 0.0
+                   and fp32_blob_route(weights, colour[0]))
+        w = weights.detach() if w32 else _half_of(weights)
         enc = torch.empty(L, B, 2, device=x.device, dtype=torch.half)
         ticket = _gridencoder.grid_encode_forward_counted(x, emb, offsets, enc, B, 3, 2, L, S, H, gridtype, align_corners, interp,
                                                           standalone=_gridencoder.precount_standalone()) if training else None
@@ -226,15 +234,15 @@
         h = torch.empty(B, 16, device=x.device, dtype=torch.half)
         c = None
         if colour is not None:
-            from ._lib import ptr, stream_of, check
+            from ._lib import lib, ptr, stream_of, check
             cweights, cshape, ray_sh, T, c_width, obj_feat = colour[:6]
             pad = float(colour[6]) if len(colour) > 6 else 0.0
-            wc = _half_of(cweights)
+            wc = cweights.detach() if w32 else _half_of(cweights)
             obj16 = object_feature_half(obj_feat, "hashgrid_mlp colour branch")
             c = torch.empty(B, c_width, device=x.device, dtype=torch.half)
             args = (ptr(enc), ptr(w), sigma.num_layers, ptr(ray_sh), int(T), ptr(wc), int(cshape.num_layers), 64, int(sigma.activation), B, ptr(h),
                     ptr(c), int(c_width), ptr(obj16))
-            fn, extra = pad_twin("foc_field_forward_train", pad, obj16 is not None)
+            fn, extra = (lib.foc_field_forward_train_w32, ()) if w32 else pad_twin("foc_field_forward_train", pad, obj16 is not None)
             check(fn(*args, *extra, stream_of(enc)), "field_forward_train")
         else:
             _ffmlp.ffmlp_forward_planar(enc, w, B, sigma.input_dim, 16, sigma.hidden_dim, sigma.num_layers, sigma.activation, sigma.output_activation, h)
@@ -242,6 +250,7 @@
             ctx.save_for_backward(x, emb, w, offsets, enc)
             ctx.cfg = (grid, sigma, B, L)
             ctx.ticket = ticket
+            ctx.w32 = w32
         if c is None:
             return h
         ctx.mark_non_differentiable(c)
@@ -258,8 +267,8 @@
         grad_h = grad_h.contiguous().half()
         g_enc = torch.empty_like(enc)
         g_w = torch.empty_like(w)
-        _ffmlp.ffmlp_backward_planar(grad_h, enc, w, B, sigma.input_dim, 16, sigma.hidden_dim, sigma.num_layers, sigma.activation,
-                                     sigma.output_activation, True, g_enc, g_w)
+        (_ffmlp.ffmlp_backward_planar_w32 if ctx.w32 else _ffmlp.ffmlp_backward_planar)(
+            grad_h, enc, w, B, sigma.input_dim, 16, sigma.hidden_dim, sigma.num_layers, sigma.activation, sigma.output_activation, True, g_enc, g_w)
         g_emb = torch.zeros_like(emb)
         _gridencoder.grid_encode_backward(g_enc, x, emb, offsets, g_emb, B, 3, 2, L, grid.log2_scale, grid.base_resolution, None, None, *grid.tail(),
                                           grad_bl=False, precount=ctx.ticket)
diff --git a/focnerf_amd/fixedstep.py b/focnerf_amd/fixedstep.py
--- a/focnerf_amd/fixedstep.py
+++ b/focnerf_amd/fixedstep.py
@@ -30,6 +30,18 @@
     if want_ray_sh:
         return enc_in, xyzs, ray_sh
     return enc_in, xyzs
+
+
+def fixed_sample_aabb(rays_o, rays_d, aabb, min_near, noise, T, bound):
+    N, dev = rays_o.shape[0], rays_o.device
+    nears = torch.empty(N, dtype=torch.float32, device=dev)
+    fars = torch.empty(N, dtype=torch.float32, device=dev)
+    enc_in = torch.empty(N * T, 3, dtype=torch.float32, device=dev)
+    ray_sh = torch.empty(N, 16, dtype=torch.float16, device=dev)
+    aabb = aabb.detach().to(device=dev, dtype=torch.float32).contiguous()
+    check(lib.foc_fixed_sample_aabb(ptr(rays_o), ptr(rays_d), ptr(aabb), ptr(noise), N, T, float(min_near), float(bound), ptr(nears), ptr(fars),
+                                    ptr(enc_in), ptr(ray_sh), stream_of(rays_o)), "fixed_sample_aabb")
+    return nears, fars, enc_in, ray_sh
 
 
 def ray_sh_rows(rays_d):
@@ -126,13 +138,14 @@
     @staticmethod
     def forward(ctx, h, cweights, ray_sh, nears, fars, noise, bg_ray, bg_scalar, N, T, density_scale, thresh, num_layers, activation, obj_feat=None,
                 want_sumsq=False, c_pre=None, w16_pre=None, input_pad=0.0, want_dist=False):
-        from .field import _half_of, pad_twin, object_feature_half
+        from .field import _half_of, pad_twin, object_feature_half, fp32_blob_route
         h = h.contiguous()
         assert h.dtype == torch.float16 and h.shape == (N * T, 16)
         assert ray_sh.dtype == torch.float16 and ray_sh.shape == (N, 16) and ray_sh.is_contiguous()
         dev, M = h.device, N * T
         st = stream_of(h)
-        w16 = w16_pre if w16_pre is not None else _half_of(cweights)
+        w32 = bool(c_pre is not None and w16_pre is None and float(input_pad) == 0.0 and fp32_blob_route(cweights))
+        w16 = cweights.detach() if w32 else w16_pre if w16_pre is not None else _half_of(cweights)
         obj16 = object_feature_half(obj_feat, "_render_tail")
         assert obj16 is None or w16.numel() == 64 * (48 + 64 * (int(num_layers) - 1) + 16)
         if c_pre is not None:
@@ -164,6 +177,7 @@
                               bg_ray if bg_ray is not None else empty, obj16 if obj16 is not None else empty,
                               ws if ctx.bg_grad or want_dist else empty, wm if want_dist else empty)
         ctx.outputs = (bool(want_sumsq), bool(want_dist))
+        ctx.w32 = w32
         ctx.flags = (noise is not None, bg_ray is not None, obj16 is not None, obj_feat.dtype if obj_feat is not None else None,
                      tuple(obj_feat.shape) if obj_feat is not None else None)
         ctx.dims = (N, T, float(density_scale), float(thresh), float(bg_scalar), int(num_layers), int(activation), float(input_pad))
@@ -207,7 +221,7 @@
         g_obj32 = torch.empty(16, dtype=torch.float32, device=dev) if has_obj and ctx.needs_input_grad[14] else None
         args = (ptr(grad_c), ptr(h), ptr(ray_sh), T, ptr(grad_h0), ptr(w16), M, 64, num_layers, activation, ptr(grad_h), ptr(g_w), ptr(wsb),
                 wsb.numel(), _C_WIDTH, ptr(obj16), ptr(g_obj32))
-        fn, extra = pad_twin("foc_color_head_backward", input_pad, has_obj)
+        fn, extra = (lib.foc_color_head_backward_w32, ()) if ctx.w32 else pad_twin("foc_color_head_backward", input_pad, has_obj)
         check(fn(*args, *extra, st), "color_head_backward")
         g_obj = g_obj32.to(obj_dtype).view(obj_shape) if g_obj32 is not None else None
         g_bg = g_image * (1 - ws).unsqueeze(-1) if ctx.bg_grad else None
@@ -263,20 +277,26 @@
     N, T = rays_o.shape[0], int(num_steps)
     dev = rays_o.device
     aabb = model.aabb_train if model.training else model.aabb_infer
-    nears, fars = raymarching.near_far_from_aabb(rays_o, rays_d, aabb, model.min_near)
+    from .field import field_plan, field_infer
+    from ._lib import get_option
+    plan = field_plan(model)
+    want_tail = plan.tail and model.training and torch.is_grad_enabled()
+    one_launch = want_tail and N > 0 and rays_o.is_cuda and get_option("FOC_SAMPLE_AABB") != 0
+    if not one_launch:
+        nears, fars = raymarching.near_far_from_aabb(rays_o, rays_d, aabb, model.min_near)
     noise = torch.rand(N * T, dtype=torch.float32, device=dev) if perturb else None
-    from .field import field_plan, field_infer
-    plan = field_plan(model)
     if getattr(model, "bg_radius", 0) > 0:
         bg_color = model._background_colour(rays_o, rays_d, bg_color)
-    want_tail = plan.tail and model.training and torch.is_grad_enabled()
     fused_infer = not torch.is_grad_enabled() and plan.infer
     if distortion and not torch.is_grad_enabled():
         raise ValueError("render_fixed_steps: distortion=True needs the training route (gradients enabled): the inference paths form no "
                          "differentiable weights; call it under torch.enable_grad() with model.train()")
     rb = ray_block_default() if fused_infer else 0
-    enc_in, _, ray_sh = fixed_sample(rays_o, rays_d, nears, fars, aabb, noise, T, model.bound, want_ray_sh=True) if want_tail else \
-        fixed_sample(rays_o, rays_d, nears, fars, aabb, noise, T, model.bound, ray_block=rb) + (None,)
+    if one_launch:
+        nears, fars, enc_in, ray_sh = fixed_sample_aabb(rays_o, rays_d, aabb, model.min_near, noise, T, model.bound)
+    else:
+        enc_in, _, ray_sh = fixed_sample(rays_o, rays_d, nears, fars, aabb, noise, T, model.bound, want_ray_sh=True) if want_tail else \
+            fixed_sample(rays_o, rays_d, nears, fars, aabb, noise, T, model.bound, ray_block=rb) + (None,)
 
     if fused_infer:
         obj_feat = model.encode_object_feature(yolo_details, dev) if plan.uses_object_feature else None
@@ -316,9 +336,10 @@
         if plan.field:
             colour = wc16 = None
             if want_tail and plan.train_forward:
-                from .field import _half_of
-                wc16 = _half_of(cweights)
-                colour = (wc16, plan.colour, ray_sh, T, _C_WIDTH, obj_feat, plan.colour_input_pad)
+                from .field import _half_of, fp32_blob_route
+                if not (plan.colour_input_pad == 0 and fp32_blob_route(cweights, fused_mlp(model, "sigma_net").weights)):
+                    wc16 = _half_of(cweights)
+                colour = (cweights if wc16 is None else wc16, plan.colour, ray_sh, T, _C_WIDTH, obj_feat, plan.colour_input_pad)
             h = hashgrid_mlp(enc, fused_mlp(model, "sigma_net"), enc_in, None, colour)
             if colour is not None:
                 h, c_pre = h
diff --git a/include/focnerf.h b/include/focnerf.h
--- a/include/focnerf.h
+++ b/include/focnerf.h
@@ -262,6 +262,18 @@
                                   const void *color_weights, uint32_t color_layers, uint32_t hidden_dim, uint32_t activation, uint32_t B,
                                   void *h, void *c, uint32_t out_width, const void *obj_feat, float input_pad, void *stream);
 
+int foc_field_forward_train_w32(const void *planes, const float *sigma_weights, uint32_t sigma_layers, const void *ray_sh, uint32_t samples_per_ray,
+                                const float *color_weights, uint32_t color_layers, uint32_t hidden_dim, uint32_t activation, uint32_t B,
+                                void *h, void *c, uint32_t out_width, const void *obj_feat, void *stream);
+int foc_ffmlp_backward_planar_w32(const void *grad, const void *inputs_planar, const float *weights, uint32_t B,
+                                  uint32_t input_dim, uint32_t output_dim, uint32_t hidden_dim, uint32_t num_layers,
+                                  uint32_t activation, uint32_t output_activation, int calc_grad_inputs,
+                                  void *grad_inputs_planar, float *grad_weights, void *workspace, uint64_t workspace_bytes, void *stream);
+int foc_color_head_backward_w32(const void *grad, const void *h, const void *ray_sh, uint32_t samples_per_ray,
+                                const void *grad_h0, const float *weights, uint32_t B, uint32_t hidden_dim,
+                                uint32_t num_layers, uint32_t activation, void *grad_h, float *grad_weights,
+                                void *workspace, uint64_t workspace_bytes, uint32_t out_width, const void *obj_feat, float *grad_obj, void *stream);
+
 int foc_allocate_splitk(uint64_t size);
 int foc_free_splitk(void);
 
@@ -315,6 +327,10 @@
 int foc_fixed_sample(const float *rays_o, const float *rays_d, const float *nears, const float *fars,
                      const float *aabb, const float *noise, uint32_t N, uint32_t T, float bound,
                      float *xyzs, float *enc_in, void *ray_sh, uint32_t ray_block, void *stream);
+
+int foc_fixed_sample_aabb(const float *rays_o, const float *rays_d, const float *aabb, const float *noise,
+                          uint32_t N, uint32_t T, float min_near, float bound, float *nears, float *fars,
+                          float *enc_in, void *ray_sh, void *stream);
 
 int foc_fixed_head_forward(const void *h, const float *rays_d, const float *nears, const float *fars,
                            const float *noise, uint32_t N, uint32_t T, float density_scale,
```
